# arnab39/equiadapt

Measured on AMD Instinct MI355X. Metric: canonicalize+invert images/sec (224x224 C8), higher is better.
Workload: dtype f32 (resampling / FFT / accumulation in fp32; the network's channel contraction as 2xfp16 split of every fp32 operand (within one fp32 ulp), 3 exact products, fp32 accumulate -- closer to fp64 than the fp32 matrix instruction, see step_ms_by_gemm_form); 1 GPU; configs[1]: 224x224x3 synthetic, C8, GroupEquivariantImageCanonicalization + ESCNNEquivariantNetwork in e2cnn's LAYER SHAPES (32 fields x 8 = 256 ch, k5, 3 layers, crop 0.8, resize 96) with this repository's own filter-bank parameterisation (bilinear-rotated banks; e2cnn's steerable basis is not restated -- e2cnn-trained weights enter via load_exported_dense), forward, then invert_canonicalization; batch_per_gpu=256, global_batch=256, parallelism=dp1 (no collective in the forward path)

## Files before the change

equiadapt_amd/_lib.py:

```python
import ctypes
import os
import subprocess
import threading

_HERE = os.path.dirname(os.path.abspath(__file__))
ROOT = os.path.dirname(_HERE)
CSRC = os.path.join(_HERE, "csrc")
SO_PATH = os.environ.get("EQA_LIB") or os.path.join(CSRC, "libeqa_hip.so")
SOURCES = [os.path.join(CSRC, f) for f in ("group_action.hip", "crop_resize.hip", "nearest_action.hip", "pooling.hip", "batchnorm.hip", "winograd.hip", "lift_conv.hip", "lift_conv_wide.hip", "lift_wgrad.hip", "pointcloud.hip", "vnsmall_train.hip", "vnsmall_tail.hip", "fftconv.hip", "lift_fft.hip", "cgemm3m.hip", "cgemm3m_bf16.hip", "smallconv.hip", "planegemm.hip", "convnet_train.hip")]
HEADERS = [os.path.join(CSRC, "eqa_common.hpp"), os.path.join(CSRC, "vn_common.hpp"), os.path.join(CSRC, "fft48.inc"), os.path.join(CSRC, "fft_common.inc")]
INCLUDE = os.path.join(ROOT, "include")

ABI_VERSION = 3

_c_f = ctypes.POINTER(ctypes.c_float)
_c_i = ctypes.POINTER(ctypes.c_int32)
_vp = ctypes.c_void_p
_int = ctypes.c_int

SIGNATURES = {
    "eqa_abi_version": (_int, []),
    "eqa_set_option": (_int, [_int, _int]),
    "eqa_get_option": (_int, [_int]),
    "eqa_fold_edge_pad_workspace_bytes": (ctypes.c_int64, [_int] * 4),
    "eqa_fold_edge_pad": (_int, [_vp, _vp, _vp, _int, _int, _int, _int, _vp]),
    "eqa_canon_transform_fwd": (_int, [_vp, _vp, _vp, _vp, _vp] + [_int] * 6 + [_vp]),
    "eqa_invert_action_fwd": (_int, [_vp, _vp, _vp, _vp, _vp, _vp] + [_int] * 6 + [_vp]),
    "eqa_group_action_pair": (_int, [_vp] * 4 + [_int, _int] + [_vp] * 5 + [_int, _int, _vp] + [_int] * 4 + [_vp]),
    "eqa_orbit_expand_fwd": (_int, [_vp, _vp, _vp, _vp] + [_int] * 5 + [_vp]),
    "eqa_group_action_fwd": (_int, [_vp, _vp, _vp, _vp, _vp, _vp] + [_int] * 12 + [_vp]),
    "eqa_group_action_fwd_hint": (_int, [_vp, _vp, _vp, _vp, _vp, _vp] + [_int] * 13 + [_vp]),
    "eqa_crop_resize_aa": (_int, [_vp] * 6 + [_int] * 9 + [_vp]),
    "eqa_mask_action_nearest": (_int, [_vp] * 5 + [_int] * 4 + [_vp]),
    "eqa_mask_action_nearest_planes": (_int, [_vp] * 5 + [_int] * 4 + [_vp]),
    "eqa_boxes_action": (_int, [_vp] * 5 + [_int, ctypes.c_float, _int, _vp]),
    "eqa_image_action_nearest": (_int, [_vp] * 5 + [_int] * 10 + [_vp]),
    "eqa_group_action_bwd_tiles": (_int, [_int, _int]),
    "eqa_group_action_bwd": (_int, [_vp] * 8 + [_int] * 12 + [_vp]),
    "eqa_group_action_bwd_theta": (_int, [_vp] * 8 + [_int] * 12 + [_vp]),
    "eqa_group_pool_workspace_bytes": (ctypes.c_int64, [_int] * 4),
    "eqa_group_pool_argmax": (_int, [_vp, _vp, _vp, _vp] + [_int] * 4 + [_vp]),
    "eqa_window_sums": (_int, [_vp, _vp, _vp, _int, _vp] + [_int] * 5 + [_vp]),
    "eqa_bn_partial_blocks": (ctypes.c_int64, [ctypes.c_int64]),
    "eqa_bn_stats_nhwc": (_int, [_vp, _vp, ctypes.c_int64, _int, _vp]),
    "eqa_bn_relu_dropout_nhwc": (_int, [_vp, _vp, _vp, _vp, ctypes.c_int64, _int, ctypes.c_float, ctypes.c_uint32, _vp]),
    "eqa_bn_bwd_reduce_nhwc": (_int, [_vp] * 5 + [ctypes.c_float, _vp, ctypes.c_int64, _int, _vp, _vp, ctypes.c_uint32, _vp]),
    "eqa_bn_bwd_apply_nhwc": (_int, [_vp] * 8 + [ctypes.c_float, _vp, ctypes.c_int64, _int, _vp, _vp, ctypes.c_uint32, _vp]),
    "eqa_window_sums_nhwc_act": (_int, [_vp, _vp, _vp, _int, ctypes.c_float, ctypes.c_uint32, _vp, _vp] + [_int] * 5 + [_vp]),
    "eqa_bn_bwd_reduce_nhwc_wsgrad": (_int, [_vp] * 4 + [ctypes.c_float, _vp] + [_int] * 5 + [_vp, _vp, ctypes.c_uint32, _vp]),
    "eqa_bn_bwd_apply_nhwc_wsgrad": (_int, [_vp] * 7 + [ctypes.c_float, _vp] + [_int] * 5 + [_vp, _vp, ctypes.c_uint32, _vp]),
    "eqa_vn_blocks": (_int, [_int]),
    "eqa_vn_knn": (_int, [_vp, _vp, _int, _int, _int, _vp]),
    "eqa_vn_convpos_stats": (_int, [_vp, _vp, _vp, _vp, _int, _int, _int, _vp]),
    "eqa_vn_convpos_fwd": (_int, [_vp] * 7 + [_int, _int, _int, _vp]),
    "eqa_vn_convpos_bwd_reduce": (_int, [_vp] * 10 + [_int, _int, _int, _vp]),
    "eqa_vn_convpos_bwd_apply": (_int, [_vp] * 12 + [_int, _int, _int, _vp]),
    "eqa_vn_tail_blocks": (_int, [_int]),
    "eqa_vn_tail_partial_floats": (_int, [_int]),
    "eqa_vn_tail_pass": (_int, [_int] + [_vp] * 8 + [_int, _int, _vp]),
    "eqa_vn_bn_finalize": (_int, [_vp, _int, _int, _int, ctypes.c_int64] + [_vp] * 5 + [ctypes.c_float, ctypes.c_float, _vp, _vp]),
    "eqa_vn_bn_bwd_finalize": (_int, [_vp, _int, _int, _int, ctypes.c_int64, _vp, _vp, _vp]),
    "eqa_window_grad_table": (_int, [_vp, _vp] + [_int] * 5 + [_vp]),
    "eqa_window_sums_gemv_bwd_workspace_bytes": (ctypes.c_int64, [_int, _int]),
    "eqa_window_sums_gemv_bwd": (_int, [_vp] * 6 + [_int, _int, _int, ctypes.c_double, _vp]),
    "eqa_window_sums_gemv": (_int, [_vp, _vp, _vp, _int, _int, _int, ctypes.c_double, ctypes.c_double, _vp]),
    "eqa_lift_conv_nhwc": (_int, [_vp, _vp, _vp, _int, _vp] + [_int] * 7 + [_vp]),
    "eqa_lift_conv_grouped": (_int, [_vp, _vp, _vp, _int, _vp] + [_int] * 7 + [_vp]),
    "eqa_lift_conv_stats_rows": (_int, [_int] * 7),
    "eqa_lift_conv_nhwc_stats": (_int, [_vp, _vp, _vp, _vp] + [_int] * 7 + [_vp]),
    "eqa_lift_conv_wgrad_supported": (_int, [_int] * 7),
    "eqa_lift_conv_wgrad_workspace_bytes": (ctypes.c_int64, [_int] * 7),
    "eqa_lift_conv_wgrad_nhwc": (_int, [_vp, _vp, _vp, _vp] + [_int] * 7 + [_vp]),
    "eqa_plane_gemm_supported": (_int, [_int, _int]),
    "eqa_plane_gemm": (_int, [_vp, _vp, _vp, ctypes.c_longlong, _int, _int, _int, _vp]),
    "eqa_winograd_f2k5_input": (_int, [_vp, _vp, _vp, _int, _int, _int, _int, _int, _vp]),
    "eqa_winograd_f2k5_output": (_int, [_vp, _vp, _int, _vp, _int, _int, _int, _int, _vp]),
    "eqa_winograd_f4k5_input": (_int, [_vp, _vp, _vp, _int, _int, _int, _int, _int, _vp]),
    "eqa_winograd_f4k5_output": (_int, [_vp, _vp, _int, _vp, _int, _int, _int, _int, _vp]),
    "eqa_winograd_f2k5_input_padded": (_int, [_vp, _vp, _int, _int, _int, _int, _int, _vp]),
    "eqa_winograd_f4k5_input_padded": (_int, [_vp, _vp, _int, _int, _int, _int, _int, _vp]),
    "eqa_winograd_f2k5_output_adjoint": (_int, [_vp, _vp, _int, _int, _int, _int, _vp]),
    "eqa_winograd_f4k5_output_adjoint": (_int, [_vp, _vp, _int, _int, _int, _int, _vp]),
    "eqa_winograd_f2k5_output_sums_workspace_bytes": (ctypes.c_int64, [_int] * 4),
    "eqa_winograd_f2k5_output_sums": (_int, [_vp, _vp, _int, _vp, _vp] + [_int] * 5 + [_vp]),
    "eqa_winograd_f4k5_output_sums": (_int, [_vp, _vp, _int, _vp, _vp] + [_int] * 5 + [_vp]),
    "eqa_fft48k5_tiles": (ctypes.c_int64, [_int]),
    "eqa_fft48k5_tile_pitch": (ctypes.c_int64, [ctypes.c_int64]),
    "eqa_fft48k5_frequencies": (_int, []),
    "eqa_fft48k5_filter_spectra": (_int, [_vp, _vp, _int, _int, _int, _vp]),
    "eqa_fft48k5_input_grad": (_int, [_vp, _vp, _vp] + [_int] * 4 + [_vp]),
    "eqa_fft48k5_grad_transform": (_int, [_vp, _vp, _vp] + [_int] * 4 + [_vp]),
    "eqa_fft48k5_filter_grad": (_int, [_vp, _vp, _int, _int, _vp]),
    "eqa_fft48k5_filter_grad3m": (_int, [_vp, _vp, _int, _int, _vp]),
    "eqa_fft48k5_cgemm3m_supported": (_int, [_int, _int]),
    "eqa_fft48k5_spectra3m_floats": (ctypes.c_int64, [_int, _int]),
    "eqa_fft48k5_filter_spectra3m": (_int, [_vp, _vp, _int, _int, _int, _vp]),
    "eqa_fft48k5_cgemm3m": (_int, [_vp, _vp, _vp, ctypes.c_int64, _int, _int, _vp]),
    "eqa_lift_conv_wide_supported": (_int, [_int, _int, _int, _int]),
    "eqa_lift_conv_wide_weight_floats": (ctypes.c_int64, [_int, _int, _int, _int]),
    "eqa_lift_conv_wide": (_int, [_vp, _vp, _vp, _int, _vp, _int, _int, _int, _int, _int, _int, _int, _vp]),
    "eqa_lift_conv_wide_wgrad_workspace_bytes": (ctypes.c_int64, [_int, _int, _int, _int]),
    "eqa_lift_conv_wide_wgrad": (_int, [_vp, _vp, _vp, _vp, _int, _int, _int, _int, _int, _int, _int, _vp]),
    "eqa_fft48k5_spectra3m_bf16_bytes": (ctypes.c_int64, [_int, _int]),
    "eqa_fft48k5_spectra3m_split": (_int, [_vp, _vp, _int, _int, _vp]),
    "eqa_fft48k5_cgemm3m_bf16x3": (_int, [_vp, _vp, _vp, ctypes.c_int64, _int, _int, _int, _vp]),
    "eqa_fft48k5_spectra3m_f16_bytes": (ctypes.c_int64, [_int, _int]),
    "eqa_fft48k5_spectra3m_split_f16": (_int, [_vp, _vp, _int, _int, ctypes.c_float, _vp]),
    "eqa_fft48k5_cgemm3m_f16x2": (_int, [_vp, _vp, _vp, ctypes.c_int64, _int, _int, _vp, _int, ctypes.c_float, _vp]),
    "eqa_fft48k5_wgrad3m_supported": (_int, [_int, _int]),
    "eqa_fft48k5_wgrad3m": (_int, [_vp, _vp, _vp, ctypes.c_int64, _int, _int, _vp]),
    "eqa_fft48k5_group": (_int, [_int, _int]),
    "eqa_fft48k5_workspace_bytes": (ctypes.c_int64, [_int] * 4),
    "eqa_fft48k5_input": (_int, [_vp, _vp, _vp, _vp] + [_int] * 5 + [_vp]),
    "eqa_fft48k5_input_grouped": (_int, [_vp, _vp, _vp, _vp] + [_int] * 5 + [_vp]),
    "eqa_fft48k5_input_grouped_supported": (_int, [_int]),
    "eqa_lift5_fft48k5_input_supported": (_int, [_int] * 4),
    "eqa_lift5_fft48k5_input": (_int, [_vp, _vp, _vp, _int, _vp] + [_int] * 4 + [_vp]),
    "eqa_lift5_fft48k5_input_dcmax": (_int, [_vp, _vp, _vp, _int, _vp, _vp] + [_int] * 4 + [_vp]),
    "eqa_lift5_pieces_f16_bytes": (ctypes.c_int64, [_int]),
    "eqa_absmax_slots": (_int, [_vp, ctypes.c_int64, _vp, _vp]),
    "eqa_lift5_fft48k5_input_f16x2": (_int, [_vp, _vp, ctypes.c_float, _vp, _int, _vp, _int, _vp, _vp] + [_int] * 4 + [_vp]),
    "eqa_lift5_pieces_bytes": (ctypes.c_int64, [_int]),
    "eqa_lift5_fft48k5_input_bf16x3": (_int, [_vp, _vp, _vp, _int, _vp] + [_int] * 4 + [_vp]),
    "eqa_fft48k5_output": (_int, [_vp, _vp, _vp, _int, _vp] + [_int] * 4 + [_vp]),
    "eqa_fft48k5_output_stats_rows": (ctypes.c_int64, [_int] * 4),
    "eqa_fft48k5_output_stats": (_int, [_vp, _vp, _vp, _vp] + [_int] * 4 + [_vp]),
    "eqa_fft48k5_output_sums": (_int, [_vp, _vp, _vp, _int, _vp, _vp] + [_int] * 5 + [_vp]),
    "eqa_fft48_supported": (_int, [_int]),
    "eqa_fft48_tiles": (ctypes.c_int64, [_int, _int]),
    "eqa_fft48_workspace_bytes": (ctypes.c_int64, [_int] * 5),
    "eqa_fft48_filter_spectra": (_int, [_vp, _vp, _int, _int, _int, _int, _vp]),
    "eqa_fft48_filter_spectra3m": (_int, [_vp, _vp, _int, _int, _int, _int, _vp]),
    "eqa_fft48_input": (_int, [_vp, _vp, _vp, _vp] + [_int] * 6 + [_vp]),
    "eqa_fft48_grad_transform": (_int, [_vp, _vp, _vp] + [_int] * 5 + [_vp]),
    "eqa_fft48_output": (_int, [_vp, _vp, _vp, _int, _vp] + [_int] * 5 + [_vp]),
    "eqa_fft48_input_grad": (_int, [_vp, _vp, _vp] + [_int] * 5 + [_vp]),
    "eqa_fft48_filter_grad": (_int, [_vp, _vp, _int, _int, _int, _int, _vp]),
    "eqa_conv_s2_supported": (_int, [_int] * 5),
    "eqa_conv_s2": (_int, [_vp, _vp, _vp, _int, _vp] + [_int] * 8 + [_vp]),
    "eqa_conv_s2_wgrad_supported": (_int, [_int] * 5),
    "eqa_conv_s2_wgrad_workspace_bytes": (ctypes.c_int64, [_int] * 8),
    "eqa_conv_s2_wgrad": (_int, [_vp] * 4 + [_int] * 8 + [_vp]),
    "eqa_conv_s2_dgrad_supported": (_int, [_int] * 4),
    "eqa_conv_s2_dgrad": (_int, [_vp] * 3 + [_int] * 7 + [_vp]),
    "eqa_bn_act_fwd": (_int, [_vp] * 5 + [ctypes.c_int64, _int, _int, _vp]),
    "eqa_bn_act_partial_blocks": (ctypes.c_int64, [ctypes.c_int64]),
    "eqa_bn_act_stats": (_int, [_vp, _vp, ctypes.c_int64, _int, _vp]),
    "eqa_bn_act_finalize": (_int, [_vp, ctypes.c_int64, _int, _vp, _vp, ctypes.c_double, ctypes.c_double] + [_vp] * 6 + [_vp]),
    "eqa_bn_act_bwd_finalize": (_int, [_vp, ctypes.c_int64, _int] + [_vp] * 7 + [_vp]),
    "eqa_bn_act_bwd_reduce": (_int, [_vp] * 8 + [ctypes.c_int64, _int, _int, _vp]),
    "eqa_bn_act_bwd_apply": (_int, [_vp] * 11 + [ctypes.c_int64, _int, _int, _vp]),
    "eqa_affine_relu_rows": (_int, [_vp, _vp, _vp, _vp, ctypes.c_int64, _int, _vp]),
    "eqa_cosine_group_activations": (_int, [_vp, _vp, _vp, _int, _int, _int, ctypes.c_float, _vp]),
    "eqa_bias_relu_nhwc": (_int, [_vp, _vp, ctypes.c_int64, _int, _vp]),
    "eqa_window_sums_nhwc_workspace_bytes": (ctypes.c_int64, [_int] * 4),
    "eqa_window_sums_nhwc": (_int, [_vp, _vp, _vp, _int, _vp, _vp] + [_int] * 5 + [_vp]),
    "eqa_window_sums_bwd_expand_nhwc": (_int, [_vp, _vp] + [_int] * 5 + [_vp]),
    "eqa_group_argmax": (_int, [_vp, _vp, _int, _int, _vp]),
    "eqa_vnsmall_workspace_bytes": (ctypes.c_int64, [_int, _int]),
    "eqa_vnsmall_fwd": (_int, [_vp, _vp, _vp, _vp, _int, _int, _int, _int, _vp]),
    "eqa_vnsmall_canonicalize": (_int, [_vp] * 6 + [_int] * 4 + [_vp]),
    "eqa_so3_rotate": (_int, [_vp, _vp, _vp, _int, _int, _int, _vp]),
    "eqa_gram_schmidt": (_int, [_vp, _vp, _int, _vp]),
    "eqa_gram_schmidt_bwd": (_int, [_vp, _vp, _vp, _int, _vp]),
    "eqa_modified_gram_schmidt": (_int, [_vp, _vp, _int, _vp]),
    "eqa_rigid_rows": (_int, [_vp, _vp, _vp, _vp, _int, _int, _vp]),
}

_lock = threading.Lock()
_lib = None


def source_hash(*names: str) -> str:
    import hashlib

    h = hashlib.sha1()
    for path in [os.path.join(CSRC, n) for n in names] + HEADERS:
        with open(path, "rb") as f:
            h.update(f.read())
    return h.hexdigest()[:16]


class EqaLibraryError(RuntimeError):
    pass


def build(force: bool = False, verbose: bool = False, extra_flags=(), out: str = None) -> str:
    import hashlib
    from concurrent.futures import ThreadPoolExecutor

    if extra_flags and not out:
        raise ValueError("a variant build (extra_flags) needs its own `out`: it must not replace the product library")
    out = out or SO_PATH
    hdr_time = max(os.path.getmtime(p) for p in HEADERS + [os.path.join(INCLUDE, "eqa_hip.h")])
    newest_src = max(hdr_time, max(os.path.getmtime(p) for p in SOURCES))
    if not force and not extra_flags and os.path.exists(out) and os.path.getmtime(out) >= newest_src:
        return out
    hipcc = os.environ.get("HIPCC", "/opt/rocm/bin/hipcc")
    flags = ["--offload-arch=gfx950", "-O3", "-fno-slp-vectorize", "-std=c++17", "-fPIC", "-I", INCLUDE, *extra_flags]
    tag = hashlib.sha1(" ".join(flags).encode()).hexdigest()[:10]
    objdir = os.path.join(CSRC, "_obj")
    os.makedirs(objdir, exist_ok=True)
    import fcntl

    lock_file = open(os.path.join(objdir, ".lock"), "w")
    fcntl.flock(lock_file, fcntl.LOCK_EX)
    try:
        if not force and not extra_flags and os.path.exists(out) and os.path.getmtime(out) >= newest_src:
            return out
        return _build_locked(hipcc, flags, tag, objdir, out, hdr_time, force, verbose, bool(extra_flags))
# ... 98 lines not shown
```

equiadapt_amd/csrc/crop_resize.hip:

```cpp
#include "eqa_common.hpp"

namespace {

constexpr int kAaBand = 8;
#ifndef EQA_AA_WIDE_MIN_K
#define EQA_AA_WIDE_MIN_K 8
#endif
constexpr int kAaMaxK = 20;

__global__ __launch_bounds__(kThreads) void crop_resize_aa_kernel(const float* __restrict__ x, float* __restrict__ y,
                                                                 const float* __restrict__ wx, const int32_t* __restrict__ x0,
                                                                 const float* __restrict__ wy, const int32_t* __restrict__ y0,
                                                                 int H, int W, int OH, int OW, int K, int max_rows) {
  extern __shared__ __attribute__((aligned(16))) float aa_tmp[];
  const int plane = blockIdx.y;
  const int r0 = blockIdx.x * kAaBand, r1 = min(r0 + kAaBand, OH);
  const int ybeg = y0[r0];
  const int yend = min(y0[r1 - 1] + K, H);
  const int nrows = min(yend - ybeg, max_rows);
  const float* src = x + (size_t)plane * H * W;
  const int rows_par = kThreads / OW;
  if (rows_par >= 1) {
    const int ox = threadIdx.x % OW, rsub = threadIdx.x / OW;
    if (rsub < rows_par) {
// ... 68 lines not shown
#pragma unroll
  for (int j = 0; j < K; ++j) {
    wv[j] = wx[ox * K + j];
    xo[j] = min(xs_g - xb + j, xl - 1);
  }
  if ((int)threadIdx.x < nband * K) tabw[threadIdx.x] = wy[r0 * K + threadIdx.x];
  const int ybeg = y0[r0];
  if ((int)threadIdx.x < nband) taby[threadIdx.x] = y0[r0 + threadIdx.x] - ybeg;
  const int yend = min(y0[r1 - 1] + K, H);
  const int nrows = min(yend - ybeg, cap_rows);
  const int nq = xl >> 2;
  const int tq = threadIdx.x & 63, tr = threadIdx.x >> 6;
  const bool prefetch = nq <= 64 && nrows <= 4 * NL;
  const size_t plane_sz = (size_t)H * W;
  const float* src0 = x + (size_t)ybeg * W + xb;
  typedef float aa_f4 __attribute__((ext_vector_type(4)));
  aa_f4 v[NL];
#define EQA_AA_PF_LOAD(plane_)                                                                                          \
  do {                                                                                                                  \
    const float* src_ = src0 + (size_t)(plane_) * plane_sz;                                                             \
    _Pragma("unroll") for (int k = 0; k < NL; ++k)                                                           \
      v[k] = *reinterpret_cast<const aa_f4*>(src_ + (size_t)min(tr + 4 * k, nrows - 1) * W + 4 * min(tq, nq - 1));     \
  } while (0)
  __builtin_amdgcn_s_waitcnt(0x0070);
  if (prefetch && plane0 < planes) EQA_AA_PF_LOAD(plane0);
  for (int plane = plane0; plane < planes; plane += plane_step) {
    if (prefetch) {
      if (tq < nq) {
#pragma unroll
        for (int k = 0; k < NL; ++k)
          if (tr + 4 * k < nrows) *reinterpret_cast<aa_f4*>(rows + (tr + 4 * k) * xl + 4 * tq) = v[k];
      }
      if (plane + plane_step < planes) EQA_AA_PF_LOAD(plane + plane_step);
    } else {
      const float* src = src0 + (size_t)plane * plane_sz;
      for (int q = tq; q < nq; q += 64)
        for (int rb = tr; rb < nrows; rb += 4) *reinterpret_cast<aa_f4*>(rows + rb * xl + 4 * q) = *reinterpret_cast<const aa_f4*>(src + (size_t)rb * W + 4 * q);
    }
    __syncthreads();
    if (rows_par >= 1) {
      if (rsub < rows_par) {
        for (int ry0 = rsub; ry0 < nrows; ry0 += 4 * rows_par) {
          float acc[4] = {0.0f, 0.0f, 0.0f, 0.0f};
#pragma unroll
          for (int u = 0; u < 4; ++u) {
            const float* row = rows + min(ry0 + u * rows_par, nrows - 1) * xl;
#pragma unroll
            for (int j = 0; j < K; ++j)
              acc[u] += wv[j] * row[xo[j]];
          }
#pragma unroll
          for (int u = 0; u < 4; ++u)
            if (ry0 + u * rows_par < nrows) tmp[(ry0 + u * rows_par) * OW + ox] = acc[u];
        }
      }
    } else {
      for (int idx = threadIdx.x; idx < nrows * OW; idx += kThreads) {
        const int ry = idx / OW, oxx = idx - ry * OW;
        const float* row = rows + ry * xl;
        const int xs = x0[oxx] - xb;
        float acc = 0.0f;
#pragma unroll
        for (int j = 0; j < K; ++j)
          acc += wx[oxx * K + j] * row[min(xs + j, xl - 1)];
        tmp[ry * OW + oxx] = acc;
      }
    }
    __syncthreads();
    float* dst = y + (size_t)plane * OH * OW;
    for (int idx = threadIdx.x; idx < nband * OW; idx += kThreads) {
      const int r = idx / OW, oxx = idx - r * OW;
      const int ys = taby[r];
      float acc = 0.0f;
#pragma unroll
      for (int j = 0; j < K; ++j)
        acc += tabw[r * K + j] * tmp[min(ys + j, nrows - 1) * OW + oxx];
      dst[(size_t)(r0 + r) * OW + oxx] = acc;
    }
    __syncthreads();
  }
#undef EQA_AA_PF_LOAD
}

__global__ __launch_bounds__(kThreads) void crop_resize_aa_wide_kernel(const float* __restrict__ x, float* __restrict__ y,
                                                                      const float* __restrict__ wx, const int32_t* __restrict__ x0,
                                                                      const float* __restrict__ wy, const int32_t* __restrict__ y0,
                                                                      int H, int W, int OH, int OW, int K, int max_rows, int xbeg,
                                                                      int xlen, int pad_shift, int row_stride, int rpi) {
  extern __shared__ __attribute__((aligned(16))) float aa_tmp[];
  float* rowbuf = aa_tmp + (size_t)max_rows * OW;
  const int plane = blockIdx.y;
  const int r0 = blockIdx.x * kAaBand, r1 = min(r0 + kAaBand, OH);
  const int ybeg = y0[r0];
  const int yend = min(y0[r1 - 1] + K, H);
  const int nrows = min(yend - ybeg, max_rows);
  const float* src = x + (size_t)plane * H * W;
  auto pos = [&](int e) { return pad_shift ? e + (e >> pad_shift) : e; };
  const bool fixed_col = (kThreads % OW) == 0 && K <= kAaMaxK;
  const bool vec_stage = rpi <= 8 && (xlen & 3) == 0 && (xbeg & 3) == 0 && (W & 3) == 0 && ((((uintptr_t)src) & 15) == 0);
  const int ox_fixed = threadIdx.x % OW;
  const int xs_fixed = x0[ox_fixed] - xbeg;
  float wreg[kAaMaxK];
#pragma unroll
  for (int j = 0; j < kAaMaxK; ++j) wreg[j] = (fixed_col && j < K) ? wx[ox_fixed * K + j] : 0.0f;
  const bool prefetch = vec_stage && xlen <= 4 * kThreads;
  const int e_pf = 4 * threadIdx.x;
  float4 pf[8];
  auto pf_load = [&](int ry0) {
    const int nr = min(rpi, nrows - ry0);
#pragma unroll
    for (int rr = 0; rr < 8; ++rr)
      pf[rr] = *reinterpret_cast<const float4*>(src + (size_t)(ybeg + ry0 + min(rr, nr - 1)) * W + xbeg + min(e_pf, xlen - 4));
  };
  if (prefetch && nrows > 0) pf_load(0);
  for (int ry0 = 0; ry0 < nrows; ry0 += rpi) {
    const int nr = min(rpi, nrows - ry0);
    if (prefetch) {
      if (e_pf < xlen) {
#pragma unroll
        for (int rr = 0; rr < 8; ++rr) {
          if (rr < nr) {
            float* lrow = rowbuf + rr * row_stride;
            lrow[pos(e_pf)] = pf[rr].x; lrow[pos(e_pf + 1)] = pf[rr].y; lrow[pos(e_pf + 2)] = pf[rr].z; lrow[pos(e_pf + 3)] = pf[rr].w;
          }
        }
      }
      if (ry0 + rpi < nrows) pf_load(ry0 + rpi);
    } else if (vec_stage) {
      for (int e = 4 * threadIdx.x; e < xlen; e += 4 * kThreads) {
        float4 v[8];
#pragma unroll
        for (int rr = 0; rr < 8; ++rr)
          v[rr] = *reinterpret_cast<const float4*>(src + (size_t)(ybeg + ry0 + min(rr, nr - 1)) * W + xbeg + e);
#pragma unroll
        for (int rr = 0; rr < 8; ++rr) {
          if (rr < nr) {
            float* lrow = rowbuf + rr * row_stride;
            lrow[pos(e)] = v[rr].x; lrow[pos(e + 1)] = v[rr].y; lrow[pos(e + 2)] = v[rr].z; lrow[pos(e + 3)] = v[rr].w;
          }
        }
      }
    } else {
      for (int rr = 0; rr < nr; ++rr) {
        const float* grow = src + (size_t)(ybeg + ry0 + rr) * W + xbeg;
        float* lrow = rowbuf + rr * row_stride;
        for (int e = threadIdx.x; e < xlen; e += kThreads) lrow[pos(e)] = grow[e];
      }
    }
    __syncthreads();
    if (fixed_col) {
      for (int rr = threadIdx.x / OW; rr < nr; rr += kThreads / OW) {
        const float* row = rowbuf + rr * row_stride;
        float acc = 0.0f;
#pragma unroll
        for (int j = 0; j < kAaMaxK; ++j)
          if (j < K) acc += wreg[j] * row[pos(min(xs_fixed + j, xlen - 1))];
        aa_tmp[(ry0 + rr) * OW + ox_fixed] = acc;
      }
    } else {
      for (int idx = threadIdx.x; idx < nr * OW; idx += kThreads) {
        const int rr = idx / OW, ox = idx - rr * OW;
        const float* row = rowbuf + rr * row_stride;
        const int xs = x0[ox] - xbeg;
        float acc = 0.0f;
        for (int j = 0; j < K; ++j) acc += wx[ox * K + j] * row[pos(min(xs + j, xlen - 1))];
        aa_tmp[(ry0 + rr) * OW + ox] = acc;
// ... 12 lines not shown
  }
}

constexpr int kAaStreamRows = 8;
__global__ __launch_bounds__(kThreads) void crop_resize_aa_stream_kernel(const float* __restrict__ x, float* __restrict__ y,
                                                                        const float* __restrict__ wx, const int32_t* __restrict__ x0,
                                                                        const float* __restrict__ wy, const int32_t* __restrict__ y0,
                                                                        int H, int W, int OH, int OW, int K, int xbeg, int xlen,
                                                                        int pad_shift, int row_stride) {
  extern __shared__ __attribute__((aligned(16))) float aa_rows[];
  const int plane = blockIdx.y;
  const int r0 = blockIdx.x * kAaBand, nr_out = min(kAaBand, OH - r0);
  int ys[kAaBand];
#pragma unroll
  for (int r = 0; r < kAaBand; ++r) ys[r] = y0[r0 + min(r, nr_out - 1)];
  const int ybeg = ys[0];
  const int span = ys[kAaBand - 1] + K - ybeg;
  const float* src = x + (size_t)plane * H * W + xbeg;
  const int e = 4 * (int)threadIdx.x;
  const int e_ld = min(e, xlen - 4);
  auto pos = [&](int i) { return pad_shift ? i + (i >> pad_shift) : i; };
  float4 acc[kAaBand];
#pragma unroll
  for (int r = 0; r < kAaBand; ++r) acc[r] = make_float4(0.f, 0.f, 0.f, 0.f);
  auto load8 = [&](float4 (&v)[kAaStreamRows], int yc) {
#pragma unroll
    for (int q = 0; q < kAaStreamRows; ++q)
      v[q] = *reinterpret_cast<const float4*>(src + (size_t)min(ybeg + yc + q, H - 1) * W + e_ld);
  };
  const int lane = threadIdx.x & 63;
  const int wq = lane >> 3, wr = lane & 7;
  const int ys_w = y0[r0 + min(wr, nr_out - 1)];
  auto wload = [&](int yc) {
    const int t = ybeg + yc + wq - ys_w;
    const bool ok = wr < nr_out && t >= 0 && t < K && yc + wq < span;
    return ok ? wy[(size_t)(r0 + wr) * K + min(max(t, 0), K - 1)] : 0.0f;
  };
  auto add8 = [&](const float4 (&v)[kAaStreamRows], float wv) {
#pragma unroll
    for (int q = 0; q < kAaStreamRows; ++q) {
#pragma unroll
      for (int r = 0; r < kAaBand; ++r) {
        const float w = __builtin_bit_cast(float, __builtin_amdgcn_readlane(__builtin_bit_cast(int, wv), 8 * q + r));
        acc[r].x += w * v[q].x; acc[r].y += w * v[q].y; acc[r].z += w * v[q].z; acc[r].w += w * v[q].w;
      }
    }
  };
  static_assert(kAaStreamRows == 8 && kAaBand == 8, "one weight per lane: 8 rows of a trip x 8 output rows = 64 lanes");
  float4 va[kAaStreamRows], vb[kAaStreamRows];
  float wa, wb = 0.0f;
  load8(va, 0);
  wa = wload(0);
  for (int yc = 0; yc < span; yc += 2 * kAaStreamRows) {
    if (yc + kAaStreamRows < span) { load8(vb, yc + kAaStreamRows); wb = wload(yc + kAaStreamRows); }
    add8(va, wa);
    if (yc + 2 * kAaStreamRows < span) { load8(va, yc + 2 * kAaStreamRows); wa = wload(yc + 2 * kAaStreamRows); }
    if (yc + kAaStreamRows < span) add8(vb, wb);
  }
  float* dst = y + (size_t)plane * OH * OW;
#pragma unroll
  for (int half = 0; half < 2; ++half) {
    if (e < xlen) {
#pragma unroll
      for (int rr = 0; rr < kAaBand / 2; ++rr) {
        float* lrow = aa_rows + rr * row_stride;
        const float4 v = acc[half * (kAaBand / 2) + rr];
        lrow[pos(e)] = v.x; lrow[pos(e + 1)] = v.y; lrow[pos(e + 2)] = v.z; lrow[pos(e + 3)] = v.w;
      }
    }
    __syncthreads();
    for (int idx = threadIdx.x; idx < (kAaBand / 2) * OW; idx += kThreads) {
      const int rr = idx / OW, ox = idx - rr * OW;
      const int r = half * (kAaBand / 2) + rr;
      if (r < nr_out) {
        const float* row = aa_rows + rr * row_stride;
        const int xs = x0[ox] - xbeg;
        float a = 0.0f;
        for (int j = 0; j < K; ++j) a += wx[ox * K + j] * row[pos(min(xs + j, xlen - 1))];
        dst[(size_t)(r0 + r) * OW + ox] = a;
      }
    }
    __syncthreads();
  }
}

}

extern "C" {

int eqa_crop_resize_aa(const float* x, float* y, const float* wx, const int32_t* x0, const float* wy, const int32_t* y0,
                       int planes, int H, int W, int OH, int OW, int K, int max_rows, int x_begin, int x_span, void* stream) {
  if (!x || !y || !wx || !x0 || !wy || !y0 || planes < 0 || H <= 0 || W <= 0 || OH <= 0 || OW <= 0 || K <= 0 || max_rows <= 0)
    return EQA_ERR_INVALID_ARG;
  const size_t lds = (size_t)max_rows * OW * sizeof(float);
  if (lds > 96 * 1024 || planes > 65535) return EQA_ERR_UNSUPPORTED;
  if (planes == 0) return EQA_OK;
  const dim3 grid((OH + kAaBand - 1) / kAaBand, planes);
  if (K > EQA_AA_WIDE_MIN_K && x_span > 0 && x_begin >= 0 && x_begin + x_span <= W) {
    const int stride = (x_span + OW / 2) / OW;
    const int pad_shift = (stride >= 2 && (stride & 1) == 0) ? __builtin_ctz((unsigned)stride) : 0;
    const int row_stride = x_span + (pad_shift ? (x_span >> pad_shift) : 0) + 1;
    const size_t row_bytes = (size_t)row_stride * sizeof(float);
    const int rpi = (int)std::min<size_t>(8, lds + row_bytes <= 96 * 1024 ? (96 * 1024 - lds) / row_bytes : 0);
    const size_t lds2 = lds + (size_t)rpi * row_bytes;
    static const bool stream_off = [] { const char* e = getenv("EQA_AA_STREAM"); return e && e[0] == '0'; }();
    if (!stream_off && x_span <= 4 * kThreads && (x_span & 3) == 0 && (x_begin & 3) == 0 && (W & 3) == 0 && (((uintptr_t)x) & 15) == 0 &&
        (size_t)(kAaBand / 2) * row_bytes <= 64 * 1024) {
      hipLaunchKernelGGL(crop_resize_aa_stream_kernel, grid, dim3(kThreads), (kAaBand / 2) * row_bytes, (hipStream_t)stream, x, y, wx, x0, wy,
                         y0, H, W, OH, OW, K, x_begin, x_span, pad_shift, row_stride);
      return launch_status();
    }
    if (rpi >= 1) {
      hipLaunchKernelGGL(crop_resize_aa_wide_kernel, grid, dim3(kThreads), lds2, (hipStream_t)stream, x, y, wx, x0, wy, y0, H, W, OH,
                         OW, K, max_rows, x_begin, x_span, pad_shift, row_stride, rpi);
      return launch_status();
    }
  }
  static const bool staged_off = [] { const char* e = getenv("EQA_AA_STAGED"); return e && e[0] == '0'; }();
  if (!staged_off && K <= EQA_AA_WIDE_MIN_K && (W & 3) == 0 && (((uintptr_t)x) & 15) == 0 && x_span > 0 && x_begin >= 0 &&
      x_begin + x_span <= W) {
    const int xb = x_begin & ~3, xl = std::min(W, (x_begin + x_span + 3) & ~3) - xb;
    static const int band_env = [] { const char* e = getenv("EQA_AA_BAND"); return e ? atoi(e) : 0; }();
    int band = band_env == 16 ? 16 : (band_env == 8 ? 8 : (OH >= 64 ? 16 : 8));
    auto staged_lds = [&](int bnd) { return ((size_t)(bnd / kAaBand) * max_rows * (xl + OW) + bnd * (EQA_AA_WIDE_MIN_K + 1)) * sizeof(float); };
    if (band == 16 && band_env != 16 && (staged_lds(16) > 64 * 1024 || 16 * K > kThreads)) band = 8;
    const int cap_rows = (band / kAaBand) * max_rows;
    const size_t lds3 = staged_lds(band);
    if (lds3 <= 64 * 1024 && band * K <= kThreads) {
      static const int per_cu = [] { const char* e = getenv("EQA_AA_BLOCKS_PER_CU"); return e ? std::max(1, atoi(e)) : 12; }();
      const int nbands = (OH + band - 1) / band;
      const int groups = std::max(1, (std::min(planes, (256 * per_cu + nbands - 1) / nbands) + kXcd - 1) / kXcd);
      const bool few = cap_rows <= 20;
#define EQA_AA_STAGED(K_)                                                                                                              \
  case K_:                                                                                                                             \
    if (band == 16)                                                                                                                    \
      hipLaunchKernelGGL((crop_resize_aa_staged_kernel<K_, 16, 10>), dim3(kXcd, nbands, groups), dim3(kThreads), lds3, (hipStream_t)stream, x, \
                         y, wx, x0, wy, y0, planes, H, W, OH, OW, cap_rows, xb, xl);                                                   \
    else if (few)                                                                                                                      \
      hipLaunchKernelGGL((crop_resize_aa_staged_kernel<K_, 8, 5>), dim3(kXcd, nbands, groups), dim3(kThreads), lds3, (hipStream_t)stream, x,  \
                         y, wx, x0, wy, y0, planes, H, W, OH, OW, cap_rows, xb, xl);                                                   \
    else                                                                                                                               \
      hipLaunchKernelGGL((crop_resize_aa_staged_kernel<K_, 8, 10>), dim3(kXcd, nbands, groups), dim3(kThreads), lds3, (hipStream_t)stream, x, \
                         y, wx, x0, wy, y0, planes, H, W, OH, OW, cap_rows, xb, xl);                                                   \
    break
      switch (K) {
        EQA_AA_STAGED(1); EQA_AA_STAGED(2); EQA_AA_STAGED(3); EQA_AA_STAGED(4); EQA_AA_STAGED(5); EQA_AA_STAGED(6); EQA_AA_STAGED(7);
        EQA_AA_STAGED(8);
        default: return EQA_ERR_UNSUPPORTED;
      }
#undef EQA_AA_STAGED
      return launch_status();
    }
  }
  hipLaunchKernelGGL(crop_resize_aa_kernel, grid, dim3(kThreads), lds, (hipStream_t)stream, x, y, wx, x0, wy, y0, H, W, OH, OW, K,
                     max_rows);
  return launch_status();
}

}
```

equiadapt_amd/csrc/fftconv.hip:

```cpp
#include <cstdlib>

#include "eqa_common.hpp"

namespace {

#include "fft_common.inc"

typedef float f32x2 __attribute__((ext_vector_type(2)));
__device__ __forceinline__ void fft_ldg2(const float2* p, float& re, float& im) {
  const f32x2 v = __builtin_nontemporal_load(reinterpret_cast<const f32x2*>(p));
  re = v[0];
  im = v[1];
}

__device__ __forceinline__ void fft_load_column(const float2* __restrict__ p, size_t fpitch, bool edge, float (&re)[kFftN],
                                                float (&im)[kFftN]) {
#pragma unroll
  for (int ky = 0; ky < kFftH; ++ky) fft_ldg2(p + ky * fpitch, re[ky], im[ky]);
  const float2* base2 = edge ? p + (size_t)(kFftH - 2) * fpitch : p + (size_t)kFftH * fpitch;
  const ptrdiff_t step2 = edge ? -(ptrdiff_t)fpitch : (ptrdiff_t)fpitch;
  const unsigned flip = edge ? 0x80000000u : 0u;
#pragma unroll
  for (int ky = kFftH; ky < kFftN; ++ky) {
    fft_ldg2(base2 + (ky - kFftH) * step2, re[ky], im[ky]);
// ... 1218 lines not shown
  if (x_grouped) return EQA_ERR_UNSUPPORTED;
  const unsigned cb = (C + kThreads - 1) / kThreads;
  const int chunk = fft_chunk_images(nimg, H, TX, C);
  for (int i0 = 0; i0 < nimg; i0 += chunk) {
    const int n = std::min(chunk, nimg - i0);
    hipLaunchKernelGGL(fft48_rows_fwd_kernel<kFftO>, dim3((unsigned)((size_t)n * H * TX), cb), dim3(kThreads), 0, st,
                       x + (size_t)i0 * H * W * C, T, in_bias, in_relu, H, W, C, TX, win);
    hipLaunchKernelGGL(fft48_cols_fwd_kernel<kFftO>, dim3((unsigned)((size_t)n * TY * TX * kFftH), cb), dim3(kThreads), 0, st, T, V, H, C,
                       TY, TX, fft_pitch(M), (size_t)i0 * TY * TX, fft_group_in(C), win);
  }
  return launch_status();
}

int eqa_fft48k5_input(const float* x, float* T, float* V, const float* in_bias, int in_relu, int nimg, int H, int W, int C,
                      void* stream) {
  if (!x || !T || !V || !fft_dims_ok(nimg, H, W, C)) return EQA_ERR_INVALID_ARG;
  if (nimg == 0) return EQA_OK;
  return fft_forward_impl(x, T, V, in_bias, in_relu, nimg, H, W, C, (int)eqa_fft48k5_tiles(H), (int)eqa_fft48k5_tiles(W), kFftN,
                          (hipStream_t)stream);
}

int eqa_fft48k5_input_grouped_supported(int C) {
  static const bool two_pass = getenv("EQA_FFT_TWO_PASS") != nullptr;
  return C > 0 && C % kFusCh == 0 && !two_pass;
}

int eqa_fft48k5_input_grouped(const float* x, float* T, float* V, const float* in_bias, int in_relu, int nimg, int H, int W, int C,
                              void* stream) {
  if (!x || !T || !V || !fft_dims_ok(nimg, H, W, C)) return EQA_ERR_INVALID_ARG;
  if (!eqa_fft48k5_input_grouped_supported(C)) return EQA_ERR_UNSUPPORTED;
  if (nimg == 0) return EQA_OK;
  return fft_forward_impl(x, T, V, in_bias, in_relu, nimg, H, W, C, (int)eqa_fft48k5_tiles(H), (int)eqa_fft48k5_tiles(W), kFftN,
                          (hipStream_t)stream, 1);
}

int eqa_fft48k5_grad_transform(const float* dy, float* T, float* G, int nimg, int OH, int OW, int C, void* stream) {
  if (!dy || !T || !G || nimg < 0 || OH <= 0 || OW <= 0 || C <= 0) return EQA_ERR_INVALID_ARG;
  if (nimg == 0) return EQA_OK;
  return fft_forward_impl(dy, T, G, nullptr, 0, nimg, OH, OW, C, (OH + kFftO - 1) / kFftO, (OW + kFftO - 1) / kFftO, kFftO,
                          (hipStream_t)stream);
}

int eqa_fft48k5_filter_grad(const float* D, float* dbank, int Cout, int Cin, void* stream) {
  if (!D || !dbank || Cout <= 0 || Cin <= 0) return EQA_ERR_INVALID_ARG;
  if (Cin > 65535) return EQA_ERR_UNSUPPORTED;
  hipLaunchKernelGGL((fft48_filter_grad_kernel<false, 5>), dim3(Cin, (Cout + kThreads - 1) / kThreads), dim3(kThreads), 0, (hipStream_t)stream, D,
                     dbank, Cout, Cin, fft_group_in(Cin), fft_group_in(Cout));
  return launch_status();
}

int eqa_fft48k5_filter_grad3m(const float* D, float* dbank, int Cout, int Cin, void* stream) {
  if (!D || !dbank || Cout <= 0 || Cin <= 0) return EQA_ERR_INVALID_ARG;
  if (Cin > 65535 || Cin % kFusCh || Cout % kFusCh) return EQA_ERR_UNSUPPORTED;
  hipLaunchKernelGGL((fft48_filter_grad_kernel<true, 5>), dim3(Cin, (Cout + kThreads - 1) / kThreads), dim3(kThreads), 0, (hipStream_t)stream, D,
                     dbank, Cout, Cin, kFusCh, kFusCh);
  return launch_status();
}

int eqa_fft48k5_output(const float* Mo, float* T2, const float* bias, int relu, float* y, int nimg, int OH, int OW, int C,
                       void* stream) {
  if (!Mo || !T2 || !y || nimg < 0 || OH <= 0 || OW <= 0 || C <= 0) return EQA_ERR_INVALID_ARG;
  if (nimg == 0) return EQA_OK;
  int fused = 0;
  const int rc = fft_output_impl<0>(Mo, T2, bias, relu, y, nimg, OH, OW, C, (hipStream_t)stream, &fused);
  return rc != EQA_OK ? rc : launch_status();
}

int64_t eqa_fft48k5_output_stats_rows(int nimg, int OH, int OW, int C) {
  if (nimg <= 0 || OH <= 0 || OW <= 0 || C <= 0) return 0;
  int fused = 0;
  int64_t rows = 0;
  const int rc = fft_output_impl<0>(nullptr, nullptr, nullptr, 0, nullptr, nimg, OH, OW, C, nullptr, &fused, nullptr, &rows);
  return rc == EQA_OK ? rows : 0;
}

int eqa_fft48k5_output_stats(const float* Mo, float* T2, float* y, double* partial, int nimg, int OH, int OW, int C, void* stream) {
  if (!Mo || !T2 || !y || !partial || nimg < 0 || OH <= 0 || OW <= 0 || C <= 0) return EQA_ERR_INVALID_ARG;
  if (nimg == 0) return EQA_OK;
  int fused = 0;
  const int rc = fft_output_impl<0>(Mo, T2, nullptr, 0, y, nimg, OH, OW, C, (hipStream_t)stream, &fused, partial);
  return rc != EQA_OK ? rc : launch_status();
}

int eqa_fft48k5_output_sums(const float* Mo, float* T2, const float* bias, int relu, double* S, void* workspace, int nimg,
                            int OH, int OW, int C, int k_next, void* stream) {
  if (!Mo || !T2 || !S || !workspace || nimg < 0 || OH <= 0 || OW <= 0 || C <= 0 || k_next <= 0) return EQA_ERR_INVALID_ARG;
  const int nb = k_next - 1;
  if ((nb != 4 && nb != 2) || OH < 2 * nb + 1 || OW < 2 * nb + 1 || k_next > kMaxWinK || nimg > 65535) return EQA_ERR_UNSUPPORTED;
  if (nimg == 0) return EQA_OK;
  hipStream_t st = (hipStream_t)stream;
  float* part = (float*)workspace;
  int fused = 0;
  const int rc = nb == 4 ? fft_output_impl<4>(Mo, T2, bias, relu, part, nimg, OH, OW, C, st, &fused)
                         : fft_output_impl<2>(Mo, T2, bias, relu, part, nimg, OH, OW, C, st, &fused);
  if (rc != EQA_OK) return rc;
  const int sub = fused ? (OW + kFftO - 1) / kFftO : 1;
  const int per_row = fused == 3 ? kPipeCons / 64 : fused;
  const int nseg = fused ? 2 * nb + per_row * ((OH + kFftO - 1) / kFftO) : OH;
  return eqa::launch_window_sums_nhwc_finalize(part, S, nimg, C, k_next, nseg * sub, st, sub);
}

}

namespace {

template <int KS>
struct FftK {
  static constexpr int O = kFftN + 1 - KS;

  static int forward(const float* x, float* T, float* V, const float* in_bias, int in_relu, int nimg, int H, int W, int C, int TY, int TX,
                     int win, hipStream_t st) {
    const size_t M = (size_t)nimg * TY * TX;
    if ((size_t)nimg * H * TX > 0x7fffffffULL || M * kFftH > 0x7fffffffULL) return EQA_ERR_UNSUPPORTED;
    static const bool two_pass = getenv("EQA_FFT_TWO_PASS") != nullptr;
    if (C % kFusCh == 0 && M * (C / kFusCh) <= 0x7fffffffULL && !two_pass &&
        allow_dynamic_lds((const void*)fft48_fwd_fused_kernel<O>, kFusLds * 4)) {
      const unsigned nwork = (unsigned)(M * (C / kFusCh));
      const size_t xb = (size_t)nimg * H * W * C * 4, vb = (size_t)kFftF * fft_pitch(M) * 2 * C * 4;
      hipLaunchKernelGGL(fft48_fwd_fused_kernel<O>, dim3(nwork), dim3(kFusThreads), kFusLds * sizeof(float), st, x, V, in_bias, in_relu, H,
                         W, C, TY, TX, fft_pitch(M), nwork, win, xb <= 0xfffffff0ULL ? (unsigned)xb : 0u,
                         vb <= 0xfffffff0ULL ? (unsigned)vb : 0u, 0);
      return launch_status();
    }
    const unsigned cb = (C + kThreads - 1) / kThreads;
    const int chunk = fft_chunk_images(nimg, H, TX, C);
    for (int i0 = 0; i0 < nimg; i0 += chunk) {
      const int n = std::min(chunk, nimg - i0);
      hipLaunchKernelGGL(fft48_rows_fwd_kernel<O>, dim3((unsigned)((size_t)n * H * TX), cb), dim3(kThreads), 0, st,
                         x + (size_t)i0 * H * W * C, T, in_bias, in_relu, H, W, C, TX, win);
      hipLaunchKernelGGL(fft48_cols_fwd_kernel<O>, dim3((unsigned)((size_t)n * TY * TX * kFftH), cb), dim3(kThreads), 0, st, T, V, H, C,
                         TY, TX, fft_pitch(M), (size_t)i0 * TY * TX, fft_group_in(C), win);
    }
    return launch_status();
  }

  static int output(const float* Mo, float* T2, const float* bias, int relu, float* y, int nimg, int OH, int OW, int C, hipStream_t st) {
    const int TY = (OH + O - 1) / O, TX = (OW + O - 1) / O;
    const size_t M = (size_t)nimg * TY * TX;
    if ((size_t)nimg * OH > 0x7fffffffULL || M * kFftH > 0x7fffffffULL) return EQA_ERR_UNSUPPORTED;
    static const bool two_pass = getenv("EQA_FFT_TWO_PASS") != nullptr;
    constexpr int lds_bytes = kFftH * (kFftN * 2 * kInvCh + kInvCh) * (int)sizeof(float);
    if (C % kInvCh == 0 && M * (C / kInvCh) <= 0x7fffffffULL && !two_pass &&
        allow_dynamic_lds((const void*)fft48_inv_fused_kernel<0, kInvCh, O>, lds_bytes)) {
      const unsigned nwork = (unsigned)(M * (C / kInvCh));
      const size_t mo_total = (size_t)kFftF * fft_pitch(M) * C * 8;
      hipLaunchKernelGGL((fft48_inv_fused_kernel<0, kInvCh, O>), dim3(nwork), dim3(kFftN * kInvCh), lds_bytes, st, Mo, bias, relu, y, OH, OW, C,
                         TY, TX, fft_pitch(M), nwork, mo_total <= 0xfffffff0ULL ? (unsigned)mo_total : 0u);
      return launch_status();
    }
    const unsigned cb = (C + kThreads - 1) / kThreads;
    const int chunk = fft_chunk_images(nimg, OH, TX, C);
    for (int i0 = 0; i0 < nimg; i0 += chunk) {
      const int n = std::min(chunk, nimg - i0);
      hipLaunchKernelGGL((fft48_cols_inv_kernel<false, O>), dim3((unsigned)((size_t)n * TY * TX * kFftH), cb), dim3(kThreads), 0, st, Mo, T2,
                         OH, C, TY, TX, fft_pitch(M), (size_t)i0 * TY * TX);
      hipLaunchKernelGGL((fft48_rows_inv_kernel<0, O>), dim3((unsigned)((size_t)n * OH), cb), dim3(kThreads), 0, st, T2, bias, relu, y, OH,
                         OW, C, TX, (size_t)i0);
    }
    return launch_status();
  }

  static int input_grad(const float* Cg, float* T2, float* dx, int nimg, int H, int W, int C, hipStream_t st) {
    const int OH = H - (KS - 1), OW = W - (KS - 1);
    const int TY = (OH + O - 1) / O, TX = (OW + O - 1) / O;
    const size_t M = (size_t)nimg * TY * TX;
    if ((size_t)nimg * H > 0x7fffffffULL || M * kFftH > 0x7fffffffULL) return EQA_ERR_UNSUPPORTED;
    const unsigned cb = (C + kThreads - 1) / kThreads;
    const int chunk = fft_chunk_images(nimg, TY * kFftN, TX, C);
    for (int i0 = 0; i0 < nimg; i0 += chunk) {
      const int n = std::min(chunk, nimg - i0);
      hipLaunchKernelGGL((fft48_cols_inv_kernel<true, O>), dim3((unsigned)((size_t)n * TY * TX * kFftH), cb), dim3(kThreads), 0, st, Cg, T2,
                         OH, C, TY, TX, fft_pitch(M), (size_t)i0 * TY * TX);
      hipLaunchKernelGGL(fft48_rows_inv_add_kernel<O>, dim3((unsigned)((size_t)n * H), cb), dim3(kThreads), 0, st, T2,
                         dx + (size_t)i0 * H * W * C, H, W, C, TY, TX);
    }
    return launch_status();
  }

  static int spectra(const float* bank, float* B, int Cout, int Cin, float sgn, hipStream_t st) {
    hipLaunchKernelGGL(fft48_filter_spectra_kernel<KS>, dim3(Cin, (Cout + kThreads - 1) / kThreads), dim3(kThreads), 0, st, bank, B, Cout,
                       Cin, fft_group_in(Cin), sgn);
    return launch_status();
// ... 101 lines not shown
```

equiadapt_amd/csrc/lift_fft.hip:

```cpp
#include <cstdlib>

#include "eqa_common.hpp"

#ifndef EQA_LF_AUX
#define EQA_LF_AUX 2
#endif

namespace {

#include "fft_common.inc"

typedef float f32x4 __attribute__((ext_vector_type(4)));
typedef unsigned u32x4 __attribute__((ext_vector_type(4)));

#ifdef EQA_LF_CLOCK
__device__ unsigned long long g_lf_clock[64];
__device__ __forceinline__ int lf_clock_slot(int wave) { return wave == 8 ? 0 : wave == 1 ? 1 : wave == 0 ? 2 : wave == 6 ? 3 : wave == 11 ? 4 : -1; }
#define LF_CLOCK_BEGIN() const bool lfc_on = blockIdx.x == 0 && (threadIdx.x & 63) == 0 && lf_clock_slot(wave) >= 0; \
  if (blockIdx.x == 0 && (threadIdx.x & 63) == 0) { unsigned hw_; asm volatile("s_getreg_b32 %0, hwreg(HW_REG_HW_ID)" : "=s"(hw_)); g_lf_clock[40 + wave] = hw_; } \
  unsigned long long lfc_t = __builtin_readcyclecounter(); unsigned long long lfc_s[16] = {0, 0, 0, 0, 0, 0, 0, 0, 0, 0, 0, 0, 0, 0, 0, 0}
#define LF_CLOCK(i) do { const unsigned long long n_ = __builtin_readcyclecounter(); lfc_s[i] += n_ - lfc_t; lfc_t = n_; } while (0)
#define LF_CLOCK_END() do { if (lfc_on) for (int i_ = 0; i_ < 8; ++i_) g_lf_clock[8 * lf_clock_slot(wave) + i_] = lfc_s[i_]; } while (0)
#else
#define LF_CLOCK_BEGIN() do { } while (0)
// ... 88 lines not shown
                                                 int relu, float* __restrict__ V, int H0, int W0, int C, int TY, int TX, size_t Mp,
                                                 unsigned nwork, unsigned v_bytes, unsigned x_bytes, unsigned bank_bytes,
                                                 float* __restrict__ dcmax, const float* __restrict__ xbound, int nxbound, float w_scale) {
  constexpr bool COLS = ROLE == kCols;
  constexpr bool PIECES = FORM == 3;
  constexpr bool H2 = FORM == 2;
  constexpr int NSUB = PIECES ? 12 : (H2 ? 4 : 3);
  constexpr int SUBROWS = kFftN / NSUB;
  constexpr int NGRP = 12 / NSUB;
  extern __shared__ float lds[];
  float* const tile = lds;
  float* const patch = lds + kLfTileFloats;
  const int tid = threadIdx.x;
  const int lane = tid & 63;
  const int wave = __builtin_amdgcn_readfirstlane(tid >> 6);
  const int j = lane & 15, q = lane >> 4;
  const int ngrp = C / kLfCh;
  const int H1 = H0 - 4, W1 = W0 - 4;
  const unsigned nblk = gridDim.x;
  const unsigned patch_b = (unsigned)(kLfTileFloats * 4);
  LF_CLOCK_BEGIN();

  const __amdgpu_buffer_rsrc_t xr = __builtin_amdgcn_make_buffer_rsrc(const_cast<float*>(x), 0, x_bytes, 0x00020000);
  float pre[COLS ? kLfPre : 1];
  auto prefetch = [&](const LfItem& it, int sub, bool live) {
    if constexpr (COLS) {
      int tq = tid;
      asm volatile("" : "+v"(tq));
#pragma unroll
      for (int i = 0; i < kLfPre; ++i) {
        const int idx = tq + kLfStagers * i;
        const int pr = idx / kLfPatchPitch, pc = idx - pr * kLfPatchPitch;
        const int gy = it.gy0 + kLfSubRows * sub + pr, gxc = it.gx0 * 3 + pc;
        const bool ok = live && idx < kLfPatchFloats && gy < H0 && gxc < W0 * 3;
        const unsigned off = ok ? (unsigned)(((it.img * H0 + gy) * (size_t)(W0 * 3) + gxc) * 4) : 0xfffffff0u;
        pre[i] = __builtin_bit_cast(float, __builtin_amdgcn_raw_buffer_load_b32(xr, off, 0, 0));
      }
    }
  };
  auto stage = [&]() {
    if constexpr (COLS) {
#pragma unroll
      for (int i = 0; i < kLfPre; ++i) {
        const int idx = tid + kLfStagers * i;
        if (idx < kLfPatchFloats) patch[idx] = pre[i];
      }
    }
  };

  float preg[COLS && PIECES ? 2 : 1][3];
  auto prefetch_grp = [&](const LfItem& it, int g, int which, bool live) {
    if constexpr (COLS && PIECES) {
      int tq = tid;
      asm volatile("" : "+v"(tq));
      const int pr = tq / 52, px = tq - pr * 52;
      const int gy = it.gy0 + 4 * g + pr, gx = it.gx0 + px;
      const bool ok = live && tq < 208 && gy < H0 && gx < W0;
      const unsigned off = ok ? (unsigned)((((it.img * H0 + gy) * (size_t)W0 + gx) * 3) * 4) : 0xfffffff0u;
#pragma unroll
      for (int c = 0; c < 3; ++c) preg[which][c] = __builtin_bit_cast(float, __builtin_amdgcn_raw_buffer_load_b32(xr, off, c * 4, 0));
    }
  };
  auto stage_grp = [&](int g, int which) {
    if constexpr (COLS && PIECES) {
      if (tid < 208) {
        const int pr = tid / 52, px = tid - pr * 52;
        __bf16 pc[3][3];
#pragma unroll
        for (int c = 0; c < 3; ++c) lf_split3(preg[which][c], pc[0][c], pc[1][c], pc[2][c]);
        char* dst = reinterpret_cast<char*>(lds) + patch_b + ((4 * g + pr) & 7) * kLpRowB + px * 8;
#pragma unroll
        for (int pl = 0; pl < 3; ++pl) {
          const lf_bf16x4 v = {pc[pl][0], pc[pl][1], pc[pl][2], (__bf16)0.0f};
          *reinterpret_cast<lf_bf16x4*>(dst + pl * kLpPlaneB) = v;
        }
      }
    }
  };

  float preh[(!COLS && H2) ? kLhPre : 1][3];
  float x_scale = 1.0f, out_scale = 1.0f;
  if constexpr (H2) {
    float mx = 0.0f;
    for (int t = lane; t < nxbound; t += 64) mx = fmaxf(mx, xbound[t]);
#pragma unroll
    for (int o = 32; o > 0; o >>= 1) mx = fmaxf(mx, __shfl_xor(mx, o));
    int ex = 0;
    if (mx > 0.0f && mx < 3.0e38f) (void)frexpf(mx, &ex);
    ex = __builtin_amdgcn_readfirstlane(min(max(14 - ex, -100), 100));
    x_scale = ldexpf(1.0f, ex);
    out_scale = ldexpf(1.0f, -ex) / w_scale;
  }
  int h_pr[(!COLS && H2) ? kLhPre : 1], h_px[(!COLS && H2) ? kLhPre : 1];
  if constexpr (!COLS && H2) {
#pragma unroll
    for (int i = 0; i < kLhPre; ++i) {
      const int idx = tid - 6 * 64 + kLfStagers * i;
      h_pr[i] = idx / 52;
      h_px[i] = idx - h_pr[i] * 52;
    }
  }
  auto prefetch_h = [&](const LfItem& it, int row0, int nrows, bool live) {
    if constexpr (!COLS && H2) {
#ifdef EQA_LF_H2_NOPREFETCH
      if (row0 >= 0) return;
#endif
#pragma unroll
      for (int i = 0; i < kLhPre; ++i) {
        const int pr = h_pr[i], px = h_px[i];
        const int gy = it.gy0 + row0 + pr, gx = it.gx0 + px;
        const bool ok = live && pr < nrows && gy < H0 && gx < W0;
        const unsigned off = ok ? (unsigned)((((it.img * H0 + gy) * (size_t)W0 + gx) * 3) * 4) : 0xfffffff0u;
#pragma unroll
        for (int c = 0; c < 3; ++c) preh[i][c] = __builtin_bit_cast(float, __builtin_amdgcn_raw_buffer_load_b32(xr, off, c * 4, 0));
      }
    }
  };
  auto stage_h = [&](int row0, int nrows) {
    if constexpr (!COLS && H2) {
#pragma unroll
      for (int i = 0; i < kLhPre; ++i) {
        asm volatile("" : "+v"(preh[i][0]), "+v"(preh[i][1]), "+v"(preh[i][2]));
        if (h_pr[i] < nrows) {
          const int pr = h_pr[i], px = h_px[i];
          _Float16 hi[3], lo[3];
#pragma unroll
          for (int c = 0; c < 3; ++c) {
            const float v = preh[i][c] * x_scale;
            hi[c] = (_Float16)v;
            lo[c] = (_Float16)(v - (float)hi[c]);
          }
          char* dst = reinterpret_cast<char*>(lds) + patch_b + ((row0 + pr) & (kLhRing - 1)) * kLhRowB + px * 8;
          const lf_f16x4 vh = {hi[0], hi[1], hi[2], (_Float16)0.0f}, vl = {lo[0], lo[1], lo[2], (_Float16)0.0f};
          *reinterpret_cast<lf_f16x4*>(dst) = vh;
          *reinterpret_cast<lf_f16x4*>(dst + kLhPlaneB) = vl;
        }
      }
    }
  };

  const int nr = (wave == 10 || wave == 11) ? 2 : 3;
  const int r0 = wave == 8 ? 0 : (wave == 9 ? 3 : (wave == 6 ? 6 : (wave == 10 ? 9 : (wave == 7 ? 11 : 14))));
  unsigned a_off[kLfSteps];
  float wreg[kLfSteps];
  f32x4 bias4;
  auto setup = [&](const LfItem& it) {
    const __amdgpu_buffer_rsrc_t br = __builtin_amdgcn_make_buffer_rsrc(const_cast<float*>(bank), 0, bank_bytes, 0x00020000);
    const unsigned wb = (unsigned)((it.grp * kLfCh + j) * 75 * 4);
#pragma unroll
    for (int t = 0; t < kLfSteps; ++t) {
      int ky, e;
      bool spare;
      lf_slot(4 * t + q, ky, e, spare);
      a_off[t] = patch_b + (unsigned)(((r0 + ky) * kLfPatchPitch + j * 3 + e) * 4);
      wreg[t] = __builtin_bit_cast(float, __builtin_amdgcn_raw_buffer_load_b32(br, spare ? 0xfffffff0u : wb + (unsigned)((ky * 15 + e) * 4), 0, 0));
    }
#pragma unroll
    for (int r = 0; r < 4; ++r) bias4[r] = bias ? bias[it.grp * kLfCh + 4 * q + r] : 0.0f;
    asm volatile("" : "+v"(bias4));
  };
#ifndef EQA_LF_AHEAD
#define EQA_LF_AHEAD 5
#endif
  constexpr int kAhead = EQA_LF_AHEAD;
  auto conv_rows = [&](const LfItem& it, int y0) {
    float b[3][kLfSteps], bq[2][3][kAhead];
    auto lds_at = [&](int t, int drow, int tx3) {
// ... 617 lines not shown
```

equiadapt_amd/csrc/pooling.hip:

```cpp
#include "eqa_common.hpp"

namespace {


constexpr int kPoolSplitTarget = 2048;


template <bool VEC>
__global__ __launch_bounds__(kThreads) void group_pool_partial_kernel(const float* __restrict__ feat,
                                                                     double* __restrict__ partial, int Cf, int G,
                                                                     int HW, int cps, int splits) {
  extern __shared__ __attribute__((aligned(16))) double acc[];
  const int s = blockIdx.x, b = blockIdx.y;
  const int tid = threadIdx.x, lane = tid & 63, wave = tid >> 6;
  for (int k = tid; k < 4 * G; k += kThreads) acc[k] = 0.0;
  __syncthreads();
  const int c_lo = s * cps, c_hi = min(c_lo + cps, Cf);
  const int planes = (c_hi - c_lo) * G;
  const float* base = feat + ((size_t)b * Cf + c_lo) * G * HW;
  for (int p = wave; p < planes; p += 4) {
    const float* pl = base + (size_t)p * HW;
    float v0 = 0.f, v1 = 0.f, v2 = 0.f, v3 = 0.f;
    if (VEC) {
      const float4* p4 = reinterpret_cast<const float4*>(pl);
// ... 343 lines not shown
#endif
  for (int it = threadIdx.x; it < nch * kk; it += blockDim.x) {
    const int cl = it / kk, uv = it - cl * kk;
    const int u = uv / k, v = uv - u * k;
    if constexpr (KW > 0) {
      constexpr int NB = KW - 1;
      float p0[NB], pc[NB][NB];
      double tc[NB];
#pragma unroll
      for (int r = 0; r < NB; ++r) p0[r] = s_brd[r < u ? r : NB + r][cl * nval];
#pragma unroll
      for (int j = 0; j < NB; ++j) {
        const int i = j < v ? 1 + j : 1 + NB + j;
        tc[j] = s_tot[cl * nval + i];
#pragma unroll
        for (int r = 0; r < NB; ++r) pc[j][r] = s_brd[r < u ? r : NB + r][cl * nval + i];
      }
      double a = s_tot[cl * nval];
#pragma unroll
      for (int r = 0; r < NB; ++r) a -= (double)p0[r];
#pragma unroll
      for (int j = 0; j < NB; ++j) {
        a -= tc[j];
#pragma unroll
        for (int r = 0; r < NB; ++r) a += (double)pc[j][r];
      }
      out[((size_t)b * C + c0) * kk + it] = a;
    } else {
      auto P = [&](int s, int i) { return (double)s_brd[s][cl * nval + i]; };
      double a = s_tot[cl * nval];
      for (int r = 0; r < nb; ++r) a -= r < u ? P(r, 0) : P(nb + r, 0);
      for (int j = 0; j < nb; ++j) {
        const int i = j < v ? 1 + j : 1 + nb + j;
        a -= s_tot[cl * nval + i];
        for (int r = 0; r < nb; ++r) a += r < u ? P(r, i) : P(nb + r, i);
      }
      out[((size_t)b * C + c0) * kk + it] = a;
    }
  }
}

constexpr int kGemvMaxE = 16;

template <int THREADS, int EMAX, int COLS>
__global__ __launch_bounds__(THREADS) void sums_gemv_kernel(const double* __restrict__ S, const double* __restrict__ Wm,
                                                            float* __restrict__ act, int K, int E, double scale, double shift) {
  __shared__ double s_red[THREADS / 64][kGemvMaxE];
  const int b = blockIdx.x;
  const double* sb = S + (size_t)b * K;
  double acc[kGemvMaxE];
#pragma unroll
  for (int e = 0; e < kGemvMaxE; ++e) acc[e] = 0.0;
  for (int j = threadIdx.x; j < K; j += COLS * THREADS) {
    double s[COLS], w[COLS][EMAX];
#pragma unroll
    for (int u = 0; u < COLS; ++u) {
      const bool in = j + u * THREADS < K;
      s[u] = in ? sb[j + u * THREADS] : 0.0;
#pragma unroll
      for (int e = 0; e < EMAX; ++e) w[u][e] = (in && e < E) ? Wm[(size_t)e * K + j + u * THREADS] : 0.0;
    }
#pragma unroll
    for (int u = 0; u < COLS; ++u)
#pragma unroll
      for (int e = 0; e < EMAX; ++e)
        if (e < E && j + u * THREADS < K) acc[e] += s[u] * w[u][e];
  }
  const int lane = threadIdx.x & 63, wave = threadIdx.x >> 6;
#pragma unroll
  for (int e = 0; e < kGemvMaxE; ++e) {
    double v = acc[e];
#pragma unroll
    for (int off = 32; off > 0; off >>= 1) v += __shfl_down(v, off, 64);
    if (lane == 0) s_red[wave][e] = v;
  }
  __syncthreads();
  if (threadIdx.x < E) {
    double v = 0.0;
    for (int w = 0; w < THREADS / 64; ++w) v += s_red[w][threadIdx.x];
    act[(size_t)b * E + threadIdx.x] = (float)(v * scale + shift);
  }
}


__global__ __launch_bounds__(kThreads) void affine_relu_rows_kernel(const float* __restrict__ h, const float* __restrict__ scale,
                                                                   const float* __restrict__ shift, float* __restrict__ z, size_t n_vec,
                                                                   int Dq) {
  const size_t i0 = (size_t)blockIdx.x * kThreads + threadIdx.x, stride = (size_t)gridDim.x * kThreads;
  QuadWalk w(i0, stride, Dq);
  for (size_t i = i0; i < n_vec; i += stride, w.next()) {
    const int q = (int)w.q;
    const float4 v = reinterpret_cast<const float4*>(h)[i];
    const float4 sc = reinterpret_cast<const float4*>(scale)[q], sh = reinterpret_cast<const float4*>(shift)[q];
    reinterpret_cast<float4*>(z)[i] = make_float4(fmaxf(v.x * sc.x + sh.x, 0.f), fmaxf(v.y * sc.y + sh.y, 0.f),
                                                  fmaxf(v.z * sc.z + sh.z, 0.f), fmaxf(v.w * sc.w + sh.w, 0.f));
  }
}

__global__ __launch_bounds__(kThreads) void cosine_group_activations_kernel(const float* __restrict__ v, const float* __restrict__ ref,
                                                                           float* __restrict__ act, int B, int G, int V, float eps) {
  const int lane = threadIdx.x & 63;
  const int r = blockIdx.x * (kThreads / 64) + (threadIdx.x >> 6);
  if (r >= G * B) return;
  float rr = 0.f, vv = 0.f;
  for (int k = lane; k < V; k += 64) {
    const float a = ref[k], x = v[(size_t)r * V + k];
    rr += a * a;
    vv += x * x;
  }
  rr = wave_sum_f(rr);
  vv = wave_sum_f(vv);
  const float inv_r = 1.0f / fmaxf(sqrtf(rr), eps), inv_v = 1.0f / fmaxf(sqrtf(vv), eps);
  float dot = 0.f;
  for (int k = lane; k < V; k += 64) dot += (ref[k] * inv_r) * (v[(size_t)r * V + k] * inv_v);
  dot = wave_sum_f(dot);
  if (lane == 0) act[(size_t)(r % B) * G + r / B] = dot;
}

}

int eqa::launch_window_sums_nhwc_finalize(const float* part, double* S, int B, int C, int k, int nseg, hipStream_t stream, int sub) {
  if (B > 65535) return EQA_ERR_UNSUPPORTED;
  const dim3 fgrid((C + kFinCh - 1) / kFinCh, B);
  const dim3 fblock(std::min(C, kFinCh) * (2 * k - 1) > kThreads ? kFinThreads : kThreads);
  if (k == 5)
    hipLaunchKernelGGL(window_sums_nhwc_finalize_kernel<5>, fgrid, fblock, 0, stream, part, S, B, C, k, nseg, sub);
  else if (k == 3)
    hipLaunchKernelGGL(window_sums_nhwc_finalize_kernel<3>, fgrid, fblock, 0, stream, part, S, B, C, k, nseg, sub);
  else if (k - 1 <= kWsSmallBorder)
    hipLaunchKernelGGL(window_sums_nhwc_finalize_kernel<0>, fgrid, fblock, 0, stream, part, S, B, C, k, nseg, sub);
  else
    hipLaunchKernelGGL((window_sums_nhwc_finalize_kernel<0, kWsMaxBorder>), fgrid, fblock, 0, stream, part, S, B, C, k, nseg, sub);
  return launch_status();
}

namespace {

constexpr int kWgtCh = 64;
__global__ __launch_bounds__(kWgtCh) void window_grad_table_kernel(const double* __restrict__ dS, float* __restrict__ table, int C, int H,
                                                                  int W, int k) {
  extern __shared__ double s_p[];
  const int kk = k * k, stride = kk + 1;
  const int b = blockIdx.y, c0 = blockIdx.x * kWgtCh, nch = min(kWgtCh, C - c0);
  const double* src = dS + ((size_t)b * C + c0) * kk;
  for (int i = threadIdx.x; i < nch * kk; i += kWgtCh) s_p[(i / kk) * stride + i % kk] = src[i];
  __syncthreads();
  const int c = threadIdx.x;
  if (c >= nch) return;
  double* p = s_p + c * stride;
  for (int u = 0; u < k; ++u)
    for (int v = 1; v < k; ++v) p[u * k + v] += p[u * k + v - 1];
  for (int u = 1; u < k; ++u)
    for (int v = 0; v < k; ++v) p[u * k + v] += p[(u - 1) * k + v];
  const int nb = k - 1, T = 2 * nb + 1;
  auto range = [&](int t, int n, int& lo, int& hi) {
    const int rep = t <= nb ? t : n - nb + (t - nb - 1);
    lo = max(0, rep - (n - k));
    hi = min(k - 1, rep);
  };
  auto rect = [&](int u0, int u1, int v0, int v1) -> double {
    if (u0 > u1 || v0 > v1) return 0.0;
    double r = p[u1 * k + v1];
    if (u0 > 0) r -= p[(u0 - 1) * k + v1];
    if (v0 > 0) r -= p[u1 * k + v0 - 1];
    if (u0 > 0 && v0 > 0) r += p[(u0 - 1) * k + v0 - 1];
    return r;
// ... 46 lines not shown
  double acc = 0.0;
  for (int s = 0; s < nslice; ++s) acc += partial[(size_t)s * n + i];
  dW[i] = scale * acc;
}

constexpr int kGemvBwdSlices = 16;

}

extern "C" {

int64_t eqa_group_pool_workspace_bytes(int B, int Cf, int G, int HW) {
  (void)HW;
  if (B <= 0 || Cf <= 0 || G <= 0) return 0;
  return (int64_t)B * pool_splits(B, Cf) * G * (int64_t)sizeof(double);
}

int eqa_group_pool_argmax(const float* feat, float* act, int32_t* gidx, void* workspace, int B, int Cf, int G, int HW,
                          void* stream) {
  if (B == 0) return EQA_OK;
  if (!feat || !act || !workspace || B < 0 || Cf <= 0 || G <= 0 || HW <= 0) return EQA_ERR_INVALID_ARG;
  if (gidx && G > 64) return EQA_ERR_UNSUPPORTED;
  if (B > 65535) return EQA_ERR_UNSUPPORTED;
  hipStream_t st = (hipStream_t)stream;
  const int splits = pool_splits(B, Cf);
  const int cps = (Cf + splits - 1) / splits;
  const int used = (Cf + cps - 1) / cps;
  double* partial = (double*)workspace;
  const bool vec = (HW % 4 == 0) && (((uintptr_t)feat & 15) == 0);
  const size_t lds = (size_t)4 * G * sizeof(double);
  if (vec)
    hipLaunchKernelGGL((group_pool_partial_kernel<true>), dim3(used, B), dim3(kThreads), lds, st, feat, partial, Cf, G, HW, cps, used);
  else
    hipLaunchKernelGGL((group_pool_partial_kernel<false>), dim3(used, B), dim3(kThreads), lds, st, feat, partial, Cf, G, HW, cps, used);
  if (hipGetLastError() != hipSuccess) return EQA_ERR_LAUNCH;
  const double inv_count = 1.0 / ((double)Cf * (double)HW);
  hipLaunchKernelGGL(group_pool_finalize_kernel, dim3((B + 3) / 4), dim3(kThreads), 0, st, partial, act, gidx, B, G, used, inv_count);
  return launch_status();
}

int eqa_group_argmax(const float* act, int32_t* gidx, int B, int G, void* stream) {
  if (B == 0 && G > 0 && G <= 64) return EQA_OK;
  if (!act || !gidx || B < 0 || G <= 0) return EQA_ERR_INVALID_ARG;
  if (G > 64) return EQA_ERR_UNSUPPORTED;
  hipLaunchKernelGGL(group_argmax_kernel, dim3((B + 3) / 4), dim3(kThreads), 0, (hipStream_t)stream, act, gidx, B, G);
  return launch_status();
}

int eqa_window_sums(const float* x, const float* scale, const float* shift, int relu, double* out, int B, int C, int H,
                    int W, int k, void* stream) {
  if (!x || !out || B < 0 || C <= 0 || H <= 0 || W <= 0 || k <= 0 || k > H || k > W) return EQA_ERR_INVALID_ARG;
  if (k > kMaxWinK) return EQA_ERR_UNSUPPORTED;
  const size_t lds = (size_t)((H * W + 3) & ~3) * sizeof(float) + (size_t)k * W * sizeof(double);
  if (lds > 64 * 1024 || (long long)B * C > 0x7fffffffLL) return EQA_ERR_UNSUPPORTED;
  if (B == 0) return EQA_OK;
  const bool vec = ((H * W) % 4 == 0) && (((uintptr_t)x & 15) == 0);
  hipStream_t st = (hipStream_t)stream;
  if (vec)
    hipLaunchKernelGGL((window_sums_kernel<true>), dim3((unsigned)(B * C)), dim3(kThreads), lds, st, x, scale, shift, relu, out, C, H, W, k);
  else
    hipLaunchKernelGGL((window_sums_kernel<false>), dim3((unsigned)(B * C)), dim3(kThreads), lds, st, x, scale, shift, relu, out, C, H, W, k);
  return launch_status();
}

int eqa_window_sums_gemv(const double* S, const double* Wm, float* act, int B, int K, int E, double scale, double shift,
                         void* stream) {
  if (B < 0 || K <= 0 || E <= 0) return EQA_ERR_INVALID_ARG;
  if (B == 0) return EQA_OK;
  if (!S || !Wm || !act) return EQA_ERR_INVALID_ARG;
  if (E > kGemvMaxE) return EQA_ERR_UNSUPPORTED;
  const int per_thread = (K + kThreads - 1) / kThreads;
  if (E <= 8 && per_thread > 5)
    hipLaunchKernelGGL((sums_gemv_kernel<kThreads, 8, 9>), dim3(B), dim3(kThreads), 0, (hipStream_t)stream, S, Wm, act, K, E, scale, shift);
  else if (E <= 8 && per_thread > 2)
    hipLaunchKernelGGL((sums_gemv_kernel<kThreads, 8, 5>), dim3(B), dim3(kThreads), 0, (hipStream_t)stream, S, Wm, act, K, E, scale, shift);
  else if (E <= 8)
    hipLaunchKernelGGL((sums_gemv_kernel<kThreads, 8, 2>), dim3(B), dim3(kThreads), 0, (hipStream_t)stream, S, Wm, act, K, E, scale, shift);
  else
    hipLaunchKernelGGL((sums_gemv_kernel<kThreads, kGemvMaxE, 5>), dim3(B), dim3(kThreads), 0, (hipStream_t)stream, S, Wm, act, K, E, scale,
                       shift);
  return launch_status();
}

int eqa_affine_relu_rows(const float* h, const float* scale, const float* shift, float* z, int64_t rows, int D, void* stream) {
  if (!h || !scale || !shift || !z || rows < 0 || D <= 0) return EQA_ERR_INVALID_ARG;
  if (D % 4 != 0 || (((uintptr_t)h | (uintptr_t)z | (uintptr_t)scale | (uintptr_t)shift) & 15)) return EQA_ERR_UNSUPPORTED;
  if (rows == 0) return EQA_OK;
  const size_t n_vec = (size_t)rows * (D / 4);
  const unsigned blocks = (unsigned)std::min<size_t>((n_vec + kThreads - 1) / kThreads, 8192);
  hipLaunchKernelGGL(affine_relu_rows_kernel, dim3(blocks), dim3(kThreads), 0, (hipStream_t)stream, h, scale, shift, z, n_vec, D / 4);
  return launch_status();
}

int eqa_cosine_group_activations(const float* v, const float* ref, float* act, int B, int G, int V, float eps, void* stream) {
  if (!v || !ref || !act || B < 0 || G <= 0 || V <= 0) return EQA_ERR_INVALID_ARG;
  if (B == 0) return EQA_OK;
  if ((int64_t)B * G > 0x7fffffff) return EQA_ERR_UNSUPPORTED;
  const int rows = B * G, per = kThreads / 64;
  hipLaunchKernelGGL(cosine_group_activations_kernel, dim3((rows + per - 1) / per), dim3(kThreads), 0, (hipStream_t)stream, v, ref, act, B,
                     G, V, eps);
  return launch_status();
}

int eqa_bias_relu_nhwc(float* x, const float* bias, int64_t n_pixels, int C, void* stream) {
  if (!x || !bias || n_pixels < 0 || C <= 0) return EQA_ERR_INVALID_ARG;
  if (C % 4 != 0 || (((uintptr_t)x | (uintptr_t)bias) & 15)) return EQA_ERR_UNSUPPORTED;
  if (n_pixels == 0) return EQA_OK;
  const size_t n_vec = (size_t)n_pixels * (C / 4);
  const unsigned blocks = (unsigned)((n_vec + kThreads - 1) / kThreads < 8192 ? (n_vec + kThreads - 1) / kThreads : 8192);
  hipLaunchKernelGGL(bias_relu_nhwc_kernel, dim3(blocks), dim3(kThreads), 0, (hipStream_t)stream, x, bias, n_vec, C / 4);
  return launch_status();
}

int eqa_window_sums_bwd_expand_nhwc(const float* table, float* dx, int B, int H, int W, int C, int k, void* stream) {
  if (!table || !dx || B < 0 || H <= 0 || W <= 0 || C <= 0 || k <= 0 || H < 2 * k - 1 || W < 2 * k - 1) return EQA_ERR_INVALID_ARG;
  if (C % 4 != 0 || (((uintptr_t)table | (uintptr_t)dx) & 15) || (size_t)B * H > 0x7fffffffULL) return EQA_ERR_UNSUPPORTED;
  if (B == 0) return EQA_OK;
  hipLaunchKernelGGL(window_sums_bwd_expand_kernel, dim3((unsigned)((size_t)B * H)), dim3(kThreads), 0, (hipStream_t)stream, table,
                     dx, H, W, C / 4, k - 1);
  return launch_status();
}

static int ws_nhwc_bands(int H, int k) {
  const int interior = H - 2 * (k - 1);
  int nb = (interior + 9) / 10;
  if (nb < 1) nb = 1;
  return nb;
}

int64_t eqa_window_sums_nhwc_workspace_bytes(int B, int C, int H, int k) {
  if (B <= 0 || C <= 0 || H <= 0 || k <= 0) return 0;
  const int nseg = 2 * (k - 1) + ws_nhwc_bands(H, k);
  return (int64_t)B * nseg * C * (1 + 2 * (k - 1)) * (int64_t)sizeof(float);
}

static int window_sums_nhwc_impl(const float* x, const float* scale, const float* shift, int relu, float drop_p, uint32_t seed, double* out,
                                 void* workspace, int B, int C, int H, int W, int k, void* stream);

int eqa_window_sums_nhwc(const float* x, const float* scale, const float* shift, int relu, double* out, void* workspace,
                         int B, int C, int H, int W, int k, void* stream) {
  return window_sums_nhwc_impl(x, scale, shift, relu, 0.0f, 0u, out, workspace, B, C, H, W, k, stream);
}

int eqa_window_sums_nhwc_act(const float* x, const float* scale, const float* shift, int relu, float drop_p, uint32_t seed, double* out,
                             void* workspace, int B, int C, int H, int W, int k, void* stream) {
  if (!(drop_p >= 0.0f && drop_p < 1.0f)) return EQA_ERR_INVALID_ARG;
  return window_sums_nhwc_impl(x, scale, shift, relu, drop_p, seed, out, workspace, B, C, H, W, k, stream);
}

static int window_sums_nhwc_impl(const float* x, const float* scale, const float* shift, int relu, float drop_p, uint32_t seed, double* out,
                                 void* workspace, int B, int C, int H, int W, int k, void* stream) {
  if (!x || !out || !workspace || B < 0 || C <= 0 || H <= 0 || W <= 0 || k <= 0) return EQA_ERR_INVALID_ARG;
  if (k > kMaxWinK || C % 4 != 0 || H < 2 * (k - 1) + 1 || W < 2 * (k - 1) + 1 || B > 65535) return EQA_ERR_UNSUPPORTED;
  if ((((uintptr_t)x) & 15) || (scale && (((uintptr_t)scale) & 15)) || (shift && (((uintptr_t)shift) & 15))) return EQA_ERR_UNSUPPORTED;
  if (B == 0) return EQA_OK;
  hipStream_t st = (hipStream_t)stream;
  const int nbands = ws_nhwc_bands(H, k);
  const int nseg = 2 * (k - 1) + nbands;
  const uint32_t thr = dropout_threshold(drop_p);
#define EQA_WS_SEG(R_, D_)                                                                                                     \
  do {                                                                                                                         \
    if (k - 1 <= kWsSmallBorder)                                                                                               \
      hipLaunchKernelGGL((window_sums_nhwc_segment_kernel<R_, D_>), dim3(nseg, B), dim3(kThreads), 0, st, x, scale, shift, relu, \
                         (float*)workspace, C, H, W, k, nbands, thr, 1.0f / (1.0f - drop_p), seed);                            \
    else                                                                                                                       \
      hipLaunchKernelGGL((window_sums_nhwc_segment_kernel<R_, D_, kWsMaxBorder>), dim3(nseg, B), dim3(kThreads), 0, st, x, scale, \
// ... 58 lines not shown
```

equiadapt_amd/images/canonicalization_networks/escnn_networks.py:

```python
import os
from typing import List, Sequence

import torch
import torch.nn as nn
import torch.nn.functional as F

from equiadapt_amd.images.canonicalization_networks.custom_group_equivariant_layers import (
    RotationEquivariantConv,
    RotationEquivariantConvLift,
    RotoReflectionEquivariantConv,
    RotoReflectionEquivariantConvLift,
)
from equiadapt_amd import ops
from equiadapt_amd.common.utils import update_running_stats
from equiadapt_amd.images.canonicalization_networks import fftconv, winograd
from equiadapt_amd.images.canonicalization_networks.pooling import (
    WindowSumsFunction,
    conv_then_group_pool,
    group_pool,
    window_sums_to_activations,
)


class _InnerBatchNorm(nn.BatchNorm3d):
# ... 361 lines not shown
        shift = bn.bias - bn.running_mean * scale
        b = conv.bias if conv.bias is not None else torch.zeros_like(scale)
        bias = b * scale + shift
        if not isinstance(conv, _DenseConv):
            scale, bias = scale.repeat_interleave(E), bias.repeat_interleave(E)
        bank = conv.expanded_weights() * scale[:, None, None, None]
        bank, bias = bank.contiguous(memory_format=torch.channels_last), bias.contiguous()
        self._fold_cache[id(conv)] = (key, bank, bias)
        return bank, bias

    def _derived(self, conv, build, *tag):
        key = self._fold_cache[id(conv)][0]
        hit = self._fold_cache.get((*tag, id(conv)))
        if hit is None or hit[0] != key:
            hit = (key, build())
            self._fold_cache[(*tag, id(conv))] = hit
        return hit[1]

    @staticmethod
    def _plain_5x5(conv) -> bool:
        return not conv.lifting and conv.kernel_size == 5 and conv.stride == 1 and conv.padding == 0

    @staticmethod
    def _lift_kernel(conv, bank, h, narrow_unchecked: bool = False):
        if not conv.lifting or os.environ.get("EQA_LIFT_MFMA", "1") == "0":
            return None
        k, (cout, cin) = conv.kernel_size, bank.shape[:2]
        unit = conv.stride == 1 and conv.padding == 0
        if (unit or narrow_unchecked) and ops.lift_conv_supported(cin, k, k, cout):
            return "narrow"
        if (unit and h.is_contiguous(memory_format=torch.channels_last) and h.shape[-2] >= k and h.shape[-1] >= k
                and ops.lift_conv_wide_supported(cin, k, k, cout)):
            return "wide"
        return None

    def _route(self, i, h, bank, convs, nhwc):
        conv, tail = convs[i], convs[-1]
        cout, cin = bank.shape[:2]
        k, kt = conv.kernel_size, tail.kernel_size
        last_before_tail = i == len(convs) - 2
        if nhwc and self._plain_5x5(conv) and fftconv.applicable(h, cin, cout):
            return "fft5", (last_before_tail and kt in (3, 5) and tail.supports_linear_tail() and min(h.shape[-2:]) - 4 >= 2 * kt - 1), 0
        if (nhwc and not conv.lifting and k != 5 and conv.stride == 1 and conv.padding == 0
                and h.is_contiguous(memory_format=torch.channels_last) and fftconv.applicable_k(h.shape, cin, cout, k, h.device)):
            return "fftk", False, 0
        if nhwc and self._plain_5x5(conv) and winograd.applicable(h, cin, cout):
            m = winograd.tile_for(h)
            if last_before_tail and not winograd.sums_applicable(h, kt, m) and winograd.sums_applicable(h, kt, 2):
                m = 2
            return "wino", last_before_tail and winograd.sums_applicable(h, kt, m), m
        lift = self._lift_kernel(conv, bank, h) if nhwc else None
        if lift == "narrow":
            nxt = convs[i + 1] if i + 1 < len(convs) - 1 else None
            if nxt is not None and self._plain_5x5(nxt):
                if fftconv.lift_fused_applicable(h.shape, bank.shape, nxt.out_channels * nxt.num_group_elements, h.device):
                    return "lift_fused", False, 0
                if fftconv.grouped_applicable((h.shape[0], cout, h.shape[2] - k + 1, h.shape[3] - k + 1), cout, cout, h.device):
                    return "lift_grouped", False, 0
            return "lift", False, 0
        return ("lift_wide" if lift == "wide" else "lib"), False, 0

    def _forward_inference(self, x: torch.Tensor) -> torch.Tensor:
        convs, norms = self._layers()
        tail = convs[-1]
        nhwc = (self.out_channels * self.num_group_elements) % 4 == 0
        h = x.contiguous(memory_format=torch.channels_last) if nhwc else x
        pending = None
        for i, (conv, bn) in enumerate(zip(convs[:-1], norms)):
            bank, bias = self._folded(conv, bn)
            route, sums, m = self._route(i, h, bank, convs, nhwc)
            k, (H, W) = conv.kernel_size, h.shape[-2:]
            last_before_tail, shift = i == len(convs) - 2, None
            if route != "fft5" and isinstance(h, (fftconv.GroupedMap, fftconv.LiftedInput)):
                h = h.materialize()
            if route in ("fft5", "fftk", "wino"):
                in_bias, pending = pending, None
                sums_k = tail.kernel_size if sums else 0
                if route == "wino":
                    U = self._derived(conv, lambda: winograd.transform_filters(bank, m), "wino", m)
                    h = winograd.conv5x5(h, U, bias, relu=True, in_bias=in_bias, in_relu=in_bias is not None, sums_k=sums_k)
                else:
                    Bf = self._derived(conv, lambda: fftconv.spectra_for_k(bank), "fft")
                    if route == "fft5":
                        h = fftconv.conv5x5(h, Bf, bias, True, in_bias, in_bias is not None, sums_k=sums_k)
                    else:
                        h = fftconv.conv_kxk(h, Bf, k, bias, True, in_bias, in_bias is not None)
            else:
                if pending is not None:
                    ops.bias_relu_nhwc_(h, pending)
                    pending = None
                if route == "lift_fused":
                    operand = {}
                    form = fftconv.LiftedInput.form_operand()
                    if form is not None:
                        operand[form[1]] = self._derived(conv, lambda: form[2](bank), form[0])
                    h = fftconv.LiftedInput(h, bank, bias, True, **operand)
                elif route != "lib":
                    pack = ops.pack_lift_weights_wide if route == "lift_wide" else ops.pack_lift_weights
                    wpk = self._derived(conv, lambda: pack(bank), "lift")
                    if route == "lift_grouped":
                        h = fftconv.GroupedMap(ops.lift_conv_grouped(h, wpk, bias, True, k, k))
                    else:
                        h = (ops.lift_conv_wide if route == "lift_wide" else ops.lift_conv_nhwc)(h, wpk, bias, True, k, k)
                else:
                    h = F.conv2d(h, bank)
                    if last_before_tail:
                        shift = bias
                    elif nhwc and h.is_contiguous(memory_format=torch.channels_last):
                        pending = bias
                    else:
                        h = torch.relu_(h + bias[None, :, None, None])
            if sums:
                return window_sums_to_activations(h, tail, H - k + 1, W - k + 1)
            if last_before_tail:
                return conv_then_group_pool(h, tail, shift=shift, relu=shift is not None)
        raise AssertionError("unreachable: the network always has at least two convolutions")

    @staticmethod
    def _inner_bn(h: torch.Tensor, bn: nn.BatchNorm3d, E: int, conv_bias) -> torch.Tensor:
        Bn, C, H, W = h.shape
        Fd = C // E
        if bn.training or bn.running_mean is None:
            n = Bn * E * H * W
            s1 = h.sum(dim=(0, 2, 3), dtype=torch.float64).view(Fd, E).sum(1)
            s2 = (h * h).sum(dim=(0, 2, 3), dtype=torch.float64).view(Fd, E).sum(1)
            mean = s1 / n
            var = (s2 / n - mean * mean).clamp_min(0.0)
            with torch.no_grad():
                full_mean = mean if conv_bias is None else mean + conv_bias.double()
                update_running_stats(bn, full_mean, var * (n / max(n - 1, 1)))
            mean, var = mean.float(), var.float()
        else:
            mean = bn.running_mean if conv_bias is None else bn.running_mean - conv_bias
            var = bn.running_var
        scale = bn.weight * torch.rsqrt(var + bn.eps)
        shift = bn.bias - mean * scale
        return h * scale.repeat_interleave(E)[None, :, None, None] + shift.repeat_interleave(E)[None, :, None, None]

    def _forward_training(self, x: torch.Tensor) -> torch.Tensor:
        mods = list(self.eqv_network)
        convs = [m for m in mods if hasattr(m, "expanded_weights")]
        norms = [m for m in mods if isinstance(m, _InnerBatchNorm)]
        drops = [m for m in mods if isinstance(m, nn.Dropout)]
        E = self.num_group_elements
        h = x.contiguous(memory_format=torch.channels_last)
        tail = convs[-1]
        S = None
        epilogue_stats = os.environ.get("EQA_TRAIN_FUSED_BN", "1") != "0" and os.environ.get("EQA_TRAIN_EPILOGUE_STATS", "1") != "0"
        for li, (conv, bn, drop) in enumerate(zip(convs[:-1], norms, drops)):
            bank = conv.expanded_weights()
            part = None
            lift = self._lift_kernel(conv, bank, h, narrow_unchecked=True)
            if not conv.lifting and conv.kernel_size == 5 and winograd.applicable(h, bank.shape[1], bank.shape[0]):
                if (epilogue_stats and (bn.training or bn.running_mean is None) and winograd.Conv5x5Function.stats_supported(h, bank)):
                    h, part = winograd.Conv5x5Function.apply(h, bank, winograd.tile_for(h), True)
                else:
                    h = winograd.Conv5x5Function.apply(h, bank, winograd.tile_for(h))
            elif (not conv.lifting and conv.kernel_size != 5
                  and fftconv.applicable_k(h.shape, bank.shape[1], bank.shape[0], conv.kernel_size, h.device,
                                           h.is_contiguous(memory_format=torch.channels_last))):
                h = fftconv.ConvKxKFunction.apply(h, bank)
            elif lift == "narrow":
                if (epilogue_stats and (bn.training or bn.running_mean is None)
                        and ops.lift_conv_stats_supported(h.shape, conv.kernel_size, conv.kernel_size, bank.shape[0])):
                    h, part = LiftConvFunction.apply(h, bank, True)
                else:
                    h = LiftConvFunction.apply(h, bank)
# ... 66 lines not shown
```

equiadapt_amd/images/canonicalization_networks/fftconv.py:

```python
import math
import os
from typing import Optional

import torch

from equiadapt_amd import _lib, ops
from equiadapt_amd.ops import _timed

N, NH, OUT = 48, 25, 44
F = N * (NH - 2) + 2 * NH
ENABLED = os.environ.get("EQA_CONV5_FFT", "1") != "0"
MIN_TILES = int(os.environ.get("EQA_FFT_MIN_TILES", "32"))
TRAIN_FORWARD = os.environ.get("EQA_FFT_TRAIN", "1") != "0"
GEMM = os.environ.get("EQA_FFT_GEMM", "3m")
GEMM_PIECES = os.environ.get("EQA_FFT_GEMM_PIECES", "auto")
AUTO_MIN_CIN = int(os.environ.get("EQA_FFT_GEMM_AUTO_MIN_CIN", "128"))
AUTO_MIN_CIN_H3 = int(os.environ.get("EQA_FFT_GEMM_AUTO_MIN_CIN_H3", "64"))
DCMAX_SLOTS = 256
LAST_FORM = None


def f16_form_takes(cin: int, cout: int) -> bool:
    return cout % 128 == 0 and cin % 32 == 0


def gemm_form(cin: int, cout: int, bounded: bool = False) -> str:
    if GEMM_PIECES in ("f32", "9", "6"):
        return GEMM_PIECES
    if bounded and f16_form_takes(cin, cout) and (GEMM_PIECES == "h3" or cin >= AUTO_MIN_CIN_H3):
        return "h3"
    return "6" if cin >= AUTO_MIN_CIN and cout % 128 == 0 else "f32"


def f16_scale(t: torch.Tensor) -> float:
    mx = float(t.abs().max().item())
    ex = 14 - math.frexp(mx)[1] if 0.0 < mx < float("inf") else 0
    return math.ldexp(1.0, max(-100, min(100, ex)))


class Spectra3M:

    __slots__ = ("data", "cin", "cout", "_pieces", "_pieces_f16")

    def __init__(self, data: torch.Tensor, cin: int, cout: int):
        self.data, self.cin, self.cout, self._pieces, self._pieces_f16 = data, cin, cout, None, None

    def pieces_f16(self):
        if self._pieces_f16 is None:
            lib = _lib.load()
            scale = f16_scale(self.data)
            bh = torch.empty(lib.eqa_fft48k5_spectra3m_f16_bytes(self.cin, self.cout) // 2, dtype=torch.int16, device=self.data.device)
            with torch.cuda.device(self.data.device):
                _lib.check(lib.eqa_fft48k5_spectra3m_split_f16(self.data.data_ptr(), bh.data_ptr(), self.cin, self.cout, scale,
                                                               ops._stream()), "eqa_fft48k5_spectra3m_split_f16")
            self._pieces_f16 = (bh, scale)
        return self._pieces_f16

    def pieces(self) -> torch.Tensor:
        if self._pieces is None:
            lib = _lib.load()
            bp = torch.empty(lib.eqa_fft48k5_spectra3m_bf16_bytes(self.cin, self.cout) // 2, dtype=torch.int16, device=self.data.device)
            with torch.cuda.device(self.data.device):
                _lib.check(lib.eqa_fft48k5_spectra3m_split(self.data.data_ptr(), bp.data_ptr(), self.cin, self.cout,
                                                           ops._stream()), "eqa_fft48k5_spectra3m_split")
            self._pieces = bp
        return self._pieces


def gemm3m_supported(cin: int, cout: int) -> bool:
    return GEMM == "3m" and bool(_lib.load().eqa_fft48k5_cgemm3m_supported(cin, cout))


def filter_spectra3m(bank: torch.Tensor, correlate: bool = True) -> Spectra3M:
    lib = _lib.load()
    Cout, Cin = bank.shape[:2]
    if not (bank.is_cuda and bank.dtype == torch.float32 and lib.eqa_fft48k5_cgemm3m_supported(Cin, Cout)):
        raise RuntimeError("filter_spectra3m: fp32 device bank with Cin % 32 == 0 and Cout % 64 == 0 expected")
    B3 = torch.empty(lib.eqa_fft48k5_spectra3m_floats(Cin, Cout), dtype=torch.float32, device=bank.device)
    with torch.cuda.device(bank.device):
        _lib.check(lib.eqa_fft48k5_filter_spectra3m(bank.contiguous().data_ptr(), B3.data_ptr(), Cout, Cin, int(correlate),
                                                    ops._stream()), "eqa_fft48k5_filter_spectra3m")
    return Spectra3M(B3, Cin, Cout)
# ... 53 lines not shown

class GroupedMap:

    def __init__(self, data: torch.Tensor):
        assert data.dim() == 5 and data.shape[-1] == 16 and data.is_contiguous()
        self.data = data
        self.shape = torch.Size((data.shape[0], data.shape[1] * 16, data.shape[2], data.shape[3]))
        self.device, self.dtype, self.is_cuda = data.device, data.dtype, data.is_cuda

    def data_ptr(self) -> int:
        return self.data.data_ptr()

    def to_channels_last(self) -> torch.Tensor:
        n, g, h, w, _ = self.data.shape
        return self.data.permute(0, 1, 4, 2, 3).reshape(n, g * 16, h, w).contiguous(memory_format=torch.channels_last)

    materialize, is_contiguous = to_channels_last, _stands_for_channels_last


class LiftedInput:

    def __init__(self, x: torch.Tensor, bank: torch.Tensor, bias: Optional[torch.Tensor], relu: bool, pieces: Optional[torch.Tensor] = None,
                 pieces_f16=None):
        assert x.dim() == 4 and x.shape[1] == 3 and bank.shape[1:] == (3, 5, 5)
        self.x = x.contiguous(memory_format=torch.channels_last)
        self.bank = bank.contiguous(memory_format=torch.channels_last)
        self.bias, self.relu = (bias.contiguous() if bias is not None else None), bool(relu)
        self.shape = torch.Size((x.shape[0], bank.shape[0], x.shape[2] - 4, x.shape[3] - 4))
        self.device, self.dtype, self.is_cuda = x.device, x.dtype, x.is_cuda
        self._pieces = pieces
        self._pieces_f16 = pieces_f16

    @staticmethod
    def split_f16(bank: torch.Tensor):
        w = bank.float()
        C = w.shape[0]
        scale = f16_scale(w)
        wp = torch.zeros(C, 5, 8, 4, dtype=torch.float32, device=w.device)
        wp[:, :, 1:6, :3] = w.permute(0, 2, 3, 1) * scale
        chunks = wp.reshape(C, 5, 4, 8)
        h1 = chunks.half()
        h2 = (chunks - h1.float()).half()
        return torch.stack([h1, h2], dim=1).contiguous(), scale

    @staticmethod
    def split_bf16(bank: torch.Tensor) -> torch.Tensor:
        w = bank.float()
        C = w.shape[0]
        wp = torch.zeros(C, 5, 6, 4, dtype=torch.float32, device=w.device)
        wp[:, :, :5, :3] = w.permute(0, 2, 3, 1)
        chunks = torch.zeros(C, 16, 8, dtype=torch.float32, device=w.device)
        chunks[:, :15] = wp.reshape(C, 5, 3, 8).reshape(C, 15, 8)
        p0 = chunks.bfloat16()
        r1 = chunks - p0.float()
        p1 = r1.bfloat16()
        p2 = (r1 - p1.float()).bfloat16()
        assert torch.equal((p0.float() + p1.float()) + p2.float(), chunks), "the three bf16 pieces of a weight must add up exactly"
        return torch.stack([p0, p1, p2], dim=1).contiguous()

    @classmethod
    def form_operand(cls):
        return {"h2": ("lifth", "pieces_f16", cls.split_f16), "bf16x3": ("liftp", "pieces", cls.split_bf16)}.get(LIFT_FFT_FORM)

    def pieces_f16(self):
        if self._pieces_f16 is None:
            self._pieces_f16 = self.split_f16(self.bank)
        return self._pieces_f16

    def pieces(self) -> torch.Tensor:
        if self._pieces is None:
            self._pieces = self.split_bf16(self.bank)
        return self._pieces

    def spectra_into(self, V: torch.Tensor, B, st: int) -> Optional[torch.Tensor]:
        lib = _lib.load()
        nimg, C, H, W = self.shape
        dims = (nimg, H + 4, W + 4, C, st)
        px, pV = self.x.data_ptr(), V.data_ptr()
        p_b = self.bias.data_ptr() if self.bias is not None else None
        want_dc = self.relu and isinstance(B, Spectra3M) and gemm_form(B.cin, B.cout, True) == "h3"
        vbound = None
        if LIFT_FFT_FORM == "h2" and px % 16 == 0:
            wh, w_scale = self.pieces_f16()
            xbound = torch.empty(DCMAX_SLOTS, dtype=torch.float32, device=self.device)
            _lib.check(lib.eqa_absmax_slots(px, self.x.numel(), xbound.data_ptr(), st), "eqa_absmax_slots")
            if want_dc:
                vbound = torch.empty(DCMAX_SLOTS, dtype=torch.float32, device=self.device)
            _lib.check(lib.eqa_lift5_fft48k5_input_f16x2(px, wh.data_ptr(), w_scale, xbound.data_ptr(), DCMAX_SLOTS, p_b, int(self.relu), pV,
                                                         vbound.data_ptr() if want_dc else None, *dims), "eqa_lift5_fft48k5_input_f16x2")
        elif LIFT_FFT_FORM == "bf16x3":
            _lib.check(lib.eqa_lift5_fft48k5_input_bf16x3(px, self.pieces().data_ptr(), p_b, int(self.relu), pV, *dims),
                       "eqa_lift5_fft48k5_input_bf16x3")
        elif want_dc:
            vbound = torch.empty(DCMAX_SLOTS, dtype=torch.float32, device=self.device)
            _lib.check(lib.eqa_lift5_fft48k5_input_dcmax(px, self.bank.data_ptr(), p_b, 1, pV, vbound.data_ptr(), *dims),
                       "eqa_lift5_fft48k5_input_dcmax")
        else:
            _lib.check(lib.eqa_lift5_fft48k5_input(px, self.bank.data_ptr(), p_b, int(self.relu), pV, *dims), "eqa_lift5_fft48k5_input")
        return vbound

    def materialize(self) -> torch.Tensor:
        return ops.lift_conv_nhwc(self.x, ops.pack_lift_weights(self.bank), self.bias, self.relu, 5, 5)

    is_contiguous = _stands_for_channels_last


LIFT_FFT_FORM = os.environ.get("EQA_LIFT_FFT_FORM", "h2")
LIFT_FFT_FUSED_DEFAULT = "1"


def lift_fused_applicable(x_shape, bank_shape, cout_next: int, device) -> bool:
    if os.environ.get("EQA_LIFT_FFT_FUSED", LIFT_FFT_FUSED_DEFAULT) == "0" or len(x_shape) != 4:
        return False
    C, Cin, kh, kw = bank_shape
    if not _lib.load().eqa_lift5_fft48k5_input_supported(Cin, kh, kw, C):
        return False
    out_shape = (x_shape[0], C, x_shape[2] - 4, x_shape[3] - 4)
    return x_shape[2] >= 5 and x_shape[3] >= 5 and grouped_applicable(out_shape, C, cout_next, device)


def _tiles_pay(shape, cin: int, cout: int, max_waste: float) -> bool:
    if shape[1] != cin or (not gemm3m_supported(cin, cout) and ops.plane_gemm_supported(cin, cout)):
        return False
    H, W = shape[-2:]
    if H < 16 or W < 16 or shape[0] * tiles(H) * tiles(W) < MIN_TILES:
        return False
    return tiles(H) * OUT <= max_waste * (H - 4) and tiles(W) * OUT <= max_waste * (W - 4)


def grouped_applicable(shape, cin: int, cout: int, device, max_waste: float = 1.12) -> bool:
    if not (ENABLED and device.type == "cuda" and len(shape) == 4 and cin % 16 == 0):
        return False
    if os.environ.get("EQA_FFT_GROUPED", "1") == "0" or not _lib.load().eqa_fft48k5_input_grouped_supported(cin):
        return False
    return _tiles_pay(shape, cin, cout, max_waste)


def applicable(x: torch.Tensor, cin: int, cout: int, max_waste: float = 1.12) -> bool:
    if isinstance(x, (GroupedMap, LiftedInput)):
        return grouped_applicable(x.shape, cin, cout, x.device, max_waste)
    if not (ENABLED and x.is_cuda and x.dtype == torch.float32 and x.dim() == 4 and x.is_contiguous(memory_format=torch.channels_last)):
        return False
    return _tiles_pay(x.shape, cin, cout, max_waste)


def _order(C: int, G: int) -> torch.Tensor:
    p = torch.arange(2 * C)
    grp, r = p // (2 * G), p % (2 * G)
    return (r // G) * C + grp * G + r % G


def group_sizes(cin: int, cout: int):
    return (16 if cin % 16 == 0 else 1), 1


def filter_spectra(bank: torch.Tensor, groups=None, correlate: bool = True) -> torch.Tensor:
    Cout, Cin = bank.shape[:2]
    if groups is None and bank.is_cuda and bank.dtype == torch.float32:
        lib = _lib.load()
        B = torch.empty((F, 2 * Cin, 2 * Cout), dtype=torch.float32, device=bank.device)
        with torch.cuda.device(bank.device):
            _lib.check(lib.eqa_fft48k5_filter_spectra(bank.contiguous().data_ptr(), B.data_ptr(), Cout, Cin, int(correlate),
                                                      ops._stream()), "eqa_fft48k5_filter_spectra")
        return B
    assert correlate, "the host construction is the correlation (forward) form"
    gin, gout = groups if groups is not None else group_sizes(Cin, Cout)
    wp = torch.zeros(Cout, Cin, N, N, dtype=torch.float64, device=bank.device)
    wp[:, :, :5, :5] = bank.double()
    W = torch.fft.rfft2(wp).conj() / float(N * N)
    ky, kx = freq_index()
    W = W[:, :, ky.to(W.device), kx.to(W.device)]
    Wr = W.real.permute(2, 1, 0).contiguous()
    Wi = W.imag.permute(2, 1, 0).contiguous()
    top = torch.cat([Wr, Wi], dim=2)
    bot = torch.cat([-Wi, Wr], dim=2)
    full = torch.cat([top, bot], dim=1)
    full = full[:, _order(Cin, gin).to(bank.device)][:, :, _order(Cout, gout).to(bank.device)]
    return full.float().contiguous()


def spectra_buffer(M: int, width: int, device) -> torch.Tensor:
    pitch = _lib.load().eqa_fft48k5_tile_pitch(M)
    return torch.empty((F, pitch, width), dtype=torch.float32, device=device)[:, :M]


def output_stats_supported(nimg: int, OH: int, OW: int, cout: int) -> bool:
    return _lib.load().eqa_fft48k5_output_stats_rows(nimg, OH, OW, cout) > 0


KSIZES = (3, 5, 7, 9)


def _transform(name: str, k: int, *args) -> None:
    lib = _lib.load()
    if k == 5:
        _lib.check(getattr(lib, "eqa_fft48k5_" + name)(*args), "eqa_fft48k5_" + name)
    else:
        _lib.check(getattr(lib, "eqa_fft48_" + name)(*args[:-1], k, args[-1]), "eqa_fft48_" + name)


def _workspace(k: int, nimg: int, rows: int, out_cols: int, C: int, device) -> torch.Tensor:
    lib = _lib.load()
    nbytes = lib.eqa_fft48k5_workspace_bytes(nimg, rows, out_cols, C) if k == 5 else lib.eqa_fft48_workspace_bytes(nimg, rows, out_cols, C, k)
    return torch.empty(max(nbytes, 4) // 4, dtype=torch.float32, device=device)


def applicable_k(x_shape, cin: int, cout: int, k: int, device, channels_last: bool = True) -> bool:
    if not (ENABLED and k in KSIZES and k != 5 and device.type == "cuda" and channels_last and len(x_shape) == 4 and x_shape[1] == cin):
        return False
    if os.environ.get("EQA_FFT_ANYK", "1") == "0":
        return False
    nimg, _, H, W = x_shape
    if H < max(16, k) or W < max(16, k) or nimg * tiles_k(H, k) * tiles_k(W, k) < 8:
        return False
    oh, ow = H - k + 1, W - k + 1
    t = tiles_k(H, k) * tiles_k(W, k)
    fft_us = t * (F * 8 * (cin + cout) * 2.2 / 4.0e6 + F * 6 * cin * cout / 100e6)
    direct_us = oh * ow * k * k * 2 * cin * cout / 110e6
    return fft_us * 1.3 < direct_us


def spectra_for_k(bank: torch.Tensor, correlate: bool = True):
    k = bank.shape[-1]
    if k == 5:
        return spectra_for(bank, correlate)
    lib = _lib.load()
    Cout, Cin = bank.shape[:2]
    assert bank.is_cuda and bank.dtype == torch.float32 and bank.shape[-2] == k and lib.eqa_fft48_supported(k)
    st = ops._stream()
    with torch.cuda.device(bank.device):
        if gemm3m_supported(Cin, Cout):
            B3 = torch.empty(lib.eqa_fft48k5_spectra3m_floats(Cin, Cout), dtype=torch.float32, device=bank.device)
            _lib.check(lib.eqa_fft48_filter_spectra3m(bank.contiguous().data_ptr(), B3.data_ptr(), Cout, Cin, k, int(correlate), st),
                       "eqa_fft48_filter_spectra3m")
            return Spectra3M(B3, Cin, Cout)
        B = torch.empty((F, 2 * Cin, 2 * Cout), dtype=torch.float32, device=bank.device)
        _lib.check(lib.eqa_fft48_filter_spectra(bank.contiguous().data_ptr(), B.data_ptr(), Cout, Cin, k, int(correlate), st),
                   "eqa_fft48_filter_spectra")
        return B


def conv_kxk(x: torch.Tensor, B, k: int, bias: Optional[torch.Tensor], relu: bool, in_bias: Optional[torch.Tensor] = None,
             in_relu: bool = False, keep_V: Optional[list] = None, sums_k: int = 0, stats: Optional[list] = None) -> torch.Tensor:
    lib = _lib.load()
    nimg, Cin, H, W = x.shape
    if isinstance(B, Spectra3M):
        Cout = B.cout
        assert B.cin == Cin
    else:
        Cout = B.shape[2] // 2
        assert B.shape == (F, 2 * Cin, 2 * Cout)
    assert k == 5 or not (sums_k or stats is not None or isinstance(x, (GroupedMap, LiftedInput))), "k = 5 only"
    OH, OW = H - k + 1, W - k + 1
    TX = tiles_k(W, k)
    M = nimg * tiles_k(H, k) * TX
    dev = x.device
    st = ops._stream()
    V = spectra_buffer(M, 2 * Cin, dev)
    p_bias = bias.data_ptr() if bias is not None else None
    vbound = None
    with torch.cuda.device(dev):
        if isinstance(x, LiftedInput):
            assert in_bias is None and not in_relu
            with _timed("lift_fft_input"):
                vbound = x.spectra_into(V, B, st)
        else:
            T = _workspace(k, nimg, H, OW, Cin, dev)
            with _timed("fft_input"):
                _transform("input_grouped" if isinstance(x, GroupedMap) else "input", k, x.data_ptr(), T.data_ptr(), V.data_ptr(),
                           in_bias.data_ptr() if in_bias is not None else None, int(in_relu), nimg, H, W, Cin, st)
            del T
        with _timed("fft_gemm"):
            Mo = contract(V, B, M, vbound)
        if keep_V is not None:
            keep_V.append(V)
        del V
        T2 = _workspace(k, nimg, OH, OW, Cout, dev)
        if sums_k:
            S = torch.empty((nimg, Cout, sums_k, sums_k), dtype=torch.float64, device=dev)
            ws = torch.empty(nimg * OH * TX * Cout * (2 * sums_k - 1), dtype=torch.float32, device=dev)
            with _timed("fft_output_sums"):
                _lib.check(lib.eqa_fft48k5_output_sums(Mo.data_ptr(), T2.data_ptr(), p_bias, int(relu), S.data_ptr(), ws.data_ptr(),
                                                       nimg, OH, OW, Cout, sums_k, st), "eqa_fft48k5_output_sums")
            return S
        y = torch.empty((nimg, Cout, OH, OW), dtype=torch.float32, device=dev, memory_format=torch.channels_last)
        if stats is not None:
            assert bias is None and not relu
            part = torch.empty((lib.eqa_fft48k5_output_stats_rows(nimg, OH, OW, Cout), Cout, 2), dtype=torch.float64, device=dev)
            with _timed("fft_output"):
                _lib.check(lib.eqa_fft48k5_output_stats(Mo.data_ptr(), T2.data_ptr(), y.data_ptr(), part.data_ptr(), nimg, OH, OW, Cout, st),
                           "eqa_fft48k5_output_stats")
            stats.append(part)
            return y
        with _timed("fft_output"):
            _transform("output", k, Mo.data_ptr(), T2.data_ptr(), p_bias, int(relu), y.data_ptr(), nimg, OH, OW, Cout, st)
        return y


def conv5x5(x: torch.Tensor, B: torch.Tensor, bias: Optional[torch.Tensor], relu: bool,
            in_bias: Optional[torch.Tensor] = None, in_relu: bool = False, sums_k: int = 0,
            keep_V: Optional[list] = None, stats: Optional[list] = None) -> torch.Tensor:
    return conv_kxk(x, B, 5, bias, relu, in_bias, in_relu, keep_V, sums_k, stats)


def grad_spectra(dy: torch.Tensor, k: int = 5) -> torch.Tensor:
    nimg, Cout, OH, OW = dy.shape
    M = nimg * tiles_k(OH + k - 1, k) * tiles_k(OW + k - 1, k)
    T = _workspace(k, nimg, OH, OW, Cout, dy.device)
    G = spectra_buffer(M, 2 * Cout, dy.device)
    with torch.cuda.device(dy.device):
        _transform("grad_transform", k, dy.data_ptr(), T.data_ptr(), G.data_ptr(), nimg, OH, OW, Cout, ops._stream())
    return G


def filter_grad_k(V: torch.Tensor, dy: torch.Tensor, cin: int, k: int, G: Optional[torch.Tensor] = None) -> torch.Tensor:
    lib = _lib.load()
    nimg, Cout, OH, OW = dy.shape
    dev = dy.device
    M = V.shape[1]
    assert V.shape == (F, M, 2 * cin) and M == nimg * tiles_k(OH + k - 1, k) * tiles_k(OW + k - 1, k)
    st = ops._stream()
    if G is None:
        G = grad_spectra(dy, k)
    dbank = torch.empty((Cout, cin, k, k), dtype=torch.float32, device=dev)
    with torch.cuda.device(dev):
        packed = GEMM == "3m" and lib.eqa_fft48k5_wgrad3m_supported(cin, Cout) and os.environ.get("EQA_FFT_WGRAD3M", "1") != "0"
        if packed:
            D = torch.empty((F, cin, 2, Cout), dtype=torch.float32, device=dev)
            _lib.check(lib.eqa_fft48k5_wgrad3m(V.data_ptr(), G.data_ptr(), D.data_ptr(), M, cin, Cout, st), "eqa_fft48k5_wgrad3m")
        else:
            D = torch.bmm(V.transpose(1, 2), G)
        if k != 5:
            _lib.check(lib.eqa_fft48_filter_grad(D.data_ptr(), dbank.data_ptr(), Cout, cin, k, int(packed), st), "eqa_fft48_filter_grad")
        elif packed:
            _lib.check(lib.eqa_fft48k5_filter_grad3m(D.data_ptr(), dbank.data_ptr(), Cout, cin, st), "eqa_fft48k5_filter_grad3m")
        else:
            _lib.check(lib.eqa_fft48k5_filter_grad(D.data_ptr(), dbank.data_ptr(), Cout, cin, st), "eqa_fft48k5_filter_grad")
    return dbank


def filter_grad(V: torch.Tensor, dy: torch.Tensor, cin: int, G: Optional[torch.Tensor] = None) -> torch.Tensor:
    return filter_grad_k(V, dy, cin, 5, G)


def input_grad(dy: torch.Tensor, bank: torch.Tensor, G: Optional[torch.Tensor] = None) -> torch.Tensor:
    k = bank.shape[-1]
    nimg, Cout, OH, OW = dy.shape
    Cin = bank.shape[1]
    dev = dy.device
    if G is None:
        G = grad_spectra(dy, k)
    B2 = spectra_for_k(bank.detach().permute(1, 0, 2, 3).contiguous(), correlate=False)
    st = ops._stream()
    H, W = OH + k - 1, OW + k - 1
    dx = torch.empty((nimg, Cin, H, W), dtype=torch.float32, device=dev, memory_format=torch.channels_last)
    with torch.cuda.device(dev):
        Cg = contract(G, B2, G.shape[1])
        T2 = _workspace(k, nimg, N * tiles_k(H, k), OW, Cin, dev)
        _transform("input_grad", k, Cg.data_ptr(), T2.data_ptr(), dx.data_ptr(), nimg, H, W, Cin, st)
    return dx


grad_spectra_k, input_grad_k = grad_spectra, input_grad


class ConvKxKFunction(torch.autograd.Function):

    @staticmethod
    def forward(ctx, x, bank):
        keep: list = []
        k = bank.shape[-1]
        y = conv_kxk(x, spectra_for_k(bank.detach()), k, None, False, keep_V=keep)
        ctx.save_for_backward(bank, *keep)
        return y

    @staticmethod
    def backward(ctx, dy):
        bank, V = ctx.saved_tensors
        k = bank.shape[-1]
        dy = dy.contiguous(memory_format=torch.channels_last)
        G = grad_spectra_k(dy, k)
        dx = input_grad_k(dy, bank, G) if ctx.needs_input_grad[0] else None
        dbank = filter_grad_k(V, dy, bank.shape[1], k, G).to(bank.dtype) if ctx.needs_input_grad[1] else None
        return dx, dbank
```

equiadapt_amd/images/canonicalization_networks/pooling.py:

```python
import torch

from equiadapt_amd import ops


class _GroupPoolFn(torch.autograd.Function):
    @staticmethod
    def forward(ctx, feature_map: torch.Tensor) -> torch.Tensor:
        ctx.shape = tuple(feature_map.shape)
        act, _ = ops.group_pool_argmax(feature_map, want_index=False)
        return act

    @staticmethod
    def backward(ctx, grad_act: torch.Tensor):
        B, C, G, H, W = ctx.shape
        return (grad_act / float(C * H * W))[:, None, :, None, None].expand(B, C, G, H, W)


def group_pool(feature_map: torch.Tensor) -> torch.Tensor:
    if feature_map.dtype != torch.float32:
        return torch.mean(feature_map, dim=(1, 3, 4))
    return _GroupPoolFn.apply(feature_map)


def conv_then_group_pool(h: torch.Tensor, layer, scale=None, shift=None, relu: bool = False) -> torch.Tensor:
    k, E, O = layer.kernel_size, layer.num_group_elements, layer.out_channels
    B, _, H, W = h.shape
    S = ops.window_sums(h, k, scale, shift, relu)
    return window_sums_to_activations(S, layer, H, W)


def window_sums_to_activations(S: torch.Tensor, layer, H: int, W: int) -> torch.Tensor:
    k, O = layer.kernel_size, layer.out_channels
    weff = layer.mean_response_weights()
    scale = 1.0 / float(O * (H - k + 1) * (W - k + 1))
    if S.is_cuda and weff.shape[0] <= 16 and not torch.is_grad_enabled():
        from equiadapt_amd import ops

        return ops.window_sums_gemv(S.flatten(1), weff, scale, layer.mean_bias_value())
    act = S.flatten(1) @ weff.t() * scale
    if layer.bias is not None:
        mb = layer.mean_bias_value()
        act = act + (mb if isinstance(mb, float) else mb.to(act.device))
    return act.float()


class WindowSumsLinearFn(torch.autograd.Function):

    @staticmethod
    def forward(ctx, S, weff, scale):
        from equiadapt_amd import ops

        S, weff = S.contiguous(), weff.contiguous()
        ctx.save_for_backward(S, weff)
        ctx.scale = scale
        return ops.window_sums_gemv(S, weff, scale, 0.0)

    @staticmethod
    @torch.autograd.function.once_differentiable
    def backward(ctx, dact):
        from equiadapt_amd import ops

        S, weff = ctx.saved_tensors
        dS, dW = ops.window_sums_gemv_bwd(dact.float().contiguous(), weff, S, ctx.scale, ctx.needs_input_grad[0], ctx.needs_input_grad[1])
        return dS, dW, None


class WindowSumsFunction(torch.autograd.Function):

    @staticmethod
    def forward(ctx, x, k):
        from equiadapt_amd import ops

        ctx.k, ctx.shape = k, x.shape
        ctx.channels_last = x.is_contiguous(memory_format=torch.channels_last)
        return ops.window_sums(x, k)

    @staticmethod
    def backward(ctx, dS):
        k = ctx.k
        B, C, H, W = ctx.shape
        nb = k - 1
        dev = dS.device

        def classes(n):
            rep = torch.cat([torch.arange(nb), torch.tensor([nb]), torch.arange(n - nb, n)]).to(dev)
            u = torch.arange(k, device=dev)
            mask = ((u[None, :] <= rep[:, None]) & (rep[:, None] <= u[None, :] + (n - k))).to(dS.dtype)
            i = torch.arange(n, device=dev)
            idx = torch.where(i < nb, i, torch.where(i >= n - nb, i - (n - nb) + nb + 1, torch.full_like(i, nb)))
            return mask, idx

        rm, ty = classes(H)
        cm, tx = classes(W)
        if dS.is_cuda and dS.dtype == torch.float64 and B <= 65535 and H >= 2 * nb + 1 and W >= 2 * nb + 1:
            from equiadapt_amd import ops

            table = ops.window_grad_table(dS.contiguous(), H, W)
        else:
            table = torch.einsum("tu,bcuv,sv->btsc", rm, dS, cm).float().contiguous()
        if table.is_cuda and C % 4 == 0:
            from equiadapt_amd import _lib, ops

            g = torch.empty((B, H, W, C), dtype=torch.float32, device=dev)
            with torch.cuda.device(dev):
                st = _lib.load().eqa_window_sums_bwd_expand_nhwc(table.data_ptr(), g.data_ptr(), B, H, W, C, k, ops._stream())
            _lib.check(st, "eqa_window_sums_bwd_expand_nhwc")
        else:
            g = table[:, ty][:, :, tx]
        g = g.permute(0, 3, 1, 2)
        if not ctx.channels_last:
            g = g.contiguous()
        return g, None
```

equiadapt_amd/ops.py:

```python
from typing import Optional, Tuple

import torch

from equiadapt_amd import _lib


MAX_WINDOW_K = 10


def _stream() -> int:
    return _raw_stream(_current_device())


try:
    _raw_stream, _current_device = torch._C._cuda_getCurrentRawStream, torch._C._cuda_getDevice
except AttributeError:
    def _raw_stream(_dev):
        return torch.cuda.current_stream().cuda_stream

    def _current_device():
        return 0


class KernelTimer:

    active: "Optional[KernelTimer]" = None

    def __init__(self):
        self.events = {}

    def __enter__(self):
        KernelTimer.active = self
        return self

    def __exit__(self, *exc):
        KernelTimer.active = None

    def summary(self):
        torch.cuda.synchronize()
        return {k: (len(v), sum(a.elapsed_time(b) for a, b in v) / len(v)) for k, v in self.events.items()}


class _timed:
    def __init__(self, name: str):
        self.t = KernelTimer.active
        self.name = name

    def __enter__(self):
        if self.t is not None:
            self.a = torch.cuda.Event(enable_timing=True)
            self.b = torch.cuda.Event(enable_timing=True)
            self.a.record()

    def __exit__(self, *exc):
        if self.t is not None:
            self.b.record()
            self.t.events.setdefault(self.name, []).append((self.a, self.b))


def _need(t: torch.Tensor, name: str, dtype=torch.float32) -> torch.Tensor:
    if not isinstance(t, torch.Tensor):
        raise TypeError(f"{name} must be a torch.Tensor")
    if not t.is_cuda:
        raise RuntimeError(f"{name} is on {t.device}: equiadapt_amd runs on an MI355X (ROCm) device only, no CPU fallback")
    if t.dtype != dtype:
        raise TypeError(f"{name} must be {dtype}, got {t.dtype} (the hot path computes in fp32 like the reference)")
    return t if t.is_contiguous() else t.contiguous()


def _opt(t: Optional[torch.Tensor], name: str, dtype) -> Tuple[Optional[torch.Tensor], Optional[int]]:
    if t is None:
        return None, None
    t = _need(t, name, dtype)
    return t, t.data_ptr()


def group_action(
    src: torch.Tensor,
    gidx: Optional[torch.Tensor],
    theta: torch.Tensor,
    flags: Optional[torch.Tensor],
    chan_map: Optional[torch.Tensor],
    pad: int,
    out_hw: Tuple[int, int],
    top_left: Tuple[int, int],
    n_out: Optional[int] = None,
) -> torch.Tensor:
    lib = _lib.load()
# ... 210 lines not shown
        _lib.check(st, "eqa_window_sums_nhwc")
        return out
    x = _need(x, "x")
    with torch.cuda.device(x.device), _timed("window_sums"):
        st = lib.eqa_window_sums(x.data_ptr(), p_scale, p_shift, int(relu), out.data_ptr(), B, C, H, W, k, _stream())
    _lib.check(st, "eqa_window_sums")
    return out


def group_argmax(act: torch.Tensor) -> torch.Tensor:
    lib = _lib.load()
    act = _need(act.detach(), "group_activations")
    B, G = act.shape
    gidx = torch.empty((B,), dtype=torch.int32, device=act.device)
    with torch.cuda.device(act.device):
        st = lib.eqa_group_argmax(act.data_ptr(), gidx.data_ptr(), B, G, _stream())
    _lib.check(st, "eqa_group_argmax")
    return gidx


def so3_rotate(x: torch.Tensor, R: torch.Tensor, transpose: bool = False) -> torch.Tensor:
    lib = _lib.load()
    x = _need(x, "x")
    R = _need(R, "R")
    B, three, N = x.shape
    if three != 3 or tuple(R.shape) != (B, 3, 3):
        raise ValueError("so3_rotate expects x:(B,3,N) and R:(B,3,3)")
    y = torch.empty_like(x)
    with torch.cuda.device(x.device):
        st = lib.eqa_so3_rotate(x.data_ptr(), R.data_ptr(), y.data_ptr(), B, N, int(transpose), _stream())
    _lib.check(st, "eqa_so3_rotate")
    return y


def gram_schmidt(v: torch.Tensor) -> torch.Tensor:
    lib = _lib.load()
    v = _need(v, "vectors")
    if v.dim() != 3 or v.shape[1:] != (3, 3):
        raise ValueError("gram_schmidt expects (B,3,3)")
    out = torch.empty_like(v)
    with torch.cuda.device(v.device):
        st = lib.eqa_gram_schmidt(v.data_ptr(), out.data_ptr(), v.shape[0], _stream())
    _lib.check(st, "eqa_gram_schmidt")
    return out


def vnsmall_forward(x: torch.Tensor, params: torch.Tensor, k: int = 20, pooling: str = "mean") -> torch.Tensor:
    lib = _lib.load()
    x = _need(x, "point_cloud")
    params = _need(params, "params")
    B, three, N = x.shape
    if pooling not in ("mean", "max"):
        raise ValueError(f"Pooling type {pooling} not supported")
    if three != 3 or params.numel() != (1310 if pooling == "mean" else 1751):
        raise ValueError("vnsmall_forward expects x:(B,3,N) and 1310 (mean) / 1751 (max) packed parameters")
    out = torch.empty((B, 3, 3), dtype=torch.float32, device=x.device)
    ws = torch.empty((max(lib.eqa_vnsmall_workspace_bytes(B, N), 4) // 4,), dtype=torch.float32, device=x.device)
    with torch.cuda.device(x.device), _timed("vnsmall_fwd"):
        st = lib.eqa_vnsmall_fwd(x.data_ptr(), params.data_ptr(), out.data_ptr(), ws.data_ptr(), B, N, k, int(pooling == "max"), _stream())
    _lib.check(st, "eqa_vnsmall_fwd")
    return out


def vnsmall_canonicalize(x: torch.Tensor, params: torch.Tensor, k: int = 20, pooling: str = "mean"):
    lib = _lib.load()
    x = _need(x, "point_cloud")
    params = _need(params, "params")
    B, three, N = x.shape
    if pooling not in ("mean", "max"):
        raise ValueError(f"Pooling type {pooling} not supported")
    if three != 3 or params.numel() != (1310 if pooling == "mean" else 1751):
        raise ValueError("vnsmall_canonicalize expects x:(B,3,N) and 1310 (mean) / 1751 (max) packed parameters")
    vec = torch.empty((B, 3, 3), dtype=torch.float32, device=x.device)
    R = torch.empty((B, 3, 3), dtype=torch.float32, device=x.device)
    y = torch.empty_like(x)
    ws = torch.empty((max(lib.eqa_vnsmall_workspace_bytes(B, N), 4) // 4,), dtype=torch.float32, device=x.device)
    with torch.cuda.device(x.device), _timed("vnsmall_fwd"):
        st = lib.eqa_vnsmall_canonicalize(x.data_ptr(), params.data_ptr(), vec.data_ptr(), R.data_ptr(), y.data_ptr(), ws.data_ptr(),
                                          B, N, k, int(pooling == "max"), _stream())
    _lib.check(st, "eqa_vnsmall_canonicalize")
    return vec, R, y


def crop_resize_aa(x: torch.Tensor, tables, out_hw: Tuple[int, int]) -> torch.Tensor:
    lib = _lib.load()
    x = _need(x, "x")
    wx, x0, wy, y0, K, max_rows, x_begin, x_span = tables
    B, C, H, W = x.shape
    y = torch.empty((B, C, out_hw[0], out_hw[1]), dtype=torch.float32, device=x.device)
    with torch.cuda.device(x.device), _timed("crop_resize_aa"):
        st = lib.eqa_crop_resize_aa(x.data_ptr(), y.data_ptr(), wx.data_ptr(), x0.data_ptr(), wy.data_ptr(), y0.data_ptr(),
                                    B * C, H, W, out_hw[0], out_hw[1], K, max_rows, x_begin, x_span, _stream())
    _lib.check(st, "eqa_crop_resize_aa")
    return y


def mask_action_nearest(masks: torch.Tensor, eidx: torch.Tensor, rtheta: torch.Tensor, flags: Optional[torch.Tensor]) -> torch.Tensor:
    lib = _lib.load()
    masks = _need(masks, "masks", torch.uint8)
    eidx = _need(eidx, "eidx", torch.int32)
    rtheta = _need(rtheta, "rtheta")
    flags, p_flags = _opt(flags, "flags", torch.int32)
    n, H, W = masks.shape
    out = torch.empty_like(masks)
    with torch.cuda.device(masks.device), _timed("mask_action"):
        st = lib.eqa_mask_action_nearest(masks.data_ptr(), out.data_ptr(), eidx.data_ptr(), rtheta.data_ptr(), p_flags,
                                         rtheta.shape[0], n, H, W, _stream())
    _lib.check(st, "eqa_mask_action_nearest")
    return out


_plane_tables: dict = {}


def mask_action_nearest_planes(mask_list, eidx: torch.Tensor, rtheta: torch.Tensor, flags: Optional[torch.Tensor]) -> torch.Tensor:
    lib = _lib.load()
    eidx = _need(eidx, "eidx", torch.int32)
    rtheta = _need(rtheta, "rtheta")
    flags, p_flags = _opt(flags, "flags", torch.int32)
    masks = [_need(m, "masks", torch.uint8) for m in mask_list]
    H, W = masks[0].shape[-2:]
    ptrs = tuple(m.data_ptr() + k * H * W for m in masks for k in range(m.shape[0]))
    n = len(ptrs)
    dev = masks[0].device
    key = (ptrs, str(dev))
    table = _plane_tables.get(key)
    if table is None:
        if len(_plane_tables) >= 64:
            _plane_tables.clear()
        table = torch.tensor(ptrs, dtype=torch.int64).to(dev)
        _plane_tables[key] = table
    out = torch.empty((n, H, W), dtype=torch.uint8, device=dev)
    with torch.cuda.device(dev), _timed("mask_action"):
        st = lib.eqa_mask_action_nearest_planes(table.data_ptr(), out.data_ptr(), eidx.data_ptr(), rtheta.data_ptr(), p_flags,
                                                rtheta.shape[0], n, H, W, _stream())
    _lib.check(st, "eqa_mask_action_nearest_planes")
    return out


def boxes_action(boxes: torch.Tensor, img_of_box: torch.Tensor, rotation_deg: torch.Tensor, width: float,
                 flip_all: bool) -> Tuple[torch.Tensor, Optional[torch.Tensor]]:
    lib = _lib.load()
    boxes = _need(boxes, "boxes")
    img_of_box = _need(img_of_box, "img_of_box", torch.int32)
    rotation_deg = _need(rotation_deg, "rotation_deg")
    out = torch.empty_like(boxes)
    flipped = torch.empty_like(boxes) if flip_all else None
    with torch.cuda.device(boxes.device):
        st = lib.eqa_boxes_action(boxes.data_ptr(), img_of_box.data_ptr(), rotation_deg.data_ptr(),
                                  flipped.data_ptr() if flip_all else None, out.data_ptr(), boxes.shape[0], float(width),
                                  int(flip_all), _stream())
    _lib.check(st, "eqa_boxes_action")
    return out, flipped


def conv_s2_supported(cin: int, cout: int, k: int, pad: int, planar: bool) -> bool:
    return bool(_lib.load().eqa_conv_s2_supported(cin, cout, k, pad, int(planar)))


def pack_conv_s2_weights(w: torch.Tensor, planar: bool) -> torch.Tensor:
    Cout, Cin, K, _ = w.shape
    if planar:
        wp = torch.zeros(Cout, 4, K, K, dtype=w.dtype, device=w.device)
        wp[:, :Cin] = w
        return wp.permute(2, 3, 1, 0).reshape(K * K, 4, Cout // 16, 16).permute(0, 2, 1, 3).contiguous()
    t = w.permute(2, 3, 1, 0).reshape(K * K, Cin // 16, 4, 4, Cout // 16, 16)
    return t.permute(0, 1, 4, 2, 5, 3).contiguous()


def conv_s2(x: torch.Tensor, wp: torch.Tensor, bias: Optional[torch.Tensor], gelu: bool, cout: int, k: int, pad: int,
            planar: bool) -> torch.Tensor:
    lib = _lib.load()
    x, wp = _need(x, "x"), _need(wp, "wp")
    bias, p_bias = _opt(bias, "bias", torch.float32)
    if planar:
# ... 98 lines not shown
        st = lib.eqa_bn_act_fwd(z.data_ptr(), scale.data_ptr(), shift.data_ptr(), p_rs, y.data_ptr(), npix, C, act, _stream())
    _lib.check(st, "eqa_bn_act_fwd")
    return y


def bn_act_bwd(gy: torch.Tensor, z: torch.Tensor, scale: torch.Tensor, shift: torch.Tensor, mean: torch.Tensor, rstd: torch.Tensor,
               gamma: torch.Tensor, rowscale: Optional[torch.Tensor], act: int):
    lib = _lib.load()
    gy, z = _need(gy, "gy"), _need(z, "z")
    rowscale, p_rs = _opt(rowscale, "rowscale", torch.float32)
    npix, C = z.shape
    part = torch.empty((max(lib.eqa_bn_act_partial_blocks(npix), 1), C, 2), dtype=torch.float64, device=z.device)
    with torch.cuda.device(z.device), _timed("bn_act_bwd_reduce"):
        st = lib.eqa_bn_act_bwd_reduce(gy.data_ptr(), z.data_ptr(), scale.data_ptr(), shift.data_ptr(), mean.data_ptr(), rstd.data_ptr(), p_rs,
                                       part.data_ptr(), npix, C, act, _stream())
    _lib.check(st, "eqa_bn_act_bwd_reduce")
    coef = torch.empty((5, C), dtype=torch.float32, device=z.device)
    with torch.cuda.device(z.device):
        st = lib.eqa_bn_act_bwd_finalize(part.data_ptr(), npix, C, gamma.data_ptr(), rstd.data_ptr(), coef[0].data_ptr(), coef[1].data_ptr(),
                                         coef[2].data_ptr(), coef[3].data_ptr(), coef[4].data_ptr(), _stream())
    _lib.check(st, "eqa_bn_act_bwd_finalize")
    dgamma, dbeta, gscale, m1, m2 = coef[0], coef[1], coef[2], coef[3], coef[4]
    dz = torch.empty_like(z)
    with torch.cuda.device(z.device), _timed("bn_act_bwd_apply"):
        st = lib.eqa_bn_act_bwd_apply(gy.data_ptr(), z.data_ptr(), scale.data_ptr(), shift.data_ptr(), mean.data_ptr(), rstd.data_ptr(), p_rs,
                                      gscale.data_ptr(), m1.data_ptr(), m2.data_ptr(), dz.data_ptr(), npix, C, act, _stream())
    _lib.check(st, "eqa_bn_act_bwd_apply")
    return dz, dgamma, dbeta


def affine_relu_rows(h: torch.Tensor, scale: torch.Tensor, shift: torch.Tensor) -> torch.Tensor:
    lib = _lib.load()
    h, scale, shift = _need(h, "h"), _need(scale, "scale"), _need(shift, "shift")
    rows, D = h.shape
    z = torch.empty_like(h)
    with torch.cuda.device(h.device):
        st = lib.eqa_affine_relu_rows(h.data_ptr(), scale.data_ptr(), shift.data_ptr(), z.data_ptr(), rows, D, _stream())
    _lib.check(st, "eqa_affine_relu_rows")
    return z


def cosine_group_activations(v: torch.Tensor, ref: torch.Tensor, num_group: int, eps: float = 1e-8) -> torch.Tensor:
    lib = _lib.load()
    v, ref = _need(v, "vector_out"), _need(ref.reshape(-1), "reference_vector")
    R, V = v.shape
    if R % num_group or ref.numel() != V:
        raise ValueError("cosine_group_activations expects (G*B, V) embeddings and a (V) reference vector")
    B = R // num_group
    act = torch.empty((B, num_group), dtype=torch.float32, device=v.device)
    with torch.cuda.device(v.device):
        st = lib.eqa_cosine_group_activations(v.data_ptr(), ref.data_ptr(), act.data_ptr(), B, num_group, V, float(eps), _stream())
    _lib.check(st, "eqa_cosine_group_activations")
    return act


def bias_relu_nhwc_(x: torch.Tensor, bias: torch.Tensor) -> torch.Tensor:
    lib = _lib.load()
    if not (x.is_cuda and x.dtype == torch.float32 and x.is_contiguous(memory_format=torch.channels_last)):
        raise RuntimeError("bias_relu_nhwc_ expects a channels-last fp32 tensor on the device")
    bias = _need(bias, "bias")
    B, C, H, W = x.shape
    with torch.cuda.device(x.device), _timed("bias_relu"):
        st = lib.eqa_bias_relu_nhwc(x.data_ptr(), bias.data_ptr(), B * H * W, C, _stream())
    _lib.check(st, "eqa_bias_relu_nhwc")
    return x


def window_sums_gemv(S: torch.Tensor, weff: torch.Tensor, scale: float, shift) -> torch.Tensor:
    lib = _lib.load()
    S = _need(S, "S", torch.float64)
    weff = _need(weff, "weff", torch.float64)
    B, K = S.shape
    E = weff.shape[0]
    act = torch.empty((B, E), dtype=torch.float32, device=S.device)
    sh = shift if isinstance(shift, float) else 0.0
    with torch.cuda.device(S.device), _timed("sums_gemv"):
        st = lib.eqa_window_sums_gemv(S.data_ptr(), weff.data_ptr(), act.data_ptr(), B, K, E, float(scale), sh, _stream())
    _lib.check(st, "eqa_window_sums_gemv")
    if not isinstance(shift, float):
        act += shift.to(torch.float32)
    return act


def window_sums_gemv_bwd(dact: torch.Tensor, weff: torch.Tensor, S: torch.Tensor, scale: float, need_dS: bool, need_dW: bool):
    lib = _lib.load()
    dact = _need(dact, "dact")
    weff, S = _need(weff, "weff", torch.float64), _need(S, "S", torch.float64)
    B, K = S.shape
    E = weff.shape[0]
    dS = torch.empty_like(S) if need_dS else None
    dW = torch.empty_like(weff) if need_dW else None
    ws = torch.empty((max(lib.eqa_window_sums_gemv_bwd_workspace_bytes(K, E), 8) // 8,), dtype=torch.float64, device=S.device) if need_dW else None
    with torch.cuda.device(S.device), _timed("sums_gemv_bwd"):
        st = lib.eqa_window_sums_gemv_bwd(dact.data_ptr(), weff.data_ptr(), S.data_ptr(), dS.data_ptr() if need_dS else None,
                                          dW.data_ptr() if need_dW else None, ws.data_ptr() if need_dW else None, B, K, E, float(scale), _stream())
    _lib.check(st, "eqa_window_sums_gemv_bwd")
    return dS, dW


def window_grad_table(dS: torch.Tensor, H: int, W: int) -> torch.Tensor:
    lib = _lib.load()
    dS = _need(dS, "dS", torch.float64)
    B, C, k, _ = dS.shape
    T = 2 * (k - 1) + 1
    table = torch.empty((B, T, T, C), dtype=torch.float32, device=dS.device)
    with torch.cuda.device(dS.device), _timed("window_grad_table"):
        st = lib.eqa_window_grad_table(dS.data_ptr(), table.data_ptr(), B, C, H, W, k, _stream())
    _lib.check(st, "eqa_window_grad_table")
    return table


def plane_gemm_supported(cin: int, cout: int) -> bool:
    return bool(_lib.load().eqa_plane_gemm_supported(cin, cout))


def pack_plane_gemm_weights(U: torch.Tensor) -> torch.Tensor:
    P, Cin, Cout = U.shape
    t = U.float().reshape(P, Cin // 16, 2, 2, 4, Cout // 32, 32)
    return t.permute(0, 1, 5, 2, 3, 6, 4).contiguous()


def plane_gemm(V: torch.Tensor, Upk: torch.Tensor, M: torch.Tensor, tiles: int) -> None:
    lib = _lib.load()
    V, Upk, M = _need(V, "V"), _need(Upk, "Upk"), _need(M, "M")
    P, Cin = V.shape[1], V.shape[2]
    Cout = M.shape[2]
    with torch.cuda.device(V.device):
        st = lib.eqa_plane_gemm(V.data_ptr(), Upk.data_ptr(), M.data_ptr(), tiles, P, Cin, Cout, _stream())
    _lib.check(st, "eqa_plane_gemm")


def lift_conv_supported(cin: int, kh: int, kw: int, cout: int) -> bool:
    return kh in (3, 5) and 9 <= kw * cin <= 15 and cout % 16 == 0


def pack_lift_weights(bank: torch.Tensor) -> torch.Tensor:
    Cout, Cin, KH, KW = bank.shape
    R = KW * Cin
    rows = bank.permute(2, 3, 1, 0).reshape(KH, R, Cout)
    q = torch.arange(8, device=bank.device)
    first = rows[:, q]
    second = rows[:, (R - 8) + q].clone()
    second[:, : 16 - R] = 0
    return torch.stack([first, second], dim=2).reshape(KH * 8, 2, Cout).float().contiguous()


def lift_conv_nhwc(x: torch.Tensor, wpk: torch.Tensor, bias: Optional[torch.Tensor], relu: bool, kh: int, kw: int) -> torch.Tensor:
    lib = _lib.load()
    if not (x.is_cuda and x.dtype == torch.float32 and x.is_contiguous(memory_format=torch.channels_last)):
        raise RuntimeError("lift_conv_nhwc expects a channels-last fp32 tensor on the device")
    wpk = _need(wpk, "wpk")
    bias, p_bias = _opt(bias, "bias", torch.float32)
    B, Cin, H, W = x.shape
    Cout = wpk.shape[2]
    y = torch.empty((B, Cout, H - kh + 1, W - kw + 1), dtype=torch.float32, device=x.device, memory_format=torch.channels_last)
    with torch.cuda.device(x.device), _timed("lift_conv"):
        st = lib.eqa_lift_conv_nhwc(x.data_ptr(), wpk.data_ptr(), p_bias, int(relu), y.data_ptr(), B, H, W, Cin, kh, kw, Cout, _stream())
    _lib.check(st, "eqa_lift_conv_nhwc")
    return y


def lift_conv_wide_supported(cin: int, kh: int, kw: int, cout: int) -> bool:
    return bool(_lib.load().eqa_lift_conv_wide_supported(cin, kh, kw, cout))


def pack_lift_weights_wide(bank: torch.Tensor) -> torch.Tensor:
# ... 153 lines not shown
```

include/eqa_hip.h:

```cpp
#ifndef EQA_HIP_H
#define EQA_HIP_H

#include <stdint.h>

#ifdef __cplusplus
extern "C" {
#endif

#define EQA_OK 0
#define EQA_ERR_INVALID_ARG (-1)
#define EQA_ERR_LAUNCH (-2)
#define EQA_ERR_UNSUPPORTED (-3)

#define EQA_FLIP_SRC 1
#define EQA_FLIP_DST 2

#define EQA_ABI_VERSION 3
int eqa_abi_version(void);

int eqa_set_option(int key, int value);
int eqa_get_option(int key);

int eqa_canon_transform_fwd(const float* x, float* y, const int32_t* gidx, const float* theta,
                            const int32_t* flags, int num_elements, int B, int C, int H, int W, int pad,
                            void* stream);

int eqa_invert_action_fwd(const float* f, float* out, const int32_t* gidx, const float* theta,
                          const int32_t* flags, const int32_t* chan_map, int num_elements, int G, int B, int C,
                          int H, int W, void* stream);

int eqa_group_action_pair(const float* x, float* y, const float* theta_canon, const int32_t* flags_canon, int pad, int C,
                          const float* f, float* out, const float* theta_inv, const int32_t* flags_inv,
                          const int32_t* chan_map, int G, int Cf, const int32_t* gidx, int num_elements, int B, int H,
                          int W, void* stream);

int eqa_orbit_expand_fwd(const float* x, float* y, const float* theta, const int32_t* flags, int num_elements,
                         int B, int C, int S, int pad, void* stream);

int eqa_group_action_fwd(const float* src, float* dst, const int32_t* gidx, const float* theta,
                         const int32_t* flags, const int32_t* chan_map, int num_elements, int G, int n_out,
                         int B, int C, int H, int W, int pad, int OH, int OW, int top, int left, void* stream);
int eqa_group_action_fwd_hint(const float* src, float* dst, const int32_t* gidx, const float* theta, const int32_t* flags,
                              const int32_t* chan_map, int num_elements, int G, int n_out, int B, int C, int H, int W,
                              int pad, int OH, int OW, int top, int left, int max_window, void* stream);

int eqa_crop_resize_aa(const float* x, float* y, const float* wx, const int32_t* x0, const float* wy, const int32_t* y0,
                       int planes, int H, int W, int OH, int OW, int K, int max_rows, int x_begin, int x_span, void* stream);

int eqa_mask_action_nearest(const uint8_t* m, uint8_t* out, const int32_t* eidx, const float* rtheta, const int32_t* flags,
                            int num_elements, int n_masks, int H, int W, void* stream);
int eqa_mask_action_nearest_planes(const uint8_t* const* planes, uint8_t* out, const int32_t* eidx, const float* rtheta,
                                   const int32_t* flags, int num_elements, int n_masks, int H, int W, void* stream);

int eqa_boxes_action(const float* boxes, const int32_t* img_of_box, const float* rotation_deg, float* flipped, float* out,
                     int n, float width, int flip_all, void* stream);

int eqa_image_action_nearest(const float* x, float* out, const int32_t* eidx, const float* rtheta, const int32_t* flags,
                             int num_elements, int n_planes, int src_mod, int H, int W, int pad, int OH, int OW, int top,
                             int left, void* stream);

int64_t eqa_fold_edge_pad_workspace_bytes(int planes, int H, int W, int pad);
int eqa_fold_edge_pad(const float* gframe, float* gsrc, void* workspace, int planes, int H, int W, int pad, void* stream);
int eqa_group_action_bwd_tiles(int OH, int OW);
int eqa_group_action_bwd(const float* src, const float* grad_out, const int32_t* gidx, const float* theta,
                         const int32_t* flags, const int32_t* chan_map, float* grad_src, float* grad_angle_partial,
                         int num_elements, int G, int n_out, int B, int C, int H, int W, int pad, int OH, int OW,
                         int top, int left, void* stream);
int eqa_group_action_bwd_theta(const float* src, const float* grad_out, const int32_t* gidx, const float* theta,
                               const int32_t* flags, const int32_t* chan_map, float* grad_src, float* grad_theta_partial,
                               int num_elements, int G, int n_out, int B, int C, int H, int W, int pad, int OH, int OW,
                               int top, int left, void* stream);

int64_t eqa_group_pool_workspace_bytes(int B, int Cf, int G, int HW);
int eqa_group_pool_argmax(const float* feat, float* act, int32_t* gidx, void* workspace, int B, int Cf, int G,
                          int HW, void* stream);

int eqa_window_sums(const float* x, const float* scale, const float* shift, int relu, double* out, int B, int C, int H,
                    int W, int k, void* stream);

int eqa_conv_s2_supported(int Cin, int Cout, int K, int pad, int planar);
int eqa_conv_s2(const float* x, const float* wp, const float* bias, int gelu, float* y, int B, int Cin, int H, int W, int Cout, int K,
                int pad, int planar, void* stream);
int eqa_conv_s2_wgrad_supported(int Cin, int Cout, int K, int pad, int planar);
int64_t eqa_conv_s2_wgrad_workspace_bytes(int B, int Cin, int H, int W, int Cout, int K, int pad, int planar);
int eqa_conv_s2_wgrad(const float* x, const float* dz, float* dw, void* workspace, int B, int Cin, int H, int W, int Cout, int K, int pad,
                      int planar, void* stream);
int eqa_conv_s2_dgrad_supported(int Cin, int Cout, int K, int pad);
int eqa_conv_s2_dgrad(const float* dz, const float* wd, float* dx, int B, int Cin, int H, int W, int Cout, int K, int pad, void* stream);
int eqa_bn_act_fwd(const float* z, const float* scale, const float* shift, const float* rowscale, float* y, int64_t npix, int C, int act,
                   void* stream);
int64_t eqa_bn_act_partial_blocks(int64_t npix);
int eqa_bn_act_stats(const float* z, double* partial, int64_t npix, int C, void* stream);
int eqa_bn_act_finalize(const double* partial, int64_t npix, int C, const float* gamma, const float* beta, double eps, double momentum,
                        float* running_mean, float* running_var, float* scale, float* shift, float* mean, float* rstd, void* stream);
int eqa_bn_act_bwd_finalize(const double* partial, int64_t npix, int C, const float* gamma, const float* rstd, float* dgamma, float* dbeta,
                            float* gscale, float* m1, float* m2, void* stream);
int eqa_bn_act_bwd_reduce(const float* gy, const float* z, const float* scale, const float* shift, const float* mean, const float* rstd,
                          const float* rowscale, double* partial, int64_t npix, int C, int act, void* stream);
int eqa_bn_act_bwd_apply(const float* gy, const float* z, const float* scale, const float* shift, const float* mean, const float* rstd,
                         const float* rowscale, const float* gscale, const float* m1, const float* m2, float* dz, int64_t npix, int C,
                         int act, void* stream);
int eqa_affine_relu_rows(const float* h, const float* scale, const float* shift, float* z, int64_t rows, int D, void* stream);
int eqa_cosine_group_activations(const float* v, const float* ref, float* act, int B, int G, int V, float eps, void* stream);
int eqa_window_grad_table(const double* dS, float* table, int B, int C, int H, int W, int k, void* stream);
int64_t eqa_window_sums_gemv_bwd_workspace_bytes(int K, int E);
int eqa_window_sums_gemv_bwd(const float* dact, const double* Wm, const double* S, double* dS, double* dWm, void* workspace, int B, int K,
                             int E, double scale, void* stream);
int eqa_bias_relu_nhwc(float* x, const float* bias, int64_t n_pixels, int C, void* stream);
int64_t eqa_window_sums_nhwc_workspace_bytes(int B, int C, int H, int k);
int eqa_window_sums_nhwc(const float* x, const float* scale, const float* shift, int relu, double* out, void* workspace,
                         int B, int C, int H, int W, int k, void* stream);
int eqa_window_sums_bwd_expand_nhwc(const float* table, float* dx, int B, int H, int W, int C, int k, void* stream);

int64_t eqa_bn_partial_blocks(int64_t n_pixels);
int eqa_bn_stats_nhwc(const float* x, double* partial, int64_t n_pixels, int C, void* stream);
int eqa_bn_relu_dropout_nhwc(const float* x, const float* scale, const float* shift, float* y, int64_t n_pixels, int C,
                             float drop_p, uint32_t seed, void* stream);
int eqa_bn_bwd_reduce_nhwc(const float* gy, const float* y, const float* x, const float* mean, const float* rstd, float drop_p,
                           double* partial, int64_t n_pixels, int C, const float* scale, const float* shift, uint32_t seed,
                           void* stream);
int eqa_bn_bwd_apply_nhwc(const float* gy, const float* y, const float* x, const float* mean, const float* rstd, const float* a,
                          const float* b, const float* d, float drop_p, float* dx, int64_t n_pixels, int C, const float* scale,
                          const float* shift, uint32_t seed, void* stream);
int eqa_window_sums_nhwc_act(const float* x, const float* scale, const float* shift, int relu, float drop_p, uint32_t seed, double* out,
                             void* workspace, int B, int C, int H, int W, int k, void* stream);
int eqa_bn_bwd_reduce_nhwc_wsgrad(const float* table, const float* x, const float* mean, const float* rstd, float drop_p,
                                  double* partial, int B, int H, int W, int C, int k, const float* scale, const float* shift,
                                  uint32_t seed, void* stream);
int eqa_bn_bwd_apply_nhwc_wsgrad(const float* table, const float* x, const float* mean, const float* rstd, const float* a,
                                 const float* b, const float* d, float drop_p, float* dx, int B, int H, int W, int C, int k,
                                 const float* scale, const float* shift, uint32_t seed, void* stream);

int eqa_window_sums_gemv(const double* S, const double* Wm, float* act, int B, int K, int E, double scale, double shift,
                         void* stream);

int eqa_lift_conv_nhwc(const float* x, const float* wpk, const float* bias, int relu, float* y, int nimg, int H, int W,
                       int Cin, int KH, int KW, int Cout, void* stream);
int eqa_lift_conv_grouped(const float* x, const float* wpk, const float* bias, int relu, float* y, int nimg, int H, int W, int Cin,
                          int KH, int KW, int Cout, void* stream);
int eqa_lift_conv_wide_supported(int Cin, int KH, int KW, int Cout);
int64_t eqa_lift_conv_wide_weight_floats(int Cin, int KH, int KW, int Cout);
int eqa_lift_conv_wide(const float* x, const float* wpk, const float* bias, int relu, float* y, int nimg, int H, int W, int Cin,
                       int KH, int KW, int Cout, void* stream);
int64_t eqa_lift_conv_wide_wgrad_workspace_bytes(int Cin, int KH, int KW, int Cout);
int eqa_lift_conv_wide_wgrad(const float* x, const float* dy, void* workspace, float* dbank, int nimg, int H, int W, int Cin, int KH,
                             int KW, int Cout, void* stream);
int eqa_lift_conv_stats_rows(int nimg, int H, int W, int Cin, int KH, int KW, int Cout);
int eqa_lift_conv_nhwc_stats(const float* x, const float* wpk, float* y, double* partial, int nimg, int H, int W, int Cin, int KH,
                             int KW, int Cout, void* stream);

int eqa_lift_conv_wgrad_supported(int nimg, int H, int W, int Cin, int Cout, int KH, int KW);
int64_t eqa_lift_conv_wgrad_workspace_bytes(int nimg, int H, int W, int Cin, int Cout, int KH, int KW);
int eqa_lift_conv_wgrad_nhwc(const float* x, const float* dy, void* workspace, float* dbank, int nimg, int H, int W, int Cin,
                             int Cout, int KH, int KW, void* stream);

int eqa_plane_gemm_supported(int Cin, int Cout);
int eqa_plane_gemm(const float* V, const float* Upk, float* M, long long T, int P, int Cin, int Cout, void* stream);

int eqa_winograd_f2k5_input(const float* x, float* V, const float* in_bias, int in_relu, int nimg, int H, int W, int C,
                            void* stream);
int eqa_winograd_f2k5_output(const float* M, const float* bias, int relu, float* y, int nimg, int OH, int OW, int C,
                             void* stream);
int eqa_winograd_f4k5_input(const float* x, float* V, const float* in_bias, int in_relu, int nimg, int H, int W, int C,
                            void* stream);
int eqa_winograd_f4k5_output(const float* M, const float* bias, int relu, float* y, int nimg, int OH, int OW, int C,
                             void* stream);
int eqa_winograd_f2k5_input_padded(const float* x, float* V, int nimg, int H, int W, int C, int pad, void* stream);
int eqa_winograd_f4k5_input_padded(const float* x, float* V, int nimg, int H, int W, int C, int pad, void* stream);
int eqa_winograd_f2k5_output_adjoint(const float* dY, float* dM, int nimg, int OH, int OW, int C, void* stream);
int eqa_winograd_f4k5_output_adjoint(const float* dY, float* dM, int nimg, int OH, int OW, int C, void* stream);
int64_t eqa_winograd_f2k5_output_sums_workspace_bytes(int nimg, int OH, int C, int k_next);
int eqa_winograd_f2k5_output_sums(const float* M, const float* bias, int relu, double* S, void* workspace, int nimg,
                                  int OH, int OW, int C, int k_next, void* stream);
int eqa_winograd_f4k5_output_sums(const float* M, const float* bias, int relu, double* S, void* workspace, int nimg,
                                  int OH, int OW, int C, int k_next, void* stream);

int64_t eqa_fft48k5_tiles(int n);
int64_t eqa_fft48k5_tile_pitch(int64_t tiles);
int eqa_fft48k5_frequencies(void);
int eqa_fft48k5_filter_spectra(const float* bank, float* B, int Cout, int Cin, int correlate, void* stream);
int eqa_fft48k5_cgemm3m_supported(int Cin, int Cout);
int64_t eqa_fft48k5_spectra3m_floats(int Cin, int Cout);
int eqa_fft48k5_filter_spectra3m(const float* bank, float* B3, int Cout, int Cin, int correlate, void* stream);
int eqa_fft48k5_cgemm3m(const float* V, const float* B3, float* Mo, int64_t M, int Cin, int Cout, void* stream);
int64_t eqa_fft48k5_spectra3m_bf16_bytes(int Cin, int Cout);
int eqa_fft48k5_spectra3m_split(const float* B3, void* Bp, int Cin, int Cout, void* stream);
int eqa_fft48k5_cgemm3m_bf16x3(const float* V, const void* Bp, float* Mo, int64_t M, int Cin, int Cout, int terms, void* stream);
int64_t eqa_fft48k5_spectra3m_f16_bytes(int Cin, int Cout);
int eqa_fft48k5_spectra3m_split_f16(const float* B3, void* Bh, int Cin, int Cout, float b_scale, void* stream);
int eqa_fft48k5_cgemm3m_f16x2(const float* V, const void* Bh, float* Mo, int64_t M, int Cin, int Cout, const float* vbound, int nbound,
                              float b_scale, void* stream);
int eqa_fft48k5_wgrad3m_supported(int Cin, int Cout);
int eqa_fft48k5_wgrad3m(const float* V, const float* G, float* D, int64_t M, int Cin, int Cout, void* stream);
int eqa_fft48k5_filter_grad3m(const float* D, float* dbank, int Cout, int Cin, void* stream);
int eqa_fft48k5_group(int C, int side);
int64_t eqa_fft48k5_workspace_bytes(int nimg, int rows, int out_cols, int C);
int eqa_fft48k5_input(const float* x, float* T, float* V, const float* in_bias, int in_relu, int nimg, int H, int W, int C,
                      void* stream);
int eqa_fft48k5_input_grouped_supported(int C);
int eqa_fft48k5_input_grouped(const float* x, float* T, float* V, const float* in_bias, int in_relu, int nimg, int H, int W, int C,
                              void* stream);
int eqa_lift5_fft48k5_input_supported(int Cin, int KH, int KW, int Cout);
int eqa_lift5_fft48k5_input(const float* x, const float* bank, const float* bias, int relu, float* V, int nimg, int H0, int W0, int Cout,
                            void* stream);
#define EQA_LIFT5_DCMAX_SLOTS 256
int eqa_lift5_fft48k5_input_dcmax(const float* x, const float* bank, const float* bias, int relu, float* V, float* dcmax, int nimg, int H0,
                                  int W0, int Cout, void* stream);
int64_t eqa_lift5_pieces_f16_bytes(int Cout);
int eqa_absmax_slots(const float* x, int64_t n, float* slots, void* stream);
int eqa_lift5_fft48k5_input_f16x2(const float* x, const void* wpieces, float w_scale, const float* xbound, int nxbound, const float* bias,
                                  int relu, float* V, float* dcmax, int nimg, int H0, int W0, int Cout, void* stream);
int64_t eqa_lift5_pieces_bytes(int Cout);
int eqa_lift5_fft48k5_input_bf16x3(const float* x, const void* wpieces, const float* bias, int relu, float* V, int nimg, int H0, int W0,
                                   int Cout, void* stream);
int eqa_fft48k5_output(const float* Mo, float* T2, const float* bias, int relu, float* y, int nimg, int OH, int OW, int C,
                       void* stream);
int64_t eqa_fft48k5_output_stats_rows(int nimg, int OH, int OW, int C);
int eqa_fft48k5_output_stats(const float* Mo, float* T2, float* y, double* partial, int nimg, int OH, int OW, int C, void* stream);
int eqa_fft48k5_grad_transform(const float* dy, float* T, float* G, int nimg, int OH, int OW, int C, void* stream);
int eqa_fft48k5_filter_grad(const float* D, float* dbank, int Cout, int Cin, void* stream);
int eqa_fft48k5_input_grad(const float* Cg, float* T2, float* dx, int nimg, int H, int W, int C, void* stream);
int eqa_fft48k5_output_sums(const float* Mo, float* T2, const float* bias, int relu, double* S, void* workspace, int nimg,
                            int OH, int OW, int C, int k_next, void* stream);

int eqa_fft48_supported(int ksize);
int64_t eqa_fft48_tiles(int n, int ksize);
int64_t eqa_fft48_workspace_bytes(int nimg, int rows, int out_cols, int C, int ksize);
int eqa_fft48_filter_spectra(const float* bank, float* B, int Cout, int Cin, int ksize, int correlate, void* stream);
int eqa_fft48_filter_spectra3m(const float* bank, float* B3, int Cout, int Cin, int ksize, int correlate, void* stream);
int eqa_fft48_input(const float* x, float* T, float* V, const float* in_bias, int in_relu, int nimg, int H, int W, int C, int ksize,
                    void* stream);
int eqa_fft48_grad_transform(const float* dy, float* T, float* G, int nimg, int OH, int OW, int C, int ksize, void* stream);
int eqa_fft48_output(const float* Mo, float* T2, const float* bias, int relu, float* y, int nimg, int OH, int OW, int C, int ksize,
                     void* stream);
int eqa_fft48_input_grad(const float* Cg, float* T2, float* dx, int nimg, int H, int W, int C, int ksize, void* stream);
int eqa_fft48_filter_grad(const float* D, float* dbank, int Cout, int Cin, int ksize, int packed, void* stream);

int eqa_group_argmax(const float* act, int32_t* gidx, int B, int G, void* stream);

int eqa_so3_rotate(const float* x, const float* R, float* y, int B, int N, int transpose, void* stream);

#define EQA_VNSMALL_PARAMS 1310
#define EQA_VNSMALL_PARAMS_MAX 1751
int64_t eqa_vnsmall_workspace_bytes(int B, int N);
int eqa_vnsmall_fwd(const float* x, const float* params, float* out, void* workspace, int B, int N, int k, int pooling,
                    void* stream);
int eqa_vnsmall_canonicalize(const float* x, const float* params, float* vectors, float* R, float* y, void* workspace, int B, int N,
                             int k, int pooling, void* stream);

int eqa_vn_blocks(int N);
int eqa_vn_knn(const float* x, int32_t* idx, int B, int N, int k, void* stream);
int eqa_vn_convpos_stats(const float* x, const int32_t* idx, const float* Wf, float* partial, int B, int N, int k, void* stream);
int eqa_vn_convpos_fwd(const float* x, const int32_t* idx, const float* Wf, const float* Wd, const float* scale, const float* shift,
                       float* pooled, int B, int N, int k, void* stream);
int eqa_vn_convpos_bwd_reduce(const float* x, const int32_t* idx, const float* Wf, const float* Wd, const float* scale,
                              const float* shift, const float* mean, const float* rstd, const float* gpool, float* partial, int B,
                              int N, int k, void* stream);
int eqa_vn_convpos_bwd_apply(const float* x, const int32_t* idx, const float* Wf, const float* Wd, const float* scale,
                             const float* shift, const float* mean, const float* rstd, const float* m1, const float* m2,
                             const float* gpool, float* partial, int B, int N, int k, void* stream);

int eqa_vn_tail_blocks(int N);
int eqa_vn_tail_partial_floats(int pass);
int eqa_vn_tail_pass(int pass, const float* pooled, const float* weights, const float* stat, const float* red, const float* mask,
                     const float* gout, float* partial, float* g_pooled, int B, int N, void* stream);
int eqa_vn_bn_finalize(const float* partial, int nblk, int stride, int C, long long M, const float* gamma, const float* beta,
                       float* running_mean, float* running_var, long long* num_batches_tracked, float momentum, float eps, float* stat,
                       void* stream);
int eqa_vn_bn_bwd_finalize(const float* partial, int nblk, int stride, int C, long long M, float* grads, float* red, void* stream);

int eqa_gram_schmidt(const float* v, float* out, int B, void* stream);
int eqa_gram_schmidt_bwd(const float* v, const float* grad_out, float* grad_v, int B, void* stream);

int eqa_modified_gram_schmidt(const float* v, float* out, int B, void* stream);
int eqa_rigid_rows(const float* x, const float* R, const float* t, float* out, int M, int mode, void* stream);

#ifdef __cplusplus
}
#endif
#endif
```

Baseline: 70460 images/s.

## Fuse crop-resize with NHWC output and absmax, defer window-sum finalize into GEMV

```diff
diff --git a/equiadapt_amd/_lib.py b/equiadapt_amd/_lib.py
--- a/equiadapt_amd/_lib.py
+++ b/equiadapt_amd/_lib.py
@@ -31,6 +31,8 @@
     "eqa_group_action_fwd": (_int, [_vp, _vp, _vp, _vp, _vp, _vp] + [_int] * 12 + [_vp]),
     "eqa_group_action_fwd_hint": (_int, [_vp, _vp, _vp, _vp, _vp, _vp] + [_int] * 13 + [_vp]),
     "eqa_crop_resize_aa": (_int, [_vp] * 6 + [_int] * 9 + [_vp]),
+    "eqa_crop_resize_aa_nhwc_slots": (ctypes.c_int64, [_int] * 10),
+    "eqa_crop_resize_aa_nhwc_absmax": (_int, [_vp] * 6 + [_int] * 10 + [_vp, ctypes.c_int64, _vp]),
     "eqa_mask_action_nearest": (_int, [_vp] * 5 + [_int] * 4 + [_vp]),
     "eqa_mask_action_nearest_planes": (_int, [_vp] * 5 + [_int] * 4 + [_vp]),
     "eqa_boxes_action": (_int, [_vp] * 5 + [_int, ctypes.c_float, _int, _vp]),
@@ -126,6 +128,10 @@
     "eqa_fft48k5_output_stats_rows": (ctypes.c_int64, [_int] * 4),
     "eqa_fft48k5_output_stats": (_int, [_vp, _vp, _vp, _vp] + [_int] * 4 + [_vp]),
     "eqa_fft48k5_output_sums": (_int, [_vp, _vp, _vp, _int, _vp, _vp] + [_int] * 5 + [_vp]),
+    "eqa_fft48k5_output_pieces": (_int, [_vp, _vp, _vp, _int, _vp] + [_int] * 5 + [_vp, _vp, _vp]),
+    "eqa_window_sums_nhwc_finalize": (_int, [_vp, _vp] + [_int] * 5 + [_vp]),
+    "eqa_window_sums_finalize_gemv_supported": (_int, [_int] * 4),
+    "eqa_window_sums_finalize_gemv": (_int, [_vp, _vp, _vp] + [_int] * 6 + [ctypes.c_double, ctypes.c_double, _vp]),
     "eqa_fft48_supported": (_int, [_int]),
     "eqa_fft48_tiles": (ctypes.c_int64, [_int, _int]),
     "eqa_fft48_workspace_bytes": (ctypes.c_int64, [_int] * 5),
diff --git a/equiadapt_amd/csrc/crop_resize.hip b/equiadapt_amd/csrc/crop_resize.hip
--- a/equiadapt_amd/csrc/crop_resize.hip
+++ b/equiadapt_amd/csrc/crop_resize.hip
@@ -174,6 +174,139 @@
 #undef EQA_AA_PF_LOAD
 }
 
+constexpr int kAaPixTrips = 6;
+
+struct __attribute__((packed, aligned(4))) aa_pix3 { float r, g, b; };
+
+template <int K, int BAND, int NL>
+__global__ __launch_bounds__(kThreads, (NL > 5 && K > 5) ? 2 : 3) void crop_resize_aa_nhwc_absmax_kernel(
+    const float* __restrict__ x, float* __restrict__ y, const float* __restrict__ wx, const int32_t* __restrict__ x0,
+    const float* __restrict__ wy, const int32_t* __restrict__ y0, int nimg, int H, int W, int OH, int OW, int cap_rows, int xb, int xl,
+    int pitch, float* __restrict__ slots) {
+  extern __shared__ __attribute__((aligned(16))) float aa_tmp[];
+  __shared__ float red[kThreads / 64];
+  float* rows = aa_tmp;
+  float* tmp = aa_tmp + (size_t)cap_rows * xl;
+  float* tabw = tmp + (size_t)cap_rows * OW;
+  int* taby = reinterpret_cast<int*>(tabw + BAND * K);
+  const int r0 = blockIdx.y * BAND, r1 = min(r0 + BAND, OH);
+  const int nband = r1 - r0;
+  const int img0 = (int)(blockIdx.z * kXcd + blockIdx.x), img_step = (int)(gridDim.z * kXcd);
+  const int rows_par = kThreads / OW;
+  const int ox = threadIdx.x % OW, rsub = threadIdx.x / OW;
+  const int xs_g = x0[ox];
+  float wv[K];
+  int xo[K];
+#pragma unroll
+  for (int j = 0; j < K; ++j) {
+    wv[j] = wx[ox * K + j];
+    xo[j] = min(xs_g - xb + j, xl - 1);
+  }
+  if ((int)threadIdx.x < nband * K) tabw[threadIdx.x] = wy[r0 * K + threadIdx.x];
+  const int ybeg = y0[r0];
+  if ((int)threadIdx.x < nband) taby[threadIdx.x] = y0[r0 + threadIdx.x] - ybeg;
+  const int yend = min(y0[r1 - 1] + K, H);
+  const int nrows = min(yend - ybeg, cap_rows);
+  const int nq = xl >> 2;
+  const int tq = threadIdx.x & 63, tr = threadIdx.x >> 6;
+  const bool prefetch = nq <= 64 && nrows <= 4 * NL;
+  const size_t plane_sz = (size_t)H * W;
+  const float* src0 = x + (size_t)ybeg * W + xb;
+  const int npix = nband * OW;
+  int qrow[kAaPixTrips], qcol[kAaPixTrips];
+#pragma unroll
+  for (int i = 0; i < kAaPixTrips; ++i) {
+    qrow[i] = __builtin_amdgcn_readfirstlane((i * kThreads) / OW);
+    qcol[i] = __builtin_amdgcn_readfirstlane((i * kThreads) % OW);
+  }
+  typedef float aa_f4 __attribute__((ext_vector_type(4)));
+  aa_f4 v[NL];
+#define EQA_AA_PF_LOAD(plane_)                                                                                          \
+  do {                                                                                                                  \
+    const float* src_ = src0 + (size_t)(plane_) * plane_sz;                                                             \
+    _Pragma("unroll") for (int k = 0; k < NL; ++k)                                                           \
+      v[k] = *reinterpret_cast<const aa_f4*>(src_ + (size_t)min(tr + 4 * k, nrows - 1) * W + 4 * min(tq, nq - 1));     \
+  } while (0)
+  __builtin_amdgcn_s_waitcnt(0x0070);
+  if (prefetch && img0 < nimg) EQA_AA_PF_LOAD((size_t)img0 * 3);
+  float amax = 0.0f;
+  for (int img = img0; img < nimg; img += img_step) {
+    float out[3][kAaPixTrips];
+#pragma unroll
+    for (int c = 0; c < 3; ++c) {
+      const size_t plane = (size_t)img * 3 + c;
+      if (prefetch) {
+        if (tq < nq) {
+#pragma unroll
+          for (int k = 0; k < NL; ++k)
+            if (tr + 4 * k < nrows) *reinterpret_cast<aa_f4*>(rows + (tr + 4 * k) * xl + 4 * tq) = v[k];
+        }
+        if (c < 2) EQA_AA_PF_LOAD(plane + 1);
+        else if (img + img_step < nimg) EQA_AA_PF_LOAD((size_t)(img + img_step) * 3);
+      } else {
+        const float* src = src0 + plane * plane_sz;
+        for (int q = tq; q < nq; q += 64)
+          for (int rb = tr; rb < nrows; rb += 4) *reinterpret_cast<aa_f4*>(rows + rb * xl + 4 * q) = *reinterpret_cast<const aa_f4*>(src + (size_t)rb * W + 4 * q);
+      }
+      __syncthreads();
+      if (rsub < rows_par) {
+        for (int ry0 = rsub; ry0 < nrows; ry0 += 4 * rows_par) {
+          float acc[4] = {0.0f, 0.0f, 0.0f, 0.0f};
+#pragma unroll
+          for (int u = 0; u < 4; ++u) {
+            const float* row = rows + min(ry0 + u * rows_par, nrows - 1) * xl;
+#pragma unroll
+            for (int j = 0; j < K; ++j)
+              acc[u] += wv[j] * row[xo[j]];
+          }
+#pragma unroll
+          for (int u = 0; u < 4; ++u)
+            if (ry0 + u * rows_par < nrows) tmp[(ry0 + u * rows_par) * OW + ox] = acc[u];
+        }
+      }
+      __syncthreads();
+#pragma unroll
+      for (int i = 0; i < kAaPixTrips; ++i) {
+        if (i * kThreads < npix) {
+          const bool wrap = ox + qcol[i] >= OW;
+          const int r = min(rsub + qrow[i] + (wrap ? 1 : 0), nband - 1), oxx = ox + qcol[i] - (wrap ? OW : 0);
+          const int ys = taby[r];
+          float acc = 0.0f;
+#pragma unroll
+          for (int j = 0; j < K; ++j)
+            acc += tabw[r * K + j] * tmp[min(ys + j, nrows - 1) * OW + oxx];
+          out[c][i] = acc;
+        } else {
+          out[c][i] = 0.0f;
+        }
+      }
+      __syncthreads();
+    }
+    float* dst = y + ((size_t)img * OH + r0) * OW * pitch;
+#pragma unroll
+    for (int i = 0; i < kAaPixTrips; ++i) {
+      const int idx = (int)threadIdx.x + i * kThreads;
+      if (idx < npix) {
+        amax = fmaxf(fmaxf(amax, fabsf(out[0][i])), fmaxf(fabsf(out[1][i]), fabsf(out[2][i])));
+        if (pitch == 4) {
+          const aa_f4 p = {out[0][i], out[1][i], out[2][i], 0.0f};
+          *reinterpret_cast<aa_f4*>(dst + (size_t)idx * 4) = p;
+        } else {
+          const aa_pix3 p = {out[0][i], out[1][i], out[2][i]};
+          *reinterpret_cast<aa_pix3*>(dst + (size_t)idx * 3) = p;
+        }
+      }
+    }
+  }
+#undef EQA_AA_PF_LOAD
+#pragma unroll
+  for (int o = 32; o > 0; o >>= 1) amax = fmaxf(amax, __shfl_xor(amax, o));
+  if ((threadIdx.x & 63) == 0) red[threadIdx.x >> 6] = amax;
+  __syncthreads();
+  if (threadIdx.x == 0)
+    slots[((size_t)blockIdx.z * gridDim.y + blockIdx.y) * gridDim.x + blockIdx.x] = fmaxf(fmaxf(red[0], red[1]), fmaxf(red[2], red[3]));
+}
+
 __global__ __launch_bounds__(kThreads) void crop_resize_aa_wide_kernel(const float* __restrict__ x, float* __restrict__ y,
                                                                       const float* __restrict__ wx, const int32_t* __restrict__ x0,
                                                                       const float* __restrict__ wy, const int32_t* __restrict__ y0,
@@ -352,6 +485,41 @@
     }
     __syncthreads();
   }
+}
+
+
+struct AaStagedPlan {
+  int band, cap_rows, xb, xl, nbands, groups;
+  size_t lds;
+  bool few;
+};
+
+bool aa_staged_plan(int units, int W, int OH, int OW, int K, int max_rows, int x_begin, int x_span, AaStagedPlan& p) {
+  static const bool staged_off = [] { const char* e = getenv("EQA_AA_STAGED"); return e && e[0] == '0'; }();
+  if (staged_off || K > EQA_AA_WIDE_MIN_K || (W & 3) != 0 || x_span <= 0 || x_begin < 0 || x_begin + x_span > W) return false;
+  p.xb = x_begin & ~3;
+  p.xl = std::min(W, (x_begin + x_span + 3) & ~3) - p.xb;
+  static const int band_env = [] { const char* e = getenv("EQA_AA_BAND"); return e ? atoi(e) : 0; }();
+  int band = band_env == 16 ? 16 : (band_env == 8 ? 8 : (OH >= 64 ? 16 : 8));
+  auto staged_lds = [&](int bnd) { return ((size_t)(bnd / kAaBand) * max_rows * (p.xl + OW) + bnd * (EQA_AA_WIDE_MIN_K + 1)) * sizeof(float); };
+  if (band == 16 && band_env != 16 && (staged_lds(16) > 64 * 1024 || 16 * K > kThreads)) band = 8;
+  p.band = band;
+  p.cap_rows = (band / kAaBand) * max_rows;
+  p.lds = staged_lds(band);
+  if (p.lds > 64 * 1024 || band * K > kThreads) return false;
+  static const int per_cu = [] { const char* e = getenv("EQA_AA_BLOCKS_PER_CU"); return e ? std::max(1, atoi(e)) : 12; }();
+  p.nbands = (OH + band - 1) / band;
+  p.groups = std::max(1, (std::min(units, (256 * per_cu + p.nbands - 1) / p.nbands) + kXcd - 1) / kXcd);
+  p.few = p.cap_rows <= 20;
+  return true;
+}
+
+bool aa_nhwc_plan(int nimg, int W, int OH, int OW, int K, int max_rows, int x_begin, int x_span, int pitch, AaStagedPlan& p) {
+  static const int per_cu = [] { const char* e = getenv("EQA_AA_NHWC_BLOCKS_PER_CU"); return e ? std::max(1, atoi(e)) : 0; }();
+  if ((pitch != 3 && pitch != 4) || nimg <= 0 || OH <= 0 || OW <= 0 || K <= 0 || max_rows <= 0) return false;
+  if (!aa_staged_plan(nimg, W, OH, OW, K, max_rows, x_begin, x_span, p)) return false;
+  if (per_cu) p.groups = std::max(1, (std::min(nimg, (256 * per_cu + p.nbands - 1) / p.nbands) + kXcd - 1) / kXcd);
+  return OW <= kThreads && p.band * OW <= kAaPixTrips * kThreads && p.lds + 64 <= 64 * 1024 && p.groups <= 65535 && p.nbands <= 65535;
 }
 
 }
@@ -386,45 +554,65 @@
       return launch_status();
     }
   }
-  static const bool staged_off = [] { const char* e = getenv("EQA_AA_STAGED"); return e && e[0] == '0'; }();
-  if (!staged_off && K <= EQA_AA_WIDE_MIN_K && (W & 3) == 0 && (((uintptr_t)x) & 15) == 0 && x_span > 0 && x_begin >= 0 &&
-      x_begin + x_span <= W) {
-    const int xb = x_begin & ~3, xl = std::min(W, (x_begin + x_span + 3) & ~3) - xb;
-    static const int band_env = [] { const char* e = getenv("EQA_AA_BAND"); return e ? atoi(e) : 0; }();
-    int band = band_env == 16 ? 16 : (band_env == 8 ? 8 : (OH >= 64 ? 16 : 8));
-    auto staged_lds = [&](int bnd) { return ((size_t)(bnd / kAaBand) * max_rows * (xl + OW) + bnd * (EQA_AA_WIDE_MIN_K + 1)) * sizeof(float); };
-    if (band == 16 && band_env != 16 && (staged_lds(16) > 64 * 1024 || 16 * K > kThreads)) band = 8;
-    const int cap_rows = (band / kAaBand) * max_rows;
-    const size_t lds3 = staged_lds(band);
-    if (lds3 <= 64 * 1024 && band * K <= kThreads) {
-      static const int per_cu = [] { const char* e = getenv("EQA_AA_BLOCKS_PER_CU"); return e ? std::max(1, atoi(e)) : 12; }();
-      const int nbands = (OH + band - 1) / band;
-      const int groups = std::max(1, (std::min(planes, (256 * per_cu + nbands - 1) / nbands) + kXcd - 1) / kXcd);
-      const bool few = cap_rows <= 20;
+  AaStagedPlan p;
+  if ((((uintptr_t)x) & 15) == 0 && aa_staged_plan(planes, W, OH, OW, K, max_rows, x_begin, x_span, p)) {
 #define EQA_AA_STAGED(K_)                                                                                                              \
   case K_:                                                                                                                             \
-    if (band == 16)                                                                                                                    \
-      hipLaunchKernelGGL((crop_resize_aa_staged_kernel<K_, 16, 10>), dim3(kXcd, nbands, groups), dim3(kThreads), lds3, (hipStream_t)stream, x, \
-                         y, wx, x0, wy, y0, planes, H, W, OH, OW, cap_rows, xb, xl);                                                   \
-    else if (few)                                                                                                                      \
-      hipLaunchKernelGGL((crop_resize_aa_staged_kernel<K_, 8, 5>), dim3(kXcd, nbands, groups), dim3(kThreads), lds3, (hipStream_t)stream, x,  \
-                         y, wx, x0, wy, y0, planes, H, W, OH, OW, cap_rows, xb, xl);                                                   \
+    if (p.band == 16)                                                                                                                  \
+      hipLaunchKernelGGL((crop_resize_aa_staged_kernel<K_, 16, 10>), dim3(kXcd, p.nbands, p.groups), dim3(kThreads), p.lds, (hipStream_t)stream, x, \
+                         y, wx, x0, wy, y0, planes, H, W, OH, OW, p.cap_rows, p.xb, p.xl);                                             \
+    else if (p.few)                                                                                                                    \
+      hipLaunchKernelGGL((crop_resize_aa_staged_kernel<K_, 8, 5>), dim3(kXcd, p.nbands, p.groups), dim3(kThreads), p.lds, (hipStream_t)stream, x,  \
+                         y, wx, x0, wy, y0, planes, H, W, OH, OW, p.cap_rows, p.xb, p.xl);                                             \
     else                                                                                                                               \
-      hipLaunchKernelGGL((crop_resize_aa_staged_kernel<K_, 8, 10>), dim3(kXcd, nbands, groups), dim3(kThreads), lds3, (hipStream_t)stream, x, \
-                         y, wx, x0, wy, y0, planes, H, W, OH, OW, cap_rows, xb, xl);                                                   \
+      hipLaunchKernelGGL((crop_resize_aa_staged_kernel<K_, 8, 10>), dim3(kXcd, p.nbands, p.groups), dim3(kThreads), p.lds, (hipStream_t)stream, x, \
+                         y, wx, x0, wy, y0, planes, H, W, OH, OW, p.cap_rows, p.xb, p.xl);                                             \
     break
-      switch (K) {
-        EQA_AA_STAGED(1); EQA_AA_STAGED(2); EQA_AA_STAGED(3); EQA_AA_STAGED(4); EQA_AA_STAGED(5); EQA_AA_STAGED(6); EQA_AA_STAGED(7);
-        EQA_AA_STAGED(8);
-        default: return EQA_ERR_UNSUPPORTED;
-      }
+    switch (K) {
+      EQA_AA_STAGED(1); EQA_AA_STAGED(2); EQA_AA_STAGED(3); EQA_AA_STAGED(4); EQA_AA_STAGED(5); EQA_AA_STAGED(6); EQA_AA_STAGED(7);
+      EQA_AA_STAGED(8);
+      default: return EQA_ERR_UNSUPPORTED;
+    }
 #undef EQA_AA_STAGED
-      return launch_status();
-    }
+    return launch_status();
   }
   hipLaunchKernelGGL(crop_resize_aa_kernel, grid, dim3(kThreads), lds, (hipStream_t)stream, x, y, wx, x0, wy, y0, H, W, OH, OW, K,
                      max_rows);
   return launch_status();
 }
 
-}
+int64_t eqa_crop_resize_aa_nhwc_slots(int nimg, int H, int W, int OH, int OW, int K, int max_rows, int x_begin, int x_span, int pitch) {
+  AaStagedPlan p;
+  if (H <= 0 || W <= 0 || !aa_nhwc_plan(nimg, W, OH, OW, K, max_rows, x_begin, x_span, pitch, p)) return 0;
+  return (int64_t)kXcd * p.nbands * p.groups;
+}
+
+int eqa_crop_resize_aa_nhwc_absmax(const float* x, float* y, const float* wx, const int32_t* x0, const float* wy, const int32_t* y0,
+                                   int nimg, int H, int W, int OH, int OW, int K, int max_rows, int x_begin, int x_span, int pitch,
+                                   float* slots, int64_t nslots, void* stream) {
+  if (!x || !y || !wx || !x0 || !wy || !y0 || !slots || nimg <= 0 || H <= 0 || W <= 0 || OH <= 0 || OW <= 0 || K <= 0 || max_rows <= 0)
+    return EQA_ERR_INVALID_ARG;
+  AaStagedPlan p;
+  if ((((uintptr_t)x | (uintptr_t)y) & 15) != 0 || !aa_nhwc_plan(nimg, W, OH, OW, K, max_rows, x_begin, x_span, pitch, p)) return EQA_ERR_UNSUPPORTED;
+  if (nslots != (int64_t)kXcd * p.nbands * p.groups) return EQA_ERR_INVALID_ARG;
+#define EQA_AA_NHWC(K_)                                                                                                                 \
+  case K_:                                                                                                                             \
+    if (p.band == 16)                                                                                                                  \
+      hipLaunchKernelGGL((crop_resize_aa_nhwc_absmax_kernel<K_, 16, 10>), dim3(kXcd, p.nbands, p.groups), dim3(kThreads), p.lds, (hipStream_t)stream, \
+                         x, y, wx, x0, wy, y0, nimg, H, W, OH, OW, p.cap_rows, p.xb, p.xl, pitch, slots);                              \
+    else if (p.few)                                                                                                                    \
+      hipLaunchKernelGGL((crop_resize_aa_nhwc_absmax_kernel<K_, 8, 5>), dim3(kXcd, p.nbands, p.groups), dim3(kThreads), p.lds, (hipStream_t)stream, \
+                         x, y, wx, x0, wy, y0, nimg, H, W, OH, OW, p.cap_rows, p.xb, p.xl, pitch, slots);                              \
+    else                                                                                                                               \
+      hipLaunchKernelGGL((crop_resize_aa_nhwc_absmax_kernel<K_, 8, 10>), dim3(kXcd, p.nbands, p.groups), dim3(kThreads), p.lds, (hipStream_t)stream, \
+                         x, y, wx, x0, wy, y0, nimg, H, W, OH, OW, p.cap_rows, p.xb, p.xl, pitch, slots);                              \
+    break
+  switch (K) {
+    EQA_AA_NHWC(1); EQA_AA_NHWC(2); EQA_AA_NHWC(3); EQA_AA_NHWC(4); EQA_AA_NHWC(5); EQA_AA_NHWC(6); EQA_AA_NHWC(7); EQA_AA_NHWC(8);
+    default: return EQA_ERR_UNSUPPORTED;
+  }
+#undef EQA_AA_NHWC
+  return launch_status();
+}
+
+}
diff --git a/equiadapt_amd/csrc/fftconv.hip b/equiadapt_amd/csrc/fftconv.hip
--- a/equiadapt_amd/csrc/fftconv.hip
+++ b/equiadapt_amd/csrc/fftconv.hip
@@ -1324,11 +1324,12 @@
   return rc != EQA_OK ? rc : launch_status();
 }
 
-int eqa_fft48k5_output_sums(const float* Mo, float* T2, const float* bias, int relu, double* S, void* workspace, int nimg,
-                            int OH, int OW, int C, int k_next, void* stream) {
-  if (!Mo || !T2 || !S || !workspace || nimg < 0 || OH <= 0 || OW <= 0 || C <= 0 || k_next <= 0) return EQA_ERR_INVALID_ARG;
+static int fft_output_pieces(const float* Mo, float* T2, const float* bias, int relu, void* workspace, int nimg, int OH, int OW, int C,
+                             int k_next, void* stream, int* nseg, int* sub) {
+  if (!Mo || !T2 || !workspace || nimg < 0 || OH <= 0 || OW <= 0 || C <= 0 || k_next <= 0) return EQA_ERR_INVALID_ARG;
   const int nb = k_next - 1;
   if ((nb != 4 && nb != 2) || OH < 2 * nb + 1 || OW < 2 * nb + 1 || k_next > kMaxWinK || nimg > 65535) return EQA_ERR_UNSUPPORTED;
+  *nseg = *sub = 0;
   if (nimg == 0) return EQA_OK;
   hipStream_t st = (hipStream_t)stream;
   float* part = (float*)workspace;
@@ -1336,10 +1337,25 @@
   const int rc = nb == 4 ? fft_output_impl<4>(Mo, T2, bias, relu, part, nimg, OH, OW, C, st, &fused)
                          : fft_output_impl<2>(Mo, T2, bias, relu, part, nimg, OH, OW, C, st, &fused);
   if (rc != EQA_OK) return rc;
-  const int sub = fused ? (OW + kFftO - 1) / kFftO : 1;
+  *sub = fused ? (OW + kFftO - 1) / kFftO : 1;
   const int per_row = fused == 3 ? kPipeCons / 64 : fused;
-  const int nseg = fused ? 2 * nb + per_row * ((OH + kFftO - 1) / kFftO) : OH;
-  return eqa::launch_window_sums_nhwc_finalize(part, S, nimg, C, k_next, nseg * sub, st, sub);
+  *nseg = (fused ? 2 * nb + per_row * ((OH + kFftO - 1) / kFftO) : OH) * *sub;
+  return launch_status();
+}
+
+int eqa_fft48k5_output_sums(const float* Mo, float* T2, const float* bias, int relu, double* S, void* workspace, int nimg,
+                            int OH, int OW, int C, int k_next, void* stream) {
+  if (!S) return EQA_ERR_INVALID_ARG;
+  int nseg = 0, sub = 0;
+  const int rc = fft_output_pieces(Mo, T2, bias, relu, workspace, nimg, OH, OW, C, k_next, stream, &nseg, &sub);
+  if (rc != EQA_OK || nimg == 0) return rc;
+  return eqa::launch_window_sums_nhwc_finalize((const float*)workspace, S, nimg, C, k_next, nseg, (hipStream_t)stream, sub);
+}
+
+int eqa_fft48k5_output_pieces(const float* Mo, float* T2, const float* bias, int relu, void* workspace, int nimg, int OH, int OW, int C,
+                              int k_next, int* nseg, int* sub, void* stream) {
+  if (!nseg || !sub) return EQA_ERR_INVALID_ARG;
+  return fft_output_pieces(Mo, T2, bias, relu, workspace, nimg, OH, OW, C, k_next, stream, nseg, sub);
 }
 
 }
diff --git a/equiadapt_amd/csrc/lift_fft.hip b/equiadapt_amd/csrc/lift_fft.hip
--- a/equiadapt_amd/csrc/lift_fft.hip
+++ b/equiadapt_amd/csrc/lift_fft.hip
@@ -194,7 +194,13 @@
   float x_scale = 1.0f, out_scale = 1.0f;
   if constexpr (H2) {
     float mx = 0.0f;
-    for (int t = lane; t < nxbound; t += 64) mx = fmaxf(mx, xbound[t]);
+    for (int t = lane; t < nxbound; t += 8 * 64) {
+      float s[8];
+#pragma unroll
+      for (int u = 0; u < 8; ++u) s[u] = xbound[min(t + 64 * u, nxbound - 1)];
+#pragma unroll
+      for (int u = 0; u < 8; ++u) mx = fmaxf(mx, s[u]);
+    }
 #pragma unroll
     for (int o = 32; o > 0; o >>= 1) mx = fmaxf(mx, __shfl_xor(mx, o));
     int ex = 0;
diff --git a/equiadapt_amd/csrc/pooling.hip b/equiadapt_amd/csrc/pooling.hip
--- a/equiadapt_amd/csrc/pooling.hip
+++ b/equiadapt_amd/csrc/pooling.hip
@@ -449,6 +449,122 @@
   }
 }
 
+
+constexpr int kTailThreads = 1024;
+constexpr int kTailBatch = 16;
+constexpr int kTailCols = 9;
+
+template <int KW>
+__global__ __launch_bounds__(kTailThreads) void window_sums_finalize_gemv_kernel(const float* __restrict__ part, const double* __restrict__ Wm,
+                                                                                 float* __restrict__ act, int C, int nseg, int sub, int E,
+                                                                                 double scale, double shift) {
+  constexpr int NB = KW - 1, NVAL = 1 + 2 * NB, KK = KW * KW;
+  extern __shared__ __attribute__((aligned(16))) double tail_smem[];
+  __shared__ double s_red[4][kGemvMaxE];
+  double* s_S = tail_smem;
+  double* s_tot = s_S + (size_t)C * KK;
+  float* s_brd = reinterpret_cast<float*>(s_tot + (size_t)C * NVAL);
+  const int b = blockIdx.x;
+  const int run = C * NVAL;
+  const size_t seg_stride = (size_t)run;
+  const float* base = part + (size_t)b * nseg * seg_stride;
+  for (int e = threadIdx.x; e < run; e += kTailThreads) {
+    const float* q = base + e;
+    float vb[2 * NB][2], va[kTailBatch], vc[kTailBatch];
+#pragma unroll
+    for (int i = 0; i < 2 * NB; ++i)
+#pragma unroll
+      for (int t = 0; t < 2; ++t) vb[i][t] = t < sub ? q[(size_t)(i * sub + t) * seg_stride] : 0.0f;
+    int s = 2 * NB * sub;
+    auto request = [&](float (&v)[kTailBatch], int s0) {
+#pragma unroll
+      for (int j = 0; j < kTailBatch; ++j) v[j] = s0 + j < nseg ? q[(size_t)(s0 + j) * seg_stride] : 0.0f;
+    };
+    double acc = 0.0;
+    auto add = [&](const float (&v)[kTailBatch], int s0) {
+#pragma unroll
+      for (int j = 0; j < kTailBatch; ++j)
+        if (s0 + j < nseg) acc += (double)v[j];
+    };
+    request(va, s);
+#pragma unroll
+    for (int i = 0; i < 2 * NB; ++i) {
+      const float w = sub == 2 ? vb[i][0] + vb[i][1] : vb[i][0];
+      s_brd[(size_t)i * run + e] = w;
+      acc += (double)w;
+    }
+    while (s < nseg) {
+      if (s + kTailBatch < nseg) request(vc, s + kTailBatch);
+      add(va, s);
+      s += kTailBatch;
+      if (s >= nseg) break;
+      if (s + kTailBatch < nseg) request(va, s + kTailBatch);
+      add(vc, s);
+      s += kTailBatch;
+    }
+    s_tot[e] = acc;
+  }
+  __syncthreads();
+  for (int it = threadIdx.x; it < C * KK; it += kTailThreads) {
+    const int c = it / KK, uv = it - c * KK;
+    const int u = uv / KW, v = uv - u * KW;
+    float p0[NB], pc[NB][NB];
+    double tc[NB];
+#pragma unroll
+    for (int r = 0; r < NB; ++r) p0[r] = s_brd[(size_t)(r < u ? r : NB + r) * run + c * NVAL];
+#pragma unroll
+    for (int j = 0; j < NB; ++j) {
+      const int i = j < v ? 1 + j : 1 + NB + j;
+      tc[j] = s_tot[c * NVAL + i];
+#pragma unroll
+      for (int r = 0; r < NB; ++r) pc[j][r] = s_brd[(size_t)(r < u ? r : NB + r) * run + c * NVAL + i];
+    }
+    double a = s_tot[c * NVAL];
+#pragma unroll
+    for (int r = 0; r < NB; ++r) a -= (double)p0[r];
+#pragma unroll
+    for (int j = 0; j < NB; ++j) {
+      a -= tc[j];
+#pragma unroll
+      for (int r = 0; r < NB; ++r) a += (double)pc[j][r];
+    }
+    s_S[it] = a;
+  }
+  __syncthreads();
+  const int lane = threadIdx.x & 63, pw = threadIdx.x >> 6;
+  const int lw = pw & 3, eg = pw >> 2;
+  const int lt = lw * 64 + lane;
+  const int K = C * KK;
+  double acc[4] = {0.0, 0.0, 0.0, 0.0};
+  for (int j = lt; j < K; j += kTailCols * 256) {
+    double sv[kTailCols], w[kTailCols][4];
+#pragma unroll
+    for (int u = 0; u < kTailCols; ++u) {
+      const bool in = j + u * 256 < K;
+      sv[u] = in ? s_S[j + u * 256] : 0.0;
+#pragma unroll
+      for (int m = 0; m < 4; ++m) w[u][m] = (in && eg + 4 * m < E) ? Wm[(size_t)(eg + 4 * m) * K + j + u * 256] : 0.0;
+    }
+#pragma unroll
+    for (int u = 0; u < kTailCols; ++u)
+#pragma unroll
+      for (int m = 0; m < 4; ++m)
+        if (eg + 4 * m < E && j + u * 256 < K) acc[m] += sv[u] * w[u][m];
+  }
+#pragma unroll
+  for (int m = 0; m < 4; ++m) {
+    double v = acc[m];
+#pragma unroll
+    for (int off = 32; off > 0; off >>= 1) v += __shfl_down(v, off, 64);
+    if (lane == 0) s_red[lw][eg + 4 * m] = v;
+  }
+  __syncthreads();
+  if ((int)threadIdx.x < E) {
+    double v = 0.0;
+    for (int w = 0; w < 4; ++w) v += s_red[w][threadIdx.x];
+    act[(size_t)b * E + threadIdx.x] = (float)(v * scale + shift);
+  }
+}
 
 __global__ __launch_bounds__(kThreads) void affine_relu_rows_kernel(const float* __restrict__ h, const float* __restrict__ scale,
                                                                    const float* __restrict__ shift, float* __restrict__ z, size_t n_vec,
@@ -661,6 +777,41 @@
   return launch_status();
 }
 
+int eqa_window_sums_nhwc_finalize(const float* part, double* S, int B, int C, int k, int nseg, int sub, void* stream) {
+  if (B < 0 || C <= 0 || k <= 0 || sub <= 0 || nseg < 2 * (k - 1) * sub + 1) return EQA_ERR_INVALID_ARG;
+  if (k > kMaxWinK) return EQA_ERR_UNSUPPORTED;
+  if (B == 0) return EQA_OK;
+  if (!part || !S) return EQA_ERR_INVALID_ARG;
+  return eqa::launch_window_sums_nhwc_finalize(part, S, B, C, k, nseg, (hipStream_t)stream, sub);
+}
+
+static size_t tail_lds_bytes(int C, int k) {
+  const size_t nval = 2 * k - 1;
+  return (size_t)C * k * k * 8 + (size_t)C * nval * 8 + (size_t)2 * (k - 1) * C * nval * 4;
+}
+
+int eqa_window_sums_finalize_gemv_supported(int C, int k, int sub, int E) {
+  return (k == 3 || k == 5) && C > 0 && sub >= 1 && sub <= 2 && E >= 1 && E <= kGemvMaxE && tail_lds_bytes(C, k) <= 158 * 1024 ? 1 : 0;
+}
+
+int eqa_window_sums_finalize_gemv(const float* part, const double* Wm, float* act, int B, int C, int k, int nseg, int sub, int E,
+                                  double scale, double shift, void* stream) {
+  if (B < 0 || C <= 0 || k <= 0 || sub <= 0 || E <= 0 || nseg < 2 * (k - 1) * sub + 1) return EQA_ERR_INVALID_ARG;
+  if (!eqa_window_sums_finalize_gemv_supported(C, k, sub, E)) return EQA_ERR_UNSUPPORTED;
+  if (B == 0) return EQA_OK;
+  if (!part || !Wm || !act) return EQA_ERR_INVALID_ARG;
+  const int lds = (int)tail_lds_bytes(C, k);
+  const void* kern = k == 5 ? (const void*)window_sums_finalize_gemv_kernel<5> : (const void*)window_sums_finalize_gemv_kernel<3>;
+  if (!allow_dynamic_lds(kern, lds)) return EQA_ERR_UNSUPPORTED;
+  if (k == 5)
+    hipLaunchKernelGGL(window_sums_finalize_gemv_kernel<5>, dim3(B), dim3(kTailThreads), lds, (hipStream_t)stream, part, Wm, act, C, nseg, sub,
+                       E, scale, shift);
+  else
+    hipLaunchKernelGGL(window_sums_finalize_gemv_kernel<3>, dim3(B), dim3(kTailThreads), lds, (hipStream_t)stream, part, Wm, act, C, nseg, sub,
+                       E, scale, shift);
+  return launch_status();
+}
+
 int eqa_affine_relu_rows(const float* h, const float* scale, const float* shift, float* z, int64_t rows, int D, void* stream) {
   if (!h || !scale || !shift || !z || rows < 0 || D <= 0) return EQA_ERR_INVALID_ARG;
   if (D % 4 != 0 || (((uintptr_t)h | (uintptr_t)z | (uintptr_t)scale | (uintptr_t)shift) & 15)) return EQA_ERR_UNSUPPORTED;
diff --git a/equiadapt_amd/images/canonicalization_networks/escnn_networks.py b/equiadapt_amd/images/canonicalization_networks/escnn_networks.py
--- a/equiadapt_amd/images/canonicalization_networks/escnn_networks.py
+++ b/equiadapt_amd/images/canonicalization_networks/escnn_networks.py
@@ -467,7 +467,7 @@
                 else:
                     Bf = self._derived(conv, lambda: fftconv.spectra_for_k(bank), "fft")
                     if route == "fft5":
-                        h = fftconv.conv5x5(h, Bf, bias, True, in_bias, in_bias is not None, sums_k=sums_k)
+                        h = fftconv.conv5x5(h, Bf, bias, True, in_bias, in_bias is not None, sums_k=sums_k, sums_pieces=True)
                     else:
                         h = fftconv.conv_kxk(h, Bf, k, bias, True, in_bias, in_bias is not None)
             else:
diff --git a/equiadapt_amd/images/canonicalization_networks/fftconv.py b/equiadapt_amd/images/canonicalization_networks/fftconv.py
--- a/equiadapt_amd/images/canonicalization_networks/fftconv.py
+++ b/equiadapt_amd/images/canonicalization_networks/fftconv.py
@@ -1,3 +1,4 @@
+import ctypes
 import math
 import os
 from typing import Optional
@@ -217,11 +218,13 @@
         vbound = None
         if LIFT_FFT_FORM == "h2" and px % 16 == 0:
             wh, w_scale = self.pieces_f16()
-            xbound = torch.empty(DCMAX_SLOTS, dtype=torch.float32, device=self.device)
-            _lib.check(lib.eqa_absmax_slots(px, self.x.numel(), xbound.data_ptr(), st), "eqa_absmax_slots")
+            xbound = ops.absmax_slots_known(self.x) if ops.STEP_FUSED else None
+            if xbound is None:
+                xbound = torch.empty(DCMAX_SLOTS, dtype=torch.float32, device=self.device)
+                _lib.check(lib.eqa_absmax_slots(px, self.x.numel(), xbound.data_ptr(), st), "eqa_absmax_slots")
             if want_dc:
                 vbound = torch.empty(DCMAX_SLOTS, dtype=torch.float32, device=self.device)
-            _lib.check(lib.eqa_lift5_fft48k5_input_f16x2(px, wh.data_ptr(), w_scale, xbound.data_ptr(), DCMAX_SLOTS, p_b, int(self.relu), pV,
+            _lib.check(lib.eqa_lift5_fft48k5_input_f16x2(px, wh.data_ptr(), w_scale, xbound.data_ptr(), xbound.numel(), p_b, int(self.relu), pV,
                                                          vbound.data_ptr() if want_dc else None, *dims), "eqa_lift5_fft48k5_input_f16x2")
         elif LIFT_FFT_FORM == "bf16x3":
             _lib.check(lib.eqa_lift5_fft48k5_input_bf16x3(px, self.pieces().data_ptr(), p_b, int(self.relu), pV, *dims),
@@ -238,6 +241,22 @@
         return ops.lift_conv_nhwc(self.x, ops.pack_lift_weights(self.bank), self.bias, self.relu, 5, 5)
 
     is_contiguous = _stands_for_channels_last
+
+
+class WindowSumPieces:
+
+    def __init__(self, part: torch.Tensor, nimg: int, C: int, k: int, nseg: int, sub: int):
+        self.part, self.nseg, self.sub = part, nseg, sub
+        self.shape = torch.Size((nimg, C, k, k))
+        self.device, self.dtype, self.is_cuda = part.device, torch.float64, part.is_cuda
+
+    def materialize(self) -> torch.Tensor:
+        nimg, C, k, _ = self.shape
+        S = torch.empty(tuple(self.shape), dtype=torch.float64, device=self.device)
+        with torch.cuda.device(self.device), _timed("fft_output_sums"):
+            _lib.check(_lib.load().eqa_window_sums_nhwc_finalize(self.part.data_ptr(), S.data_ptr(), nimg, C, k, self.nseg, self.sub,
+                                                                 ops._stream()), "eqa_window_sums_nhwc_finalize")
+        return S
 
 
 LIFT_FFT_FORM = os.environ.get("EQA_LIFT_FFT_FORM", "h2")
@@ -376,7 +395,8 @@
 
 
 def conv_kxk(x: torch.Tensor, B, k: int, bias: Optional[torch.Tensor], relu: bool, in_bias: Optional[torch.Tensor] = None,
-             in_relu: bool = False, keep_V: Optional[list] = None, sums_k: int = 0, stats: Optional[list] = None) -> torch.Tensor:
+             in_relu: bool = False, keep_V: Optional[list] = None, sums_k: int = 0, stats: Optional[list] = None,
+             sums_pieces: bool = False) -> torch.Tensor:
     lib = _lib.load()
     nimg, Cin, H, W = x.shape
     if isinstance(B, Spectra3M):
@@ -412,8 +432,15 @@
         del V
         T2 = _workspace(k, nimg, OH, OW, Cout, dev)
         if sums_k:
+            ws = torch.empty(nimg * OH * TX * Cout * (2 * sums_k - 1), dtype=torch.float32, device=dev)
+            if sums_pieces and ops.STEP_FUSED:
+                nseg, sub = ctypes.c_int(0), ctypes.c_int(0)
+                with _timed("fft_output_sums"):
+                    _lib.check(lib.eqa_fft48k5_output_pieces(Mo.data_ptr(), T2.data_ptr(), p_bias, int(relu), ws.data_ptr(), nimg, OH, OW,
+                                                             Cout, sums_k, ctypes.byref(nseg), ctypes.byref(sub), st),
+                               "eqa_fft48k5_output_pieces")
+                return WindowSumPieces(ws, nimg, Cout, sums_k, nseg.value, sub.value)
             S = torch.empty((nimg, Cout, sums_k, sums_k), dtype=torch.float64, device=dev)
-            ws = torch.empty(nimg * OH * TX * Cout * (2 * sums_k - 1), dtype=torch.float32, device=dev)
             with _timed("fft_output_sums"):
                 _lib.check(lib.eqa_fft48k5_output_sums(Mo.data_ptr(), T2.data_ptr(), p_bias, int(relu), S.data_ptr(), ws.data_ptr(),
                                                        nimg, OH, OW, Cout, sums_k, st), "eqa_fft48k5_output_sums")
@@ -434,8 +461,8 @@
 
 def conv5x5(x: torch.Tensor, B: torch.Tensor, bias: Optional[torch.Tensor], relu: bool,
             in_bias: Optional[torch.Tensor] = None, in_relu: bool = False, sums_k: int = 0,
-            keep_V: Optional[list] = None, stats: Optional[list] = None) -> torch.Tensor:
-    return conv_kxk(x, B, 5, bias, relu, in_bias, in_relu, keep_V, sums_k, stats)
+            keep_V: Optional[list] = None, stats: Optional[list] = None, sums_pieces: bool = False) -> torch.Tensor:
+    return conv_kxk(x, B, 5, bias, relu, in_bias, in_relu, keep_V, sums_k, stats, sums_pieces)
 
 
 def grad_spectra(dy: torch.Tensor, k: int = 5) -> torch.Tensor:
diff --git a/equiadapt_amd/images/canonicalization_networks/pooling.py b/equiadapt_amd/images/canonicalization_networks/pooling.py
--- a/equiadapt_amd/images/canonicalization_networks/pooling.py
+++ b/equiadapt_amd/images/canonicalization_networks/pooling.py
@@ -29,13 +29,17 @@
     return window_sums_to_activations(S, layer, H, W)
 
 
-def window_sums_to_activations(S: torch.Tensor, layer, H: int, W: int) -> torch.Tensor:
+def window_sums_to_activations(S, layer, H: int, W: int) -> torch.Tensor:
+    from equiadapt_amd.images.canonicalization_networks.fftconv import WindowSumPieces
+
     k, O = layer.kernel_size, layer.out_channels
     weff = layer.mean_response_weights()
     scale = 1.0 / float(O * (H - k + 1) * (W - k + 1))
+    if isinstance(S, WindowSumPieces):
+        if not torch.is_grad_enabled() and ops.window_sums_finalize_gemv_supported(S, weff):
+            return ops.window_sums_finalize_gemv(S, weff, scale, layer.mean_bias_value())
+        S = S.materialize()
     if S.is_cuda and weff.shape[0] <= 16 and not torch.is_grad_enabled():
-        from equiadapt_amd import ops
-
         return ops.window_sums_gemv(S.flatten(1), weff, scale, layer.mean_bias_value())
     act = S.flatten(1) @ weff.t() * scale
     if layer.bias is not None:
diff --git a/equiadapt_amd/ops.py b/equiadapt_amd/ops.py
--- a/equiadapt_amd/ops.py
+++ b/equiadapt_amd/ops.py
@@ -1,9 +1,13 @@
+import os
+import weakref
 from typing import Optional, Tuple
 
 import torch
 
 from equiadapt_amd import _lib
 
+
+STEP_FUSED = os.environ.get("EQA_STEP_FUSED", "1") != "0"
 
 MAX_WINDOW_K = 10
 
@@ -380,15 +384,54 @@
     return vec, R, y
 
 
-def crop_resize_aa(x: torch.Tensor, tables, out_hw: Tuple[int, int]) -> torch.Tensor:
+_absmax_known = {}
+
+
+def _absmax_publish(y: torch.Tensor, slots: torch.Tensor) -> None:
+    key = (y.device.index, y.untyped_storage().data_ptr())
+
+    def drop(ref, key=key):
+        entry = _absmax_known.get(key)
+        if entry is not None and entry[0] is ref:
+            del _absmax_known[key]
+
+    _absmax_known[key] = (weakref.ref(y, drop), y._version, slots)
+
+
+def absmax_slots_known(x: torch.Tensor) -> Optional[torch.Tensor]:
+    entry = _absmax_known.get((x.device.index, x.untyped_storage().data_ptr()))
+    if entry is None:
+        return None
+    y = entry[0]()
+    if (y is None or x._version != entry[1] or y._version != entry[1] or x.data_ptr() != y.data_ptr() or x.shape != y.shape
+            or x.stride() != y.stride()):
+        return None
+    return entry[2]
+
+
+def crop_resize_aa(x: torch.Tensor, tables, out_hw: Tuple[int, int], pitch: int = 3) -> torch.Tensor:
     lib = _lib.load()
     x = _need(x, "x")
     wx, x0, wy, y0, K, max_rows, x_begin, x_span = tables
     B, C, H, W = x.shape
-    y = torch.empty((B, C, out_hw[0], out_hw[1]), dtype=torch.float32, device=x.device)
+    OH, OW = out_hw
+    if STEP_FUSED and C == 3 and x.data_ptr() % 16 == 0:
+        n = lib.eqa_crop_resize_aa_nhwc_slots(B, H, W, OH, OW, K, max_rows, x_begin, x_span, pitch)
+        if n > 0:
+            buf = torch.empty((B, OH, OW, pitch), dtype=torch.float32, device=x.device)
+            slots = torch.empty((n,), dtype=torch.float32, device=x.device)
+            with torch.cuda.device(x.device), _timed("crop_resize_aa"):
+                st = lib.eqa_crop_resize_aa_nhwc_absmax(x.data_ptr(), buf.data_ptr(), wx.data_ptr(), x0.data_ptr(), wy.data_ptr(),
+                                                        y0.data_ptr(), B, H, W, OH, OW, K, max_rows, x_begin, x_span, pitch,
+                                                        slots.data_ptr(), n, _stream())
+            _lib.check(st, "eqa_crop_resize_aa_nhwc_absmax")
+            y = (buf if pitch == 3 else buf[..., :3]).permute(0, 3, 1, 2)
+            _absmax_publish(y, slots)
+            return y
+    y = torch.empty((B, C, OH, OW), dtype=torch.float32, device=x.device)
     with torch.cuda.device(x.device), _timed("crop_resize_aa"):
         st = lib.eqa_crop_resize_aa(x.data_ptr(), y.data_ptr(), wx.data_ptr(), x0.data_ptr(), wy.data_ptr(), y0.data_ptr(),
-                                    B * C, H, W, out_hw[0], out_hw[1], K, max_rows, x_begin, x_span, _stream())
+                                    B * C, H, W, OH, OW, K, max_rows, x_begin, x_span, _stream())
     _lib.check(st, "eqa_crop_resize_aa")
     return y
 
@@ -653,6 +696,28 @@
     return act
 
 
+def window_sums_finalize_gemv_supported(pieces, weff: torch.Tensor) -> bool:
+    _, C, k, _ = pieces.shape
+    return bool(STEP_FUSED and pieces.is_cuda and weff.is_cuda and weff.dtype == torch.float64
+                and _lib.load().eqa_window_sums_finalize_gemv_supported(C, k, pieces.sub, weff.shape[0]))
+
+
+def window_sums_finalize_gemv(pieces, weff: torch.Tensor, scale: float, shift) -> torch.Tensor:
+    lib = _lib.load()
+    weff = _need(weff, "weff", torch.float64)
+    B, C, k, _ = pieces.shape
+    E = weff.shape[0]
+    act = torch.empty((B, E), dtype=torch.float32, device=pieces.device)
+    sh = shift if isinstance(shift, float) else 0.0
+    with torch.cuda.device(pieces.device), _timed("sums_gemv"):
+        st = lib.eqa_window_sums_finalize_gemv(pieces.part.data_ptr(), weff.data_ptr(), act.data_ptr(), B, C, k, pieces.nseg, pieces.sub, E,
+                                               float(scale), sh, _stream())
+    _lib.check(st, "eqa_window_sums_finalize_gemv")
+    if not isinstance(shift, float):
+        act += shift.to(torch.float32)
+    return act
+
+
 def window_sums_gemv_bwd(dact: torch.Tensor, weff: torch.Tensor, S: torch.Tensor, scale: float, need_dS: bool, need_dW: bool):
     lib = _lib.load()
     dact = _need(dact, "dact")
diff --git a/include/eqa_hip.h b/include/eqa_hip.h
--- a/include/eqa_hip.h
+++ b/include/eqa_hip.h
@@ -46,6 +46,11 @@
 
 int eqa_crop_resize_aa(const float* x, float* y, const float* wx, const int32_t* x0, const float* wy, const int32_t* y0,
                        int planes, int H, int W, int OH, int OW, int K, int max_rows, int x_begin, int x_span, void* stream);
+
+int64_t eqa_crop_resize_aa_nhwc_slots(int nimg, int H, int W, int OH, int OW, int K, int max_rows, int x_begin, int x_span, int pitch);
+int eqa_crop_resize_aa_nhwc_absmax(const float* x, float* y, const float* wx, const int32_t* x0, const float* wy, const int32_t* y0,
+                                   int nimg, int H, int W, int OH, int OW, int K, int max_rows, int x_begin, int x_span, int pitch,
+                                   float* slots, int64_t nslots, void* stream);
 
 int eqa_mask_action_nearest(const uint8_t* m, uint8_t* out, const int32_t* eidx, const float* rtheta, const int32_t* flags,
                             int num_elements, int n_masks, int H, int W, void* stream);
@@ -133,6 +138,10 @@
 
 int eqa_window_sums_gemv(const double* S, const double* Wm, float* act, int B, int K, int E, double scale, double shift,
                          void* stream);
+int eqa_window_sums_nhwc_finalize(const float* part, double* S, int B, int C, int k, int nseg, int sub, void* stream);
+int eqa_window_sums_finalize_gemv_supported(int C, int k, int sub, int E);
+int eqa_window_sums_finalize_gemv(const float* part, const double* Wm, float* act, int B, int C, int k, int nseg, int sub, int E,
+                                  double scale, double shift, void* stream);
 
 int eqa_lift_conv_nhwc(const float* x, const float* wpk, const float* bias, int relu, float* y, int nimg, int H, int W,
                        int Cin, int KH, int KW, int Cout, void* stream);
@@ -222,6 +231,8 @@
 int eqa_fft48k5_input_grad(const float* Cg, float* T2, float* dx, int nimg, int H, int W, int C, void* stream);
 int eqa_fft48k5_output_sums(const float* Mo, float* T2, const float* bias, int relu, double* S, void* workspace, int nimg,
                             int OH, int OW, int C, int k_next, void* stream);
+int eqa_fft48k5_output_pieces(const float* Mo, float* T2, const float* bias, int relu, void* workspace, int nimg, int OH, int OW, int C,
+                              int k_next, int* nseg, int* sub, void* stream);
 
 int eqa_fft48_supported(int ksize);
 int64_t eqa_fft48_tiles(int n, int ksize);
```

Measured after the change: 70900 images/s (median of 2 runs). Within noise of the previous version (+0.6%).
